# sonniki/image-captioning-with-external-knowledge

Hardware: AMD Instinct MI355X
Metric: decode_steps_per_sec (higher is better)
Workload: dtype f32 (3xbf16 split products, fp32 accumulate); 1 GPU; cfg2: geo variant, per-GPU batch 64 x 20 decode positions, 14x14x2048 features, K=20 knowledge rows, vocab 10000; global_batch=64, graph=True, collective_backend=none, split_allreduce=False, parallelism=dp1 (one flat-bucket all-reduce per step)

## Files before the change

image-captioning-with-external-knowledge_amd/csrc/backward.hip:

```cpp
#include "common.h"

namespace ick {
namespace {

template <int NJ>
__global__ __launch_bounds__(256) void layernorm_bwd_kernel(const float* __restrict__ dy, const float* __restrict__ x,
                                                            const float* __restrict__ res,
                                                            const float* __restrict__ gamma,
                                                            const float* __restrict__ mean,
                                                            const float* __restrict__ rstd, float* __restrict__ dz,
                                                            float* __restrict__ dgamma, float* __restrict__ dbeta,
                                                            int64_t rows, int d, int rows_per_block,
                                                            float* __restrict__ dx_drop, DropArg darg,
                                                            float* __restrict__ partials) {
    chain_priority();
    extern __shared__ float sm[];
    const Dropout drop = darg.get();
    const int lane = threadIdx.x & 63, wave = threadIdx.x >> 6;
    float ag[NJ], ab[NJ], gm[NJ];
#pragma unroll
    for (int j = 0; j < NJ; ++j) {
        const int c = lane + 64 * j;
        ag[j] = 0.f; ab[j] = 0.f;
        gm[j] = c < d ? gamma[c] : 0.f;
// ... 208 lines not shown
                const float gw = g * enc / 5.0f;
#pragma unroll
                for (int w = 0; w < 5; ++w)
                    if (name[w] % kDetParts == p) dword[(int64_t)name[w] * d + c] += gw;
            }
            g = enc_g;
        }
        if (c >= type_off && ty % kDetParts == p) dtype_emb[(int64_t)ty * (d - type_off) + (c - type_off)] += g;
    }
}

__global__ __launch_bounds__(256) void fact_encode_bwd_det_kernel(const float* __restrict__ dfe,
                                                                  const int64_t* __restrict__ facts, float* __restrict__ dee,
                                                                  float* __restrict__ dpred, int num_pred, int B, int K,
                                                                  int F, int d) {
    const int p = blockIdx.x, c = blockIdx.y * 256 + threadIdx.x;
    for (int row = 0; row < B * F; ++row) {
        const int b = row / F;
        int subj = (int)facts[(int64_t)row * 3 + 1];
        int pred = (int)facts[(int64_t)row * 3 + 2];
        subj = subj < 0 ? 0 : (subj >= K ? K - 1 : subj);
        pred = pred < 0 ? 0 : (pred >= num_pred ? num_pred - 1 : pred);
        const bool e_mine = (b * K + subj) % kDetParts == p, p_mine = pred % kDetParts == p;
        if ((!e_mine && !p_mine) || c >= d) continue;
        const float g = dfe[(int64_t)row * d + c];
        if (e_mine) dee[((int64_t)b * K + subj) * d + c] += g;
        if (p_mine) dpred[(int64_t)pred * d + c] += g;
    }
}

__global__ __launch_bounds__(256) void pointer_bwd_dh_kernel(const float* __restrict__ ds, int64_t ds_ld, int col0,
                                                             const float* __restrict__ ctx, const float* __restrict__ w,
                                                             const float* __restrict__ ind, float* __restrict__ dh,
                                                             int T, int Kc, int d) {
    chain_priority();
    const int b = blockIdx.y, t = blockIdx.x;
    const float* dsr = ds + ((int64_t)b * T + t) * ds_ld + col0;
    for (int c = threadIdx.x; c < d; c += 256) {
        float acc = 0.f;
        const float* cc = ctx + (int64_t)b * Kc * d + c;
        int k = 0;
        for (; k + 8 <= Kc; k += 8) {
            float v[8], g[8];
#pragma unroll
            for (int q = 0; q < 8; ++q) {
                v[q] = cc[(int64_t)(k + q) * d];
                g[q] = dsr[k + q];
                if (ind) g[q] *= ind[((int64_t)b * T + t) * Kc + k + q];
            }
#pragma unroll
            for (int q = 0; q < 8; ++q) acc = fmaf(g[q], v[q], acc);
        }
        for (; k < Kc; ++k) {
            float g = dsr[k];
            if (ind) g *= ind[((int64_t)b * T + t) * Kc + k];
            acc = fmaf(g, cc[(int64_t)k * d], acc);
        }
        dh[((int64_t)b * T + t) * d + c] += acc * w[c];
    }
}

template <bool SEQ>
__global__ __launch_bounds__(256) void pointer_bwd_dctx_kernel(const float* __restrict__ ds, int64_t ds_ld, int col0,
                                                               const float* __restrict__ h, const float* __restrict__ ctx,
                                                               const float* __restrict__ w, const float* __restrict__ ind,
                                                               float* __restrict__ dctx, float* __restrict__ dw,
                                                               float* __restrict__ dbias, int B, int T, int Kc, int d) {
    chain_priority();
    extern __shared__ float gs[];
    float* red = gs + T * Kc;
    float* dwp = red + 4;
    const int lane = threadIdx.x & 63, wave = threadIdx.x >> 6;
  for (int b = SEQ ? 0 : blockIdx.x; b < (SEQ ? B : (int)blockIdx.x + 1); ++b) {
    float bsum = 0.f;
    for (int idx = threadIdx.x; idx < T * Kc; idx += 256) {
        const int t = idx / Kc, k = idx - t * Kc;
        float g = ds[((int64_t)b * T + t) * ds_ld + col0 + k];
        bsum += g;
        if (ind) g *= ind[((int64_t)b * T + t) * Kc + k];
        gs[idx] = g;
    }
    bsum = block_sum<4>(bsum, red);
    if (threadIdx.x == 0 && blockIdx.y == 0) { if (SEQ) dbias[0] += bsum; else atomicAdd(dbias, bsum); }
    const int c = blockIdx.y * 64 + lane;
    const bool ok = c < d;
    const float* hb = h + (int64_t)b * T * d + (ok ? c : 0);
    const float wc = ok ? w[c] : 0.f;
    float dwl = 0.f;
    for (int k = wave; k < Kc; k += 4) {
        float acc = 0.f;
        for (int t = 0; t < T; ++t) acc = fmaf(gs[t * Kc + k], hb[(int64_t)t * d], acc);
        if (ok) {
            const int64_t o = ((int64_t)b * Kc + k) * d + c;
            dctx[o] += acc * wc;
            dwl = fmaf(acc, ctx[o], dwl);
        }
    }
    dwp[wave * 64 + lane] = dwl;
    __syncthreads();
    if (wave == 0 && ok) {
        const float t = (dwp[lane] + dwp[64 + lane]) + (dwp[128 + lane] + dwp[192 + lane]);
        if (SEQ) dw[c] += t; else atomicAdd(dw + c, t);
    }
    if (SEQ) __syncthreads();
  }
}

__global__ __launch_bounds__(256) void entity_encode_bwd_kernel(int variant, const float* __restrict__ dee,
                                                                const float* __restrict__ ent, int cols,
                                                                const float* __restrict__ ee,
// ... 226 lines not shown
    hipLaunchKernelGGL(relu_bwd_kernel, dim3((int)std::min<int64_t>(ceil_div(n, 256), 2048)), dim3(256), 0,
                       (hipStream_t)stream, dy, act, dx, n, scale);
    ICK_LAUNCH_RET();
}

extern "C" int ick_colsum(const float* a, int64_t M, int32_t N, int64_t ld, float* out, void* stream) {
    ICK_CHECK_ARG(a && out && M > 0 && N > 0 && ld >= N);
    const int rpb = deterministic() ? (int)std::min<int64_t>(M, 1 << 30) : 64;
    ICK_CHECK_ARG(ceil_div(M, rpb) <= 65535);
    hipLaunchKernelGGL(colsum_kernel, dim3(ceil_div(N, 64), ceil_div(M, rpb)), dim3(256), 0, (hipStream_t)stream, a, M,
                       N, ld, out, rpb);
    ICK_LAUNCH_RET();
}

extern "C" int ick_caption_embed_bwd(const float* dx, const int64_t* captions, const int64_t* masks, float* dword,
                                     float* dee, float* dfe, int32_t B, int32_t L, int32_t K, int32_t F, int32_t V,
                                     int32_t d, int32_t pad_token, float scale, float drop_p, uint32_t drop_seed,
                                     uint32_t drop_site, const uint32_t* drop_epoch, void* stream) {
    ICK_CHECK_ARG(dx && captions && masks && dee && B > 0 && L > 0 && K > 0 && d > 0);
    if (deterministic())
        hipLaunchKernelGGL(caption_embed_bwd_det_kernel, dim3(kDetParts, ceil_div(d, 256)), dim3(256), 0,
                           (hipStream_t)stream, dx, captions, masks, dword, dee, dfe, B, L, K, F, V, d, pad_token, scale,
                           DropArg{drop_p, drop_seed, drop_site, drop_epoch});
    else
        hipLaunchKernelGGL(caption_embed_bwd_kernel, dim3(ceil_div((int64_t)B * L, 4)), dim3(256), 0, (hipStream_t)stream,
                           dx, captions, masks, dword, dee, dfe, B, L, K, F, V, d, pad_token, scale,
                           DropArg{drop_p, drop_seed, drop_site, drop_epoch});
    ICK_LAUNCH_RET();
}

extern "C" int ick_pointer_scores_bwd(const float* ds, int64_t ds_ld, int32_t col0, const float* h, const float* ctx,
                                      const float* w, const float* ind, float* dh, float* dctx, float* dw,
                                      float* dbias, int32_t B, int32_t T, int32_t Kc, int32_t d, void* stream) {
    ICK_CHECK_ARG(ds && h && ctx && w && dh && dctx && dw && dbias && B > 0 && B <= 65535 && T > 0 && Kc > 0 && d > 0);
    hipStream_t s = (hipStream_t)stream;
    hipLaunchKernelGGL(pointer_bwd_dh_kernel, dim3(T, B), dim3(256), 0, s, ds, ds_ld, col0, ctx, w, ind, dh, T, Kc, d);
    const size_t smem = ((size_t)T * Kc + 4 + 256) * sizeof(float);
    ICK_CHECK_ARG(smem <= 64 * 1024);
    if (deterministic())
        hipLaunchKernelGGL(pointer_bwd_dctx_kernel<true>, dim3(1, ceil_div(d, 64)), dim3(256), smem, s, ds, ds_ld, col0, h,
                           ctx, w, ind, dctx, dw, dbias, B, T, Kc, d);
    else
        hipLaunchKernelGGL(pointer_bwd_dctx_kernel<false>, dim3(B, ceil_div(d, 64)), dim3(256), smem, s, ds, ds_ld, col0, h,
                           ctx, w, ind, dctx, dw, dbias, B, T, Kc, d);
    ICK_LAUNCH_RET();
}

extern "C" int ick_entity_encode_bwd(int32_t variant, const float* dee, const float* entities, int32_t ent_cols,
                                     const float* ee, const float* word_emb, int32_t vocab, float* dtype_emb,
                                     int32_t ntypes, float* dword, int32_t B, int32_t K, int32_t d, void* stream) {
    ICK_CHECK_ARG(dee && entities && dtype_emb && B > 0 && K > 0 && d > 6);
    if (variant == ICK_NEWS) ICK_CHECK_ARG(ee && word_emb && vocab > 0);
    if (deterministic())
        hipLaunchKernelGGL(entity_encode_bwd_det_kernel, dim3(kDetParts, ceil_div(d, 256)), dim3(256), 0,
                           (hipStream_t)stream, variant, dee, entities, ent_cols, ee, word_emb, vocab, dtype_emb, ntypes,
                           dword, B, K, d);
    else
        hipLaunchKernelGGL(entity_encode_bwd_kernel, dim3(ceil_div((int64_t)B * K, 4)), dim3(256), 0, (hipStream_t)stream,
                           variant, dee, entities, ent_cols, ee, word_emb, vocab, dtype_emb, ntypes, dword, B, K, d);
    ICK_LAUNCH_RET();
}

extern "C" int ick_fact_encode_bwd(const float* dfe, const int64_t* facts, float* dee, float* dpred, int32_t num_pred,
                                   int32_t B, int32_t K, int32_t F, int32_t d, void* stream) {
    ICK_CHECK_ARG(dfe && facts && dee && dpred && B > 0 && K > 0 && F > 0 && d > 0);
    if (deterministic())
        hipLaunchKernelGGL(fact_encode_bwd_det_kernel, dim3(kDetParts, ceil_div(d, 256)), dim3(256), 0, (hipStream_t)stream,
                           dfe, facts, dee, dpred, num_pred, B, K, F, d);
    else
        hipLaunchKernelGGL(fact_encode_bwd_kernel, dim3(ceil_div((int64_t)B * F, 4)), dim3(256), 0, (hipStream_t)stream,
                           dfe, facts, dee, dpred, num_pred, B, K, F, d);
    ICK_LAUNCH_RET();
}

extern "C" int ick_context_gate_bwd(const int64_t* captions, const int64_t* facts, const float* dgate, float* dw,
                                    float* dbias, int32_t B, int32_t L, int32_t T, int32_t K, int32_t F, int32_t V,
                                    int32_t num_pred, int32_t d, int32_t mode, void* stream) {
// ... 53 lines not shown
```

image-captioning-with-external-knowledge_amd/csrc/common.h:

```cpp
#pragma once
#include <hip/hip_runtime.h>
#include <stdint.h>
#include <stdlib.h>

#include "ick_amd.h"

namespace ick {

using f32x4 = __attribute__((ext_vector_type(4))) float;

constexpr int kWave = 64;

inline int ceil_div(int64_t a, int64_t b) { return (int)((a + b - 1) / b); }

extern int g_deterministic;
inline bool deterministic() {
    if (g_deterministic < 0) {
        const char* e = getenv("ICK_DETERMINISTIC");
        g_deterministic = (e && e[0] && e[0] != '0') ? 1 : 0;
    }
    return g_deterministic == 1;
}

#define ICK_CHECK_ARG(cond)          \
// ... 84 lines not shown
    for (int i = 1; i < NW; ++i) r = fmaxf(r, scratch[i]);
    return r;
}

__device__ __forceinline__ uint32_t drop_hash(uint32_t seed, uint32_t site, uint32_t idx) {
    uint32_t x = idx * 0x9E3779B1u ^ (seed + site * 0x85EBCA6Bu);
    x ^= x >> 16; x *= 0x85EBCA6Bu; x ^= x >> 13; x *= 0xC2B2AE35u; x ^= x >> 16;
    return x;
}
struct Dropout {
    uint32_t thr, seed, site;
    float scale;
    __device__ __forceinline__ bool on() const { return thr != 0u; }
    __device__ __forceinline__ float mask(uint32_t idx) const { return drop_hash(seed, site, idx) >= thr ? scale : 0.f; }
};
__host__ __device__ __forceinline__ Dropout make_dropout(float p, uint32_t seed, uint32_t site) {
    Dropout d{0u, seed, site, 1.f};
    if (p > 0.f) {
        d.thr = (uint32_t)fminf(p * 4294967296.f, 4294967040.f);
        d.scale = 1.f / (1.f - p);
    }
    return d;
}
__device__ __forceinline__ uint32_t epoch_seed(uint32_t seed, const uint32_t* epoch) {
    if (epoch == nullptr) return seed;
#if defined(__HIP_DEVICE_COMPILE__)
    uint32_t v;
    asm volatile("s_load_dword %0, %1, 0x0\n\ts_waitcnt lgkmcnt(0)" : "=s"(v) : "s"(epoch) : "memory");
    return seed + v;
#else
    return seed + *epoch;
#endif
}
constexpr int kRuleHistMax = 128;
__device__ __forceinline__ uint4 rule_words(const int32_t* words) {
    if (words == nullptr) return make_uint4(0u, 0u, 0u, 0u);
#if defined(__HIP_DEVICE_COMPILE__)
    uint64_t w01;
    uint32_t w2;
    asm volatile("s_load_dwordx2 %0, %2, 0x0\n\ts_load_dword %1, %2, 0x8\n\ts_waitcnt lgkmcnt(0)"
                 : "=&s"(w01), "=&s"(w2) : "s"(words) : "memory");
    return make_uint4((uint32_t)w01, (uint32_t)(w01 >> 32), w2, 0u);
#else
    return make_uint4((uint32_t)words[0], (uint32_t)words[1], (uint32_t)words[2], (uint32_t)words[3]);
#endif
}

template <typename Tok>
__device__ __forceinline__ void mark_bans(const Tok* hist, int t, int n, int m, int end_token, uint32_t* bits, int c0,
                                          int nwords, int* hs) {
    const int tid = threadIdx.x, nt = blockDim.x;
    for (int w = tid; w < nwords; w += nt) bits[w] = 0u;
    if (n > 0)
        for (int p = tid; p < t; p += nt) hs[p] = (int)hist[p];
    __syncthreads();
    if (n > 0) {
        for (int p = n - 1 + tid; p < t; p += nt) {
            bool match = true;
            for (int j = 1; j < n; ++j) match = match && hs[p - j] == hs[t - j];
            const int c = hs[p] - c0;
            if (match && c >= 0 && c < 32 * nwords) atomicOr(&bits[c >> 5], 1u << (c & 31));
        }
    }
    if (tid == 0 && t < m) {
        const int c = end_token - c0;
        if (c >= 0 && c < 32 * nwords) atomicOr(&bits[c >> 5], 1u << (c & 31));
// ... 13 lines not shown
```

image-captioning-with-external-knowledge_amd/csrc/gemm.hip:

```cpp
#include <algorithm>
#include <cmath>
#include <cstdlib>
#include <type_traits>

#include "common.h"
#include "gemm_common.h"

#ifdef ICK_GEMM_STAMPS
__device__ unsigned long long ick_gemm_stamps[16384][8];
#define ICK_GSTAMP(i)                                                                                          \
    do {                                                                                                       \
        if (threadIdx.x == 0 && stamp_id < 16384) ick_gemm_stamps[stamp_id][i] = __builtin_readcyclecounter(); \
    } while (0)
extern "C" int ick_debug_read_gemm_stamps(unsigned long long* out, int n) {
    return (int)hipMemcpyFromSymbol(out, HIP_SYMBOL(ick_gemm_stamps), sizeof(unsigned long long) * 8 * n);
}
#else
#define ICK_GSTAMP(i)
#endif

namespace ick {

int launch_gemm_ps(const ick_gemm_args& a, bool akm, int tile, int tiles_m, int tiles_n, int kchunk, int split, int a_nt,
                   hipStream_t s);
// ... 179 lines not shown
__device__ __forceinline__ void read_frag_spl(const float* lds, int row0, int i, int q, bf16x8_t (&f)[3]) {
    const char* base = reinterpret_cast<const char*>(lds);
    if constexpr (KM) {
        constexpr int KLINE = kmajor_kline(R), PLANE = 32 * KLINE;
        const char* at = base + (8 * q + (i >> 2)) * KLINE + ((row0 ^ ((kKmSwapOn * (q & 1)) << (kmajor_swap(R) + 2))) + 4 * (i & 3)) * 2;
#pragma unroll
        for (int p = 0; p < 3; ++p) {
            const s16x4_t lo4 = __builtin_amdgcn_ds_read_tr16_b64_v4i16((lds_s16x4_ptr)(at + p * PLANE));
            const s16x4_t hi4 = __builtin_amdgcn_ds_read_tr16_b64_v4i16((lds_s16x4_ptr)(at + p * PLANE + 4 * KLINE));
            f[p] = __builtin_bit_cast(bf16x8_t, __builtin_shufflevector(lo4, hi4, 0, 1, 2, 3, 4, 5, 6, 7));
        }
    } else {
        constexpr int PLANE = R * 64;
        const int row = row0 + i;
        const char* at = base + row * 64 + 16 * (q ^ kc_swz(row));
#pragma unroll
        for (int p = 0; p < 3; ++p)
            f[p] = __builtin_bit_cast(bf16x8_t, *reinterpret_cast<const u32x4_t*>(at + p * PLANE));
    }
}

__device__ __forceinline__ bool split_major(int& bid, int& zid, int nt, int nsplit) {
    if (nsplit < 8 || (nsplit & 7) != 0) return false;
    const int lin = bid + nt * zid;
    const int x = lin & 7, j = lin >> 3;
    const int r = j / nt;
    zid = x + 8 * r;
    bid = j - r * nt;
    return true;
}

template <int WM, int WN, int TM, int TN, bool AKM, bool BKM, bool VEC, int BKT, bool SPL = false, int LSTG = 2>
__device__ __forceinline__ void gemm_tile(const ick_gemm_args& p, int tiles_m, int tiles_n, int kchunk, int bid,
                                          int zid, float* smem, bool xcd_remap = true) {
    constexpr int BM = WM * TM * 16, BN = WN * TN * 16;
    constexpr int BK = BKT;
    using SA = Stager<BM, AKM, VEC, BKT, WM * WN * 64, SPL>;
    using SB = Stager<BN, BKM, VEC, BKT, WM * WN * 64, SPL>;
    constexpr int STAGE = SA::FLOATS + SB::FLOATS;
#ifdef ICK_GEMM_STAMPS
    const int stamp_id = bid + zid * tiles_m * tiles_n;
    if (threadIdx.x == 0 && stamp_id < 16384) {
        unsigned hw;
        asm volatile("s_getreg_b32 %0, hwreg(HW_REG_HW_ID)" : "=s"(hw));
        unsigned xcc;
        asm volatile("s_getreg_b32 %0, hwreg(HW_REG_XCC_ID)" : "=s"(xcc));
        ick_gemm_stamps[stamp_id][7] = ((unsigned long long)xcc << 32) | hw;
    }
#endif
    ICK_GSTAMP(0);

    const int nwg = tiles_m * tiles_n;
    if (xcd_remap) {
        const int xcd = bid & 7, qq = nwg >> 3, rr = nwg & 7;
        bid = (xcd < rr ? xcd * (qq + 1) : rr * (qq + 1) + (xcd - rr) * qq) + (bid >> 3);
    }
    int tm, tn;
    if (tiles_m <= tiles_n) { tm = bid % tiles_m; tn = bid / tiles_m; }
    else { tn = bid % tiles_n; tm = bid / tiles_n; }
    const int m0 = tm * BM, n0 = tn * BN;
    const int kbeg = zid * kchunk;
    const int kend = min(p.K, kbeg + kchunk);

    const RowMap amap{p.a_grp, p.a_gs, p.a_gmap, p.a_rs};
    const RowMap bmap{0, 0, nullptr, p.b_rs};
    SA sa; SB sb;
    sa.init(p.A, amap, p.a_ks, m0, p.M, p.a_extent);
    const bool only = (p.flags & ICK_GEMM_COLSUM_ONLY) != 0;
    sb.init(only ? p.A : p.B, bmap, p.b_ks, n0, p.N, p.b_extent);

    const int lane = threadIdx.x & 63, wave = threadIdx.x >> 6;
    const int wm = wave / WN, wn = wave % WN;
    const int fi = lane & 15, fq = lane >> 4;

    f32x4 acc[TM][TN];
#pragma unroll
    for (int a = 0; a < TM; ++a)
#pragma unroll
        for (int b = 0; b < TN; ++b) acc[a][b] = f32x4{0.f, 0.f, 0.f, 0.f};

    const int nk = (kend - kbeg + BK - 1) / BK;
    const bool colsum = AKM && p.colsum_a != nullptr && tn == 0;
    float csum = 0.f;
    if constexpr (SPL && AKM) sa.want_cs = colsum;
    if (nk > 0) {
        sa.template load<0>(kbeg, kend);
        if (!only) sb.template load<0>(kbeg, kend);
        if (nk > 1) { sa.template load<1>(kbeg + BK, kend); if (!only) sb.template load<1>(kbeg + BK, kend); }
        sa.template store<0>(smem, kbeg, kend);
        if (!only) sb.template store<0>(smem + SA::FLOATS, kbeg, kend);
    }
    __syncthreads();
    ICK_GSTAMP(1);
    auto phase = [&](int it, auto cur) {
        constexpr int CUR = decltype(cur)::value, NXT = 1 - CUR;
        const float* As = smem + (LSTG == 2 ? CUR * STAGE : 0);
        const float* Bs = As + SA::FLOATS;
        const int k0 = kbeg + it * BK;
        if (it + 2 < nk) { sa.template load<CUR>(k0 + 2 * BK, kend); if (!only) sb.template load<CUR>(k0 + 2 * BK, kend); }
        if constexpr (SPL) {
// ... 54 lines not shown
                    for (int b = 0; b < TN; ++b)
                        acc[a][b] = __builtin_amdgcn_mfma_f32_16x16x4f32(af[a][u], bf[b][u], acc[a][b], 0, 0, 0);
        }
        if constexpr (AKM && !SPL) {
            if (colsum && threadIdx.x < BM) {
#pragma unroll 8
                for (int k = 0; k < BK; ++k) csum += As[k * SA::LD + threadIdx.x];
            }
        }
        if constexpr (LSTG == 1) __syncthreads();
        if (it + 1 < nk) {
            float* An = smem + (LSTG == 2 ? NXT * STAGE : 0);
            sa.template store<NXT>(An, k0 + BK, kend);
            if (!only) sb.template store<NXT>(An + SA::FLOATS, k0 + BK, kend);
        }
        __syncthreads();
    };
    for (int it = 0; it < nk; it += 2) {
        phase(it, std::integral_constant<int, 0>{});
        if (it + 1 < nk) phase(it + 1, std::integral_constant<int, 1>{});
    }

    ICK_GSTAMP(2);
    if constexpr (SPL && AKM) {
        if (colsum) {
            *reinterpret_cast<float4*>(smem + sa.r0 * BM + 4 * sa.c) = sa.cs;
            __syncthreads();
            if (threadIdx.x < BM) {
#pragma unroll 4
                for (int r = 0; r < SA::KP; ++r) csum += smem[r * BM + threadIdx.x];
            }
        }
    }
    if (colsum && threadIdx.x < BM && m0 + (int)threadIdx.x < p.M) atomicAdd(p.colsum_a + m0 + threadIdx.x, csum);
    if (only) return;

    gemm_epilogue<TM, TN>(p, acc, m0, n0, wm, wn, fi, fq, zid);
    ICK_GSTAMP(3);
}

template <int WM, int WN, int TM, int TN, bool AKM, bool BKM, bool VEC, int BKT, bool SPL, int LSTG = 2>
__global__ __launch_bounds__(WM * WN * 64) void gemm_kernel(ick_gemm_args p, int tiles_m, int tiles_n, int kchunk) {
    extern __shared__ __attribute__((aligned(16))) float smem[];
    if constexpr (TM == 1) chain_priority();
    const int nt = tiles_m * tiles_n;
    int bid = blockIdx.x, zid = blockIdx.z;
    const bool by_split = split_major(bid, zid, nt, gridDim.z);
    gemm_tile<WM, WN, TM, TN, AKM, BKM, VEC, BKT, SPL, LSTG>(p, tiles_m, tiles_n, kchunk, bid, zid, smem, !by_split);
}

constexpr int kGroupMax = 8;
struct GroupArgs {
    int count;
    int wg_end[kGroupMax];
    int tiles_m[kGroupMax], tiles_n[kGroupMax], kchunk[kGroupMax], split[kGroupMax];
    ick_gemm_args g[kGroupMax];
};

template <int WM, int WN, int TM, int TN, bool AKM, bool BKM, bool VEC, int BKT, bool SPL>
__global__ __launch_bounds__(256) void gemm_group_kernel(GroupArgs ga) {
    extern __shared__ __attribute__((aligned(16))) float smem[];
    int gi = 0;
    while (gi + 1 < ga.count && (int)blockIdx.x >= ga.wg_end[gi]) ++gi;
    const int local = blockIdx.x - (gi > 0 ? ga.wg_end[gi - 1] : 0);
    const int nt = ga.tiles_m[gi] * ga.tiles_n[gi];
    if (local >= nt * ga.split[gi]) return;
    int zid = local / nt, bid = local - zid * nt;
    const bool by_split = split_major(bid, zid, nt, ga.split[gi]);
    gemm_tile<WM, WN, TM, TN, AKM, BKM, VEC, BKT, SPL>(ga.g[gi], ga.tiles_m[gi], ga.tiles_n[gi], ga.kchunk[gi], bid, zid,
                                                       smem, !by_split);
}

struct Plan {
    ick_gemm_args a;
    bool akm, bkm, vec;
    bool big;
    bool wide;
    bool spl;
    bool xl;
    bool ps;
    int ps_tile, ps_nt;
    int tiles_m, tiles_n, kchunk, split;
};

template <int WM, int WN, int TM, int TN, bool AKM, bool BKM, bool VEC, bool SPL, int LSTG = 2>
int launch_tile_s(const Plan& pl, hipStream_t s) {
    constexpr int BM = WM * TM * 16, BN = WN * TN * 16, NT = WM * WN * 64;
    constexpr int STAGE = Stager<BM, AKM, VEC, 32, NT, SPL>::FLOATS + Stager<BN, BKM, VEC, 32, NT, SPL>::FLOATS;
    constexpr size_t smem = LSTG * STAGE * sizeof(float);
    static_assert(smem <= 160 * 1024, "tile exceeds the LDS of a CU");
    const size_t lds = smem;
    if (lds > 64 * 1024) {
        static LdsAttrOnce attr;
        if (int e = attr.ensure(reinterpret_cast<const void*>(gemm_kernel<WM, WN, TM, TN, AKM, BKM, VEC, 32, SPL, LSTG>), 160 * 1024))
            return e;
    }
    const int gx = pl.tiles_m * pl.tiles_n;
    hipLaunchKernelGGL((gemm_kernel<WM, WN, TM, TN, AKM, BKM, VEC, 32, SPL, LSTG>), dim3(gx, 1, pl.split),
                       dim3(NT), lds, s, pl.a, pl.tiles_m, pl.tiles_n, pl.kchunk);
    ICK_LAUNCH_RET();
}
template <int WM, int WN, int TM, int TN, bool AKM, bool BKM, bool VEC>
int launch_tile(const Plan& pl, hipStream_t s) {
// ... 52 lines not shown
        g_gemm_split = e ? std::min(2, std::max(0, atoi(e))) : 1;
    }
    return g_gemm_split;
}

inline bool aligned16(const void* p) { return (reinterpret_cast<uintptr_t>(p) & 15) == 0; }

int make_plan(const ick_gemm_args* in, Plan& pl, int force_big = 0) {
    if (!in) return ICK_EINVAL;
    ick_gemm_args& a = pl.a;
    a = *in;
    if (a.flags & ICK_GEMM_COLSUM_ONLY) {
        ICK_CHECK_ARG(a.A && a.colsum_a && a.M > 0 && a.K > 0);
        a.B = a.A; a.C = a.colsum_a; a.bias = nullptr; a.gate = nullptr;
        a.N = 1; a.b_rs = 1; a.b_ks = a.a_ks; a.c_rs = 1; a.c_grp = 0; a.hs_dh = 0; a.b_extent = a.a_extent;
        a.drop_p = 0.f;
        a.flags = ICK_GEMM_COLSUM_ONLY | ICK_GEMM_ATOMIC;
    }
    ICK_CHECK_ARG(a.A && a.B && a.C);
    ICK_CHECK_ARG(a.M > 0 && a.N > 0 && a.K > 0);
    const bool akm = a.a_rs == 1 && a.a_ks != 1, bkm = a.b_rs == 1 && a.b_ks != 1;
    ICK_CHECK_ARG((a.a_rs == 1) || (a.a_ks == 1));
    ICK_CHECK_ARG((a.b_rs == 1) || (a.b_ks == 1));
    if (a.split_k > 1) ICK_CHECK_ARG(a.flags & ICK_GEMM_ATOMIC);
    if (a.colsum_a) ICK_CHECK_ARG(akm);
    if (a.gate) ICK_CHECK_ARG(a.hs_dh <= 0 && a.c_grp <= 0 && a.split_k <= 1 && !(a.flags & (ICK_GEMM_ATOMIC | ICK_GEMM_ACCUM)));
    if (a.hs_dh > 0) {
        ICK_CHECK_ARG(a.hs_dhp >= a.hs_dh && a.hs_H > 0 && a.hs_S > 0 && a.hs_s0 >= 0);
        ICK_CHECK_ARG(a.N % (a.hs_H * a.hs_dh) == 0);
        ICK_CHECK_ARG(a.hs_s0 + (a.c_grp > 0 ? a.c_grp : a.M) <= a.hs_S);
    } else {
        a.hs_dh = 0;
    }
    if (a.a_grp <= 0) { a.a_grp = 0; a.a_gmap = nullptr; }
    if (a.c_grp <= 0) { a.c_grp = 0; a.c_gmap = nullptr; }
    bool avec, bvec;
    if (akm) {
        avec = aligned16(a.A) && a.a_ks % 4 == 0 && a.M % 4 == 0 && (a.a_grp == 0 || (a.a_grp % 4 == 0 && a.a_gs % 4 == 0));
    } else {
        avec = aligned16(a.A) && a.a_rs % 4 == 0 && a.K % 4 == 0 && (a.a_grp == 0 || a.a_gs % 4 == 0);
    }
    if (a.flags & ICK_GEMM_COLSUM_ONLY) bvec = true;
    else if (bkm) bvec = aligned16(a.B) && a.b_ks % 4 == 0 && a.N % 4 == 0;
    else bvec = aligned16(a.B) && a.b_rs % 4 == 0 && a.K % 4 == 0;
    auto extent_of = [](int64_t rows, int64_t rs, int64_t K, int64_t ks, int grp, int64_t gs, bool has_map) -> int64_t {
        if (has_map) return 0;
        if (grp <= 0) return (rows - 1) * rs + (K - 1) * ks + 1;
        const int64_t ng = (rows + grp - 1) / grp;
        return (ng - 1) * gs + (std::min<int64_t>(grp, rows) - 1) * rs + (K - 1) * ks + 1;
    };
    if (a.a_extent <= 0) a.a_extent = extent_of(a.M, a.a_rs, a.K, a.a_ks, a.a_grp, a.a_gs, a.a_gmap != nullptr);
    if (a.b_extent <= 0) a.b_extent = extent_of(a.N, a.b_rs, a.K, a.b_ks, 0, 0, false);
    const int64_t kMaxExtent = ((int64_t)1 << 29) - 64;
    a.a_extent = std::min(a.a_extent & ~(int64_t)3, kMaxExtent - 4);
    a.b_extent = std::min(a.b_extent & ~(int64_t)3, kMaxExtent - 4);
    const int64_t a_need = extent_of(a.M, a.a_rs, a.K, a.a_ks, a.a_grp, a.a_gs, a.a_gmap != nullptr);
    const int64_t b_need = extent_of(a.N, a.b_rs, a.K, a.b_ks, 0, 0, false);
    pl.vec = avec && bvec && a.a_extent >= 4 && a.b_extent >= 4 && a_need <= a.a_extent + 3 && b_need <= a.b_extent + 3;
    pl.akm = akm; pl.bkm = bkm;
    a.flags &= 0xff;
    const int split_req = a.split_k > 1 ? a.split_k : 1;
    const int64_t wgs64 = (int64_t)ceil_div(a.M, 64) * ceil_div(a.N, 64) * split_req;
    pl.big = !pl.vec || wgs64 >= 512;
    if (force_big > 0) pl.big = true;
    pl.wide = pl.vec && pl.big && a.M >= 128 && akm && !bkm && a.N <= 320 && a.M >= 4096 && a.K >= 1024 && split_req == 1;
    pl.spl = pl.vec && pl.big && (gemm_split_mode() == 2 || (gemm_split_mode() == 1 && !bkm));
// ... 139 lines not shown
```

image-captioning-with-external-knowledge_amd/csrc/gemm_common.h:

```cpp
#pragma once
#include "common.h"

namespace ick {
namespace {

struct RowMap {
    int grp;
    int64_t gs;
    const int32_t* gmap;
    int64_t rs;
    __device__ __forceinline__ int64_t operator()(int r) const {
        if (grp <= 0) return (int64_t)r * rs;
        const int g = r / grp;
        const int i = r - g * grp;
        const int64_t gg = gmap ? (int64_t)gmap[g] : (int64_t)g;
        return gg * gs + (int64_t)i * rs;
    }
};

template <int N>
__device__ __forceinline__ void map_rows(const RowMap& m, const int (&rows)[N], int64_t (&off)[N]) {
    if (m.grp <= 0) {
#pragma unroll
        for (int i = 0; i < N; ++i) off[i] = (int64_t)rows[i] * m.rs;
// ... 13 lines not shown
    for (int i = 0; i < N; ++i) off[i] = (int64_t)g[i] * m.gs + (int64_t)in[i] * m.rs;
}

__device__ __forceinline__ int64_t col_offset(const ick_gemm_args& p, int col) {
    if (p.hs_dh <= 0) return col;
    const int hd = p.hs_H * p.hs_dh;
    const int seg = col / hd, r = col - seg * hd;
    const int h = r / p.hs_dh, j = r - h * p.hs_dh;
    return ((int64_t)seg * p.hs_H + h) * ((int64_t)p.hs_S * p.hs_dhp) + j;
}

typedef unsigned int u32x4_t __attribute__((ext_vector_type(4)));
constexpr uint32_t kOobOffset = 0x80000000u;

typedef __bf16 bf16x2_t __attribute__((ext_vector_type(2)));
typedef __bf16 bf16x8_t __attribute__((ext_vector_type(8)));
typedef float f32x2_t __attribute__((ext_vector_type(2)));
typedef short s16x4_t __attribute__((ext_vector_type(4)));
typedef __attribute__((address_space(3))) s16x4_t* lds_s16x4_ptr;

__device__ __forceinline__ uint32_t pack_bf16(float a, float b) {
    return __builtin_bit_cast(uint32_t, __builtin_convertvector(f32x2_t{a, b}, bf16x2_t));
}
__device__ __forceinline__ void split3(float a, float b, uint32_t& hi, uint32_t& mid, uint32_t& lo) {
    hi = pack_bf16(a, b);
    const float ra = a - __builtin_bit_cast(float, hi << 16), rb = b - __builtin_bit_cast(float, hi & 0xffff0000u);
    mid = pack_bf16(ra, rb);
    const float sa = ra - __builtin_bit_cast(float, mid << 16), sb = rb - __builtin_bit_cast(float, mid & 0xffff0000u);
    lo = pack_bf16(sa, sb);
}
__device__ __forceinline__ int kc_swz(int row) { return (-(row >> 2)) & 3; }

template <int TM, int TN>
__device__ __forceinline__ void gemm_epilogue(const ick_gemm_args& p, f32x4 (&acc)[TM][TN], int m0, int n0, int wm, int wn,
                                              int fi, int fq, int zid) {
    const bool hs = p.hs_dh > 0;
    const RowMap cmap{p.c_grp, p.c_gs, p.c_gmap, hs ? (int64_t)p.hs_dhp : p.c_rs};
    const int64_t row_bias = hs ? (int64_t)p.hs_s0 * p.hs_dhp : 0;
    const bool relu = p.flags & ICK_GEMM_RELU;
    const int mode = (p.flags & ICK_GEMM_ATOMIC) ? 2 : ((p.flags & ICK_GEMM_ACCUM) ? 1 : 0);
    float bv[TN];
    int cols[TN];
    int64_t co[TN];
#pragma unroll
    for (int b = 0; b < TN; ++b) {
        cols[b] = n0 + (wn * TN + b) * 16 + fi;
        co[b] = col_offset(p, cols[b]);
        bv[b] = (p.bias != nullptr && zid == 0 && cols[b] < p.N) ? p.bias[cols[b]] : 0.f;
    }
    const float alpha = p.alpha;
    int64_t coff[TM][4];
    int rowid[TM][4];
    const Dropout drop = make_dropout(p.drop_p, epoch_seed(p.drop_seed, p.drop_epoch), p.drop_site);
    {
        int rws[TM * 4];
        int64_t mo[TM * 4];
#pragma unroll
        for (int a = 0; a < TM; ++a)
#pragma unroll
            for (int r = 0; r < 4; ++r) {
                rowid[a][r] = m0 + (wm * TM + a) * 16 + fq * 4 + r;
                rws[a * 4 + r] = min(rowid[a][r], p.M - 1);
            }
        map_rows<TM * 4>(cmap, rws, mo);
#pragma unroll
        for (int a = 0; a < TM; ++a)
#pragma unroll
            for (int r = 0; r < 4; ++r) coff[a][r] = rowid[a][r] < p.M ? mo[a * 4 + r] + row_bias : -1;
    }
#pragma unroll
    for (int a = 0; a < TM; ++a)
#pragma unroll
        for (int r = 0; r < 4; ++r)
#pragma unroll
            for (int b = 0; b < TN; ++b) {
                float v = acc[a][b][r] * alpha + bv[b];
                if (relu) v = fmaxf(v, 0.f);
                if (drop.on()) v *= drop.mask((uint32_t)rowid[a][r] * (uint32_t)p.N + (uint32_t)cols[b]);
                acc[a][b][r] = v;
            }
    if (p.gate != nullptr) {
        float g[TM][4][TN];
#pragma unroll
        for (int a = 0; a < TM; ++a)
#pragma unroll
            for (int r = 0; r < 4; ++r)
#pragma unroll
                for (int b = 0; b < TN; ++b)
                    g[a][r][b] = p.gate[(coff[a][r] >= 0 && cols[b] < p.N) ? (int64_t)rowid[a][r] * p.gate_rs + cols[b] : 0];
#pragma unroll
        for (int a = 0; a < TM; ++a)
#pragma unroll
            for (int r = 0; r < 4; ++r)
#pragma unroll
                for (int b = 0; b < TN; ++b) acc[a][b][r] = g[a][r][b] > 0.f ? acc[a][b][r] * p.gate_scale : 0.f;
    }
    if (mode == 1) {
        float old[TM][4][TN];
#pragma unroll
        for (int a = 0; a < TM; ++a)
#pragma unroll
// ... 33 lines not shown
```

image-captioning-with-external-knowledge_amd/csrc/gemm_ps.hip:

```cpp
#include <algorithm>

#include "gemm_common.h"

#ifdef ICK_PS_STAMPS
__device__ unsigned long long ick_ps_stamps[10];
#define ICK_PSTAMP(var)                                   \
    do {                                                  \
        __builtin_amdgcn_sched_barrier(0);                \
        var = __builtin_amdgcn_s_memtime();               \
        __builtin_amdgcn_sched_barrier(0);                \
    } while (0)
extern "C" int ick_debug_read_ps_stamps(unsigned long long* out) {
    return (int)hipMemcpyFromSymbol(out, HIP_SYMBOL(ick_ps_stamps), sizeof(ick_ps_stamps));
}
#else
#define ICK_PSTAMP(var)
#endif

namespace ick {
namespace {

typedef __attribute__((address_space(3))) void* lds_void_ptr;

inline int64_t ps_rows(int N) { return (int64_t)ceil_div(N, 64) * 64; }
inline int64_t ps_bytes(int N, int K) { return (int64_t)ceil_div(K, 32) * 3 * ps_rows(N) * 64; }

constexpr int kPsMaxItems = 16;
struct PsBatch {
    int count;
    int first[kPsMaxItems + 1];
    ick_presplit_item it[kPsMaxItems];
};

__global__ __launch_bounds__(256) void presplit_kernel(PsBatch b) {
    __shared__ float tile[64][33];
    int gi = 0;
    while (gi + 1 < b.count && (int)blockIdx.x >= b.first[gi + 1]) ++gi;
    const ick_presplit_item it = b.it[gi];
    const int local = blockIdx.x - b.first[gi];
    const int blocks_n = (it.N + 63) / 64;
    const int nb = local % blocks_n, s = local / blocks_n;
    const int t = threadIdx.x;
    const float* src = it.src;
    const bool al16 = (reinterpret_cast<uintptr_t>(src) & 15) == 0;
    if (it.src_cs == 1) {
        const int r = t >> 2, kk = (t & 3) * 8;
        const int n = nb * 64 + r;
        const int k0 = 32 * s + kk;
        if (al16 && (it.src_rs & 3) == 0 && n < it.N && k0 + 7 < it.K) {
            const float4* q = reinterpret_cast<const float4*>(src + (int64_t)n * it.src_rs + k0);
            const float4 a = q[0], b = q[1];
            tile[r][kk + 0] = a.x; tile[r][kk + 1] = a.y; tile[r][kk + 2] = a.z; tile[r][kk + 3] = a.w;
            tile[r][kk + 4] = b.x; tile[r][kk + 5] = b.y; tile[r][kk + 6] = b.z; tile[r][kk + 7] = b.w;
        } else {
#pragma unroll
            for (int j = 0; j < 8; ++j) {
                const int k = k0 + j;
                tile[r][kk + j] = (n < it.N && k < it.K) ? src[(int64_t)n * it.src_rs + k] : 0.f;
            }
        }
    } else {
        const int kk = t >> 3, r0 = (t & 7) * 8;
        const int k = 32 * s + kk;
        const int n0 = nb * 64 + r0;
        if (al16 && it.src_rs == 1 && (it.src_cs & 3) == 0 && n0 + 7 < it.N && k < it.K) {
            const float4* q = reinterpret_cast<const float4*>(src + n0 + (int64_t)k * it.src_cs);
            const float4 a = q[0], b = q[1];
            tile[r0 + 0][kk] = a.x; tile[r0 + 1][kk] = a.y; tile[r0 + 2][kk] = a.z; tile[r0 + 3][kk] = a.w;
            tile[r0 + 4][kk] = b.x; tile[r0 + 5][kk] = b.y; tile[r0 + 6][kk] = b.z; tile[r0 + 7][kk] = b.w;
        } else {
#pragma unroll
            for (int j = 0; j < 8; ++j) {
                const int n = n0 + j;
                tile[n - nb * 64][kk] = (n < it.N && k < it.K) ? src[(int64_t)n * it.src_rs + (int64_t)k * it.src_cs] : 0.f;
            }
        }
    }
    __syncthreads();
    const int r = t >> 2, c = t & 3;
    uint32_t h[4], m[4], l[4];
#pragma unroll
    for (int j = 0; j < 4; ++j) split3(tile[r][8 * c + 2 * j], tile[r][8 * c + 2 * j + 1], h[j], m[j], l[j]);
    const int64_t np = (int64_t)blocks_n * 64;
    char* dst = reinterpret_cast<char*>(it.dst) + ((int64_t)s * 3 * np + nb * 64 + r) * 64 + c * 16;
    *reinterpret_cast<uint4*>(dst) = uint4{h[0], h[1], h[2], h[3]};
    *reinterpret_cast<uint4*>(dst + np * 64) = uint4{m[0], m[1], m[2], m[3]};
    *reinterpret_cast<uint4*>(dst + 2 * np * 64) = uint4{l[0], l[1], l[2], l[3]};
}

}

template <int WM_, int WN_, int TM_, int TN_, bool AKM_, int D_, int PF_>
struct PsCfg {
    static constexpr int WM = WM_, WN = WN_, TM = TM_, TN = TN_, D = D_;
    static constexpr int PF = PF_ < TN_ ? PF_ : TN_;
    static constexpr int ST = D + 1;
    static constexpr bool AKM = AKM_;
    static constexpr int BM = WM * TM * 16, BN = WN * TN * 16, NW = WM * WN, NT = NW * 64;
    static constexpr int A_STAGE = BM * 32 * 4;
    static constexpr int B_PLANE = BN * 64;
    static constexpr int B_STAGE = 3 * B_PLANE;
    static constexpr int NPA = BM / 8;
    static constexpr int NPB = 3 * BN / 16;
    static constexpr int PA_W = NPA / NW;
    static constexpr int PB_W = (NPB + NW - 1) / NW;
    static constexpr bool UNIFORM = D >= 2;
    static constexpr int SCRATCH = UNIFORM && (NPB % NW != 0) ? 1024 : 0;
// ... 74 lines not shown
#ifdef ICK_PS_STAMPS
    unsigned long long t_start = 0, t_loop = 0, t_end = 0;
    ICK_PSTAMP(t_start);
    const unsigned long long rt_start = __builtin_amdgcn_s_memrealtime();
#endif
    char* const As = smem_ps;
    char* const Bs = smem_ps + ST * C::A_STAGE;
    char* const scratch = Bs + ST * C::B_STAGE;
    const int lane = threadIdx.x & 63;
    const int wave = __builtin_amdgcn_readfirstlane((int)(threadIdx.x >> 6));
    constexpr int WN = C::WN;
    const int wm = wave / WN, wn = wave % WN;
    const int fi = lane & 15, fq = lane >> 4;

    int bid = blockIdx.x;
    int zid = blockIdx.z;
    {
        const int nwg = tiles_m * tiles_n;
        if (gridDim.z > 1) {
            const int total = nwg * (int)gridDim.z, lin = bid + nwg * zid;
            const int xcd = lin & 7, qq = total >> 3, rr = total & 7;
            const int v = xcd * qq + min(xcd, rr) + (lin >> 3);
            zid = v / nwg;
            bid = v - zid * nwg;
        } else {
            const int xcd = bid & 7, qq = nwg >> 3, rr = nwg & 7;
            bid = (xcd < rr ? xcd * (qq + 1) : rr * (qq + 1) + (xcd - rr) * qq) + (bid >> 3);
        }
    }
    int tm, tn;
    if (tiles_m <= tiles_n) { tm = bid % tiles_m; tn = bid / tiles_m; }
    else { tn = bid % tiles_n; tm = bid / tiles_n; }
    const int m0 = tm * BM, n0 = tn * BN;
    const int kbeg = zid * kchunk;
    const int kend = min(p.K, kbeg + kchunk);
    const int nk = (kend - kbeg + 31) >> 5;
    const int s0 = kbeg >> 5;

    const __amdgpu_buffer_rsrc_t rsrc_a =
        __builtin_amdgcn_make_buffer_rsrc(const_cast<float*>(p.A), (short)0, (int)(p.a_extent * 4), 0x00020000);
    const RowMap amap{p.a_grp, p.a_gs, p.a_gmap, p.a_rs};
    uint32_t avoff[C::PA_W];
    int akl[C::PA_W];
#pragma unroll
    for (int j = 0; j < C::PA_W; ++j) {
        const int g = wave + NW * j;
        int row, extra;
        if constexpr (AKM) {
            constexpr int LPK = BM / 4, KPP = 64 / LPK;
            const int kl = g * KPP + lane / LPK, cpos = lane % LPK;
            const int c = (cpos - 4 * ((kl >> 3) & 3)) & (LPK - 1);
            row = m0 + 4 * c;
            akl[j] = kl;
            extra = 0;
            const int one[1] = {min(row, p.M - 1)};
            int64_t mo[1];
            map_rows<1>(amap, one, mo);
            avoff[j] = row < p.M ? (uint32_t)(mo[0] * 4) + (uint32_t)((int64_t)kl * p.a_ks * 4) : kOobOffset;
        } else {
            const int rt = g * 8 + (lane >> 3), cpos = lane & 7;
            const int c = cpos ^ ((rt >> 1) & 7);
            row = m0 + rt;
            akl[j] = 4 * c;
            extra = 4 * c;
            const int one[1] = {min(row, p.M - 1)};
            int64_t mo[1];
            map_rows<1>(amap, one, mo);
            avoff[j] = row < p.M ? (uint32_t)((mo[0] + extra) * 4) : kOobOffset;
        }
    }
    const __amdgpu_buffer_rsrc_t rsrc_b =
        __builtin_amdgcn_make_buffer_rsrc(const_cast<void*>(p.b_ps), (short)0, (int)bps_bytes, 0x00020000);
    const uint32_t bvoff = (uint32_t)((n0 + (lane >> 2)) * 64 + (((lane & 3) ^ ((-(lane >> 4)) & 3)) * 16));

    auto dma_b = [&](int it, int buf) { ps_dma_b<C>(rsrc_b, Bs, scratch, buf, wave, bvoff, s0 + it, it < nk, n0, np_rows); };
    auto dma_a = [&](int it, int buf) {
        const int k0 = kbeg + 32 * it;
        const uint32_t soff = it < nk ? (uint32_t)(AKM ? (int64_t)k0 * p.a_ks * 4 : (int64_t)k0 * 4) : 0u;
        ps_dma_a<C>(rsrc_a, As, buf, wave, avoff, akl, k0, kend, soff, a_nt != 0);
    };

    f32x4 acc[TM][TN];
#pragma unroll
    for (int a = 0; a < TM; ++a)
#pragma unroll
        for (int b = 0; b < TN; ++b) acc[a][b] = f32x4{0.f, 0.f, 0.f, 0.f};

#pragma unroll
    for (int i = 0; i < D; ++i) { dma_b(i, i); dma_a(i, i); }
    ICK_WAIT_VMCNT(C::IN_FLIGHT);
    ICK_LDS_BARRIER();

#ifdef ICK_PS_STAMPS
    unsigned long long ph[6] = {0, 0, 0, 0, 0, 0}, ta = 0, tb = 0, tc = 0, td = 0, te = 0, tf = 0;
    ICK_PSTAMP(t_loop);
#endif
    int buf = 0;
    for (int it = 0; it < nk; ++it) {
        ICK_PSTAMP(ta);
        int nb = buf + D;
        if (nb >= ST) nb -= ST;
// ... 56 lines not shown
                for (int j = 0; j < GB; ++j)
#pragma unroll
                    for (int a = 0; a < TM; ++a) {
                        const int b = g * GB + j;
                        if (b < TN)
                            acc[a][b] = __builtin_amdgcn_mfma_f32_16x16x32_bf16(af[a][pa[q]], bf[g & 1][j][pb[q]], acc[a][b], 0, 0, 0);
                    }
                constexpr int NS = NG * 6, NP = C::PB_W + C::PA_W;
                constexpr int SPAN = D >= 2 ? NS : (NS + 1) / 2;
                constexpr int STRIDE = SPAN / NP > 0 ? SPAN / NP : 1;
                const int slot = g * 6 + q;
                if (slot % STRIDE == 0 && slot / STRIDE < NP) piece(slot / STRIDE);
                if (slot == NS - 1) {
#pragma unroll
                    for (int r = (NS - 1) / STRIDE + 1; r < NP; ++r) piece(r);
                }
            }
        }
        ICK_PSTAMP(td);
        ICK_WAIT_VMCNT(C::IN_FLIGHT);
        ICK_PSTAMP(te);
        ICK_LDS_BARRIER();
        ICK_PSTAMP(tf);
#ifdef ICK_PS_STAMPS
        ph[0] += tb - ta; ph[1] += tc - tb; ph[2] += td - tc; ph[3] += te - td; ph[4] += tf - te; ph[5] += 1;
#endif
        if (++buf == ST) buf = 0;
    }
#ifdef ICK_PS_STAMPS
    ICK_PSTAMP(t_end);
    const unsigned long long t_loop_end = t_end;
#endif
    ICK_WAIT_VMCNT(0);
    gemm_epilogue<TM, TN>(p, acc, m0, n0, wm, wn, fi, fq, zid);
#ifdef ICK_PS_STAMPS
    asm volatile("s_waitcnt vmcnt(0)" ::: "memory");
    ICK_PSTAMP(t_end);
    if (threadIdx.x == 0 && blockIdx.x == (gridDim.x >> 1) && blockIdx.z == 0) {
        for (int i = 0; i < 6; ++i) ick_ps_stamps[i] = ph[i];
        ick_ps_stamps[6] = t_loop - t_start;
        ick_ps_stamps[7] = t_end - t_loop_end;
        ick_ps_stamps[8] = t_end - t_start;
        ick_ps_stamps[9] = __builtin_amdgcn_s_memrealtime() - rt_start;
    }
#endif
}


namespace {

template <class C>
int launch_ps_cfg(const ick_gemm_args& a, int np_rows, int64_t bytes, int tiles_m, int tiles_n, int kchunk, int split,
                  int a_nt, hipStream_t s) {
    static LdsAttrOnce attr;
    if (int e = attr.ensure(reinterpret_cast<const void*>(gemm_ps_kernel<C::WM, C::WN, C::TM, C::TN, C::AKM, C::D, C::PF>), 160 * 1024))
        return e;
    hipLaunchKernelGGL((gemm_ps_kernel<C::WM, C::WN, C::TM, C::TN, C::AKM, C::D, C::PF>), dim3(tiles_m * tiles_n, 1, split),
                       dim3(C::NT), C::LDS, s, a, np_rows, bytes, tiles_m, tiles_n, kchunk, a_nt);
    ICK_LAUNCH_RET();
}

template <int WM, int WN, int TM, int TN, int D, int PF>
int launch_ps_tile(const ick_gemm_args& a, bool akm, int np, int64_t bytes, int tiles_m, int tiles_n, int kchunk, int split,
                   int a_nt, hipStream_t s) {
    if (akm) return launch_ps_cfg<PsCfg<WM, WN, TM, TN, true, D, PF>>(a, np, bytes, tiles_m, tiles_n, kchunk, split, a_nt, s);
    return launch_ps_cfg<PsCfg<WM, WN, TM, TN, false, D, PF>>(a, np, bytes, tiles_m, tiles_n, kchunk, split, a_nt, s);
}
// ... 18 lines not shown
        case 1: return launch_ps_tile<8, 1, 1, 8, 1, 2>(a, akm, np, bytes, tiles_m, tiles_n, kchunk, split, a_nt, s);
        case 2: return launch_ps_tile<8, 1, 1, 10, 2, 10>(a, akm, np, bytes, tiles_m, tiles_n, kchunk, split, a_nt, s);
        case 3: return launch_ps_tile<4, 2, 2, 10, 1, 3>(a, akm, np, bytes, tiles_m, tiles_n, kchunk, split, a_nt, s);
        case 4: return launch_ps_tile<8, 1, 1, 8, 2, 8>(a, akm, np, bytes, tiles_m, tiles_n, kchunk, split, a_nt, s);
        case 5: return launch_ps_tile<4, 2, 2, 4, 1, 2>(a, akm, np, bytes, tiles_m, tiles_n, kchunk, split, a_nt, s);
        case 6: return launch_ps_tile<4, 2, 2, 5, 2, 5>(a, akm, np, bytes, tiles_m, tiles_n, kchunk, split, a_nt, s);
        case 7: return launch_ps_tile<4, 1, 2, 8, 1, 2>(a, akm, np, bytes, tiles_m, tiles_n, kchunk, split, a_nt, s);
        case 8: return launch_ps_tile<2, 2, 2, 5, 1, 5>(a, akm, np, bytes, tiles_m, tiles_n, kchunk, split, a_nt, s);
        case 9: return launch_ps_tile<8, 1, 1, 5, 1, 2>(a, akm, np, bytes, tiles_m, tiles_n, kchunk, split, a_nt, s);
        case 10: return launch_ps_tile<8, 1, 1, 10, 1, 10>(a, akm, np, bytes, tiles_m, tiles_n, kchunk, split, a_nt, s);
    }
    return ICK_EINVAL;
}

}

extern "C" int ick_presplit_bytes(int32_t N, int32_t K, int64_t* bytes) {
    if (N <= 0 || K <= 0 || !bytes) return ICK_EINVAL;
    *bytes = ick::ps_bytes(N, K);
    return ICK_OK;
}

extern "C" int ick_presplit_weights(const ick_presplit_item* items, int32_t count, void* stream) {
    using namespace ick;
    if (!items || count <= 0) return ICK_EINVAL;
    for (int i0 = 0; i0 < count; i0 += kPsMaxItems) {
        PsBatch b;
        b.count = std::min(kPsMaxItems, count - i0);
        int total = 0;
        for (int i = 0; i < b.count; ++i) {
            const ick_presplit_item& it = items[i0 + i];
            ICK_CHECK_ARG(it.src && it.dst && it.N > 0 && it.K > 0);
            ICK_CHECK_ARG(it.src_cs == 1 || it.src_rs == 1);
            ICK_CHECK_ARG((reinterpret_cast<uintptr_t>(it.dst) & 15) == 0);
            b.it[i] = it;
            b.first[i] = total;
            total += ceil_div(it.N, 64) * ceil_div(it.K, 32);
        }
        b.first[b.count] = total;
        hipLaunchKernelGGL(presplit_kernel, dim3(total), dim3(256), 0, (hipStream_t)stream, b);
        hipError_t e = hipGetLastError();
        if (e != hipSuccess) return (int)e;
    }
    return ICK_OK;
}
```

image-captioning-with-external-knowledge_amd/csrc/score_head.hip:

```cpp
#include "common.h"

namespace ick {
namespace {

constexpr int kMaxPerLane = 16;

template <int NJ>
__global__ __launch_bounds__(256) void pointer_scores_kernel(const float* __restrict__ h, const float* __restrict__ ctx,
                                                             const float* __restrict__ w, const float* __restrict__ bias,
                                                             const float* __restrict__ ind, float* __restrict__ out,
                                                             int T, int Kc, int d, int64_t out_ld, int col0,
                                                             const int32_t* __restrict__ out_gmap) {
    chain_priority();
    constexpr int KB = 4;
    const int lane = threadIdx.x & 63, wave = threadIdx.x >> 6;
    const int b = blockIdx.y, t = blockIdx.x;
    const float* hr = h + ((int64_t)b * T + t) * d;
    float hv[NJ], wv[NJ];
#pragma unroll
    for (int j = 0; j < NJ; ++j) {
        const int c = lane + 64 * j;
        hv[j] = c < d ? hr[c] : 0.f;
        wv[j] = c < d ? w[c] : 0.f;
    }
    const int ob = out_gmap ? out_gmap[b] : b;
    float* orow = out + ((int64_t)ob * T + t) * out_ld + col0;
    const float bs = bias[0];
    for (int k0 = wave; k0 < Kc; k0 += 4 * KB) {
        float cv[KB][NJ];
#pragma unroll
        for (int q = 0; q < KB; ++q) {
            const int k = k0 + 4 * q;
            const float* cr = ctx + ((int64_t)b * Kc + (k < Kc ? k : 0)) * d;
#pragma unroll
            for (int j = 0; j < NJ; ++j) {
                const int c = lane + 64 * j;
                cv[q][j] = (k < Kc && c < d) ? cr[c] : 0.f;
            }
        }
#pragma unroll
        for (int q = 0; q < KB; ++q) {
            const int k = k0 + 4 * q;
            if (k >= Kc) break;
            float acc = 0.f;
#pragma unroll
            for (int j = 0; j < NJ; ++j) acc = fmaf(__fmul_rn(hv[j], cv[q][j]), wv[j], acc);
            acc = wave_sum(acc);
            if (lane == 0) {
                const float f = ind ? ind[((int64_t)b * T + t) * Kc + k] : 1.f;
                orow[k] = acc * f + bs;
            }
        }
    }
}

struct Top2 {
    float v1, v2;
    int i1, i2;
};
// ... 81 lines not shown
    }
    out = o[i];
    if (i < max_len - 1) {
        next_token[b] = out;
        next_mask[b] = (has_facts && out >= V + K) ? 2 : (out >= V ? 1 : 0);
    }
}

__global__ void greedy_update_kernel(const int32_t* __restrict__ best, const int32_t* __restrict__ second,
                                     int64_t* __restrict__ output, int32_t* __restrict__ hist,
                                     int32_t* __restrict__ finished, int64_t* __restrict__ next_token,
                                     int64_t* __restrict__ next_mask, int B, int step, int max_len, int V, int K,
                                     int has_facts, int end_token) {
    const int b = blockIdx.x * blockDim.x + threadIdx.x;
    if (b >= B) return;
    greedy_update_one(b, best[b], second[b], output, hist, finished, next_token, next_mask, step, max_len, V, K,
                      has_facts, end_token);
}

__global__ __launch_bounds__(256) void greedy_select_kernel(const float* __restrict__ scores, int64_t ld, int Vx,
                                                            int64_t* __restrict__ output, int32_t* __restrict__ hist,
                                                            int32_t* __restrict__ finished,
                                                            int64_t* __restrict__ next_token,
                                                            int64_t* __restrict__ next_mask, int step, int max_len,
                                                            int V, int K, int has_facts, int end_token) {
    __shared__ Top2 sh[256];
    const int b = blockIdx.x;
    const Top2 t = row_top2(scores + (int64_t)b * ld, Vx, sh);
    if (threadIdx.x == 0)
        greedy_update_one(b, t.i1, t.i2 == 0x7fffffff ? t.i1 : t.i2, output, hist, finished, next_token, next_mask, step,
                          max_len, V, K, has_facts, end_token);
}

template <bool kWeighted>
__global__ __launch_bounds__(256) void packed_ce_rows_kernel(const float* __restrict__ scores, int64_t ld,
                                                             const int64_t* __restrict__ caps,
                                                             const int32_t* __restrict__ dl, int L, int Vx, int pad,
                                                             float* __restrict__ row_loss, float* __restrict__ dscores,
                                                             const float* __restrict__ weight) {
    __shared__ float red[4];
    const int t = blockIdx.x, b = blockIdx.y, tid = threadIdx.x;
    const int64_t row = (int64_t)b * L + t;
    const float* r = scores + row * ld;
    float* dr = dscores ? dscores + row * ld : nullptr;
    int64_t target = -1;
    bool use = t < L - 1 && t < dl[b];
    if (use) {
        target = caps[(int64_t)b * L + t + 1];
        use = target != pad && target >= 0 && target < Vx;
    }
    if (!use) {
        if (tid == 0) row_loss[row] = -1.f;
        if (dr) {
            const int z4 = ((ld & 3) == 0 && (reinterpret_cast<uintptr_t>(dscores) & 15) == 0) ? (int)(Vx >> 2) : 0;
            float4* d4 = reinterpret_cast<float4*>(dr);
            for (int i = tid; i < z4; i += 256) d4[i] = make_float4(0.f, 0.f, 0.f, 0.f);
            for (int i = 4 * z4 + tid; i < Vx; i += 256) dr[i] = 0.f;
        }
        return;
    }
    constexpr int kCeVec = 10;
    const bool in_regs = (Vx & 3) == 0 && (ld & 3) == 0 && Vx <= 256 * 4 * kCeVec &&
                         (reinterpret_cast<uintptr_t>(scores) & 15) == 0 &&
                         (dr == nullptr || (reinterpret_cast<uintptr_t>(dscores) & 15) == 0);
    if (in_regs) {
        const float4* r4 = reinterpret_cast<const float4*>(r);
        const int n4 = Vx >> 2;
        float4 x[kCeVec];
        float m = -INFINITY;
#pragma unroll
        for (int j = 0; j < kCeVec; ++j) {
            const int i = tid + 256 * j;
            x[j] = i < n4 ? r4[i] : make_float4(-INFINITY, -INFINITY, -INFINITY, -INFINITY);
            m = fmaxf(m, fmaxf(fmaxf(x[j].x, x[j].y), fmaxf(x[j].z, x[j].w)));
        }
        m = block_max<4>(m, red);
        float s = 0.f;
#pragma unroll
        for (int j = 0; j < kCeVec; ++j) {
// ... 81 lines not shown
            }
#pragma unroll
            for (int j = 0; j < 4; ++j) {
                const int i = i0 + tid + 256 * j;
                if (i < n4) {
                    float4 gq = make_float4(__expf(x[j].x - m) * inv, __expf(x[j].y - m) * inv, __expf(x[j].z - m) * inv,
                                            __expf(x[j].w - m) * inv);
                    if (i == tq) {
                        if (tr == 0) gq.x -= wr; else if (tr == 1) gq.y -= wr; else if (tr == 2) gq.z -= wr; else gq.w -= wr;
                    }
                    d4[i] = gq;
                }
            }
        }
        for (int i0 = 4 * n4; i0 < Vx; i0 += 256 * 8) {
            float x[8];
#pragma unroll
            for (int j = 0; j < 8; ++j) {
                const int i = i0 + tid + 256 * j;
                x[j] = i < Vx ? r[i] : 0.f;
            }
#pragma unroll
            for (int j = 0; j < 8; ++j) {
                const int i = i0 + tid + 256 * j;
                if (i < Vx) dr[i] = __expf(x[j] - m) * inv - (i == target ? wr : 0.f);
            }
        }
    }
}

template <bool kWeighted>
__global__ __launch_bounds__(256) void packed_ce_reduce_kernel(const float* __restrict__ row_loss, int n, int L,
                                                               const float* __restrict__ weight,
                                                               float* __restrict__ loss_sum, float* __restrict__ count) {
    __shared__ float red[4];
    float s = 0.f, c = 0.f;
    for (int i = threadIdx.x; i < n; i += 256) {
        const float v = row_loss[i];
        if (v > -0.5f) { s += kWeighted ? weight[i / L] * v : v; c += 1.f; }
    }
    s = block_sum<4>(s, red);
    c = block_sum<4>(c, red);
    if (threadIdx.x == 0) { loss_sum[0] = s; count[0] = c; }
}

}
}

extern "C" int ick_pointer_scores(const float* h, const float* ctx, const float* w, const float* bias,
                                  const float* ind, float* out, int32_t B, int32_t T, int32_t Kc, int32_t d,
                                  int64_t out_ld, int32_t col0, const int32_t* out_gmap, void* stream) {
    using namespace ick;
    ICK_CHECK_ARG(h && ctx && w && bias && out && B > 0 && T > 0 && Kc > 0 && d > 0 && d <= 64 * kMaxPerLane);
    ICK_CHECK_ARG(B <= 65535 && col0 >= 0 && out_ld >= col0 + Kc);
    hipStream_t s = (hipStream_t)stream;
    if (d <= 320)
        hipLaunchKernelGGL(pointer_scores_kernel<5>, dim3(T, B), dim3(256), 0, s, h, ctx, w, bias, ind, out, T, Kc, d,
                           out_ld, col0, out_gmap);
    else if (d <= 512)
        hipLaunchKernelGGL(pointer_scores_kernel<8>, dim3(T, B), dim3(256), 0, s, h, ctx, w, bias, ind, out, T, Kc, d,
                           out_ld, col0, out_gmap);
    else
        hipLaunchKernelGGL(pointer_scores_kernel<kMaxPerLane>, dim3(T, B), dim3(256), 0, s, h, ctx, w, bias, ind, out, T,
                           Kc, d, out_ld, col0, out_gmap);
    ICK_LAUNCH_RET();
}

extern "C" int ick_top2(const float* scores, int64_t ld, int32_t B, int32_t Vx, int32_t* best, int32_t* second,
                        void* stream) {
    using namespace ick;
    ICK_CHECK_ARG(scores && best && second && B > 0 && Vx > 0 && ld >= Vx);
    hipLaunchKernelGGL(top2_kernel, dim3(B), dim3(256), 0, (hipStream_t)stream, scores, ld, Vx, best, second);
    ICK_LAUNCH_RET();
}

extern "C" int ick_greedy_update(const int32_t* best, const int32_t* second, int64_t* output, int32_t* top2_hist,
                                 int32_t* finished, int64_t* next_token, int64_t* next_mask, int32_t B, int32_t step,
                                 int32_t max_len, int32_t V, int32_t K, int32_t has_facts, int32_t end_token,
                                 void* stream) {
    using namespace ick;
    ICK_CHECK_ARG(best && second && output && top2_hist && finished && next_token && next_mask);
    ICK_CHECK_ARG(B > 0 && step >= 0 && step < max_len);
    hipLaunchKernelGGL(greedy_update_kernel, dim3(ceil_div(B, 64)), dim3(64), 0, (hipStream_t)stream, best, second,
                       output, top2_hist, finished, next_token, next_mask, B, step, max_len, V, K, has_facts,
                       end_token);
    ICK_LAUNCH_RET();
}

extern "C" int ick_greedy_select(const float* scores, int64_t ld, int32_t B, int32_t Vx, int64_t* output,
                                 int32_t* top2_hist, int32_t* finished, int64_t* next_token, int64_t* next_mask,
                                 int32_t step, int32_t max_len, int32_t V, int32_t K, int32_t has_facts,
                                 int32_t end_token, void* stream) {
    using namespace ick;
    ICK_CHECK_ARG(scores && output && top2_hist && finished && next_token && next_mask);
    ICK_CHECK_ARG(B > 0 && Vx > 0 && ld >= Vx && step >= 0 && step < max_len);
    hipLaunchKernelGGL(greedy_select_kernel, dim3(B), dim3(256), 0, (hipStream_t)stream, scores, ld, Vx, output,
                       top2_hist, finished, next_token, next_mask, step, max_len, V, K, has_facts, end_token);
    ICK_LAUNCH_RET();
}

extern "C" int ick_packed_ce(const float* scores, int64_t ld, const int64_t* captions_sorted,
                             const int32_t* decode_len, int32_t B, int32_t L, int32_t Vx, int32_t pad_token,
                             float* row_loss, float* loss_sum, float* count, float* dscores, void* stream) {
    using namespace ick;
    ICK_CHECK_ARG(scores && captions_sorted && decode_len && row_loss && loss_sum && count);
    ICK_CHECK_ARG(B > 0 && B <= 65535 && L > 0 && Vx > 0 && ld >= Vx);
    hipStream_t s = (hipStream_t)stream;
    hipLaunchKernelGGL(packed_ce_rows_kernel<false>, dim3(L, B), dim3(256), 0, s, scores, ld, captions_sorted, decode_len,
                       L, Vx, pad_token, row_loss, dscores, nullptr);
    hipLaunchKernelGGL(packed_ce_reduce_kernel<false>, dim3(1), dim3(256), 0, s, row_loss, B * L, L, nullptr, loss_sum,
                       count);
    ICK_LAUNCH_RET();
}

extern "C" int ick_packed_ce_weighted(const float* scores, int64_t ld, const int64_t* captions_sorted,
                                      const int32_t* decode_len, const float* weights, int32_t B, int32_t L, int32_t Vx,
                                      int32_t pad_token, float* row_loss, float* loss_sum, float* count, float* dscores,
                                      void* stream) {
    using namespace ick;
    ICK_CHECK_ARG(scores && captions_sorted && decode_len && weights && row_loss && loss_sum && count);
    ICK_CHECK_ARG(B > 0 && B <= 65535 && L > 0 && Vx > 0 && ld >= Vx && (int64_t)B * L <= INT32_MAX);
    hipStream_t s = (hipStream_t)stream;
    hipLaunchKernelGGL(packed_ce_rows_kernel<true>, dim3(L, B), dim3(256), 0, s, scores, ld, captions_sorted, decode_len,
                       L, Vx, pad_token, row_loss, dscores, weights);
    hipLaunchKernelGGL(packed_ce_reduce_kernel<true>, dim3(1), dim3(256), 0, s, row_loss, B * L, L, weights, loss_sum,
                       count);
    ICK_LAUNCH_RET();
}
```

image-captioning-with-external-knowledge_amd/decoder.py:

```python
import math
import os
import struct

import torch
from torch import nn

from . import ops
from .lib import IckError

VARIANT_TYPE_OFFSET = {"geo": 4, "knowledge": 6, "news": 5}
VARIANT_NUM_TYPES = {"geo": 1000, "knowledge": 1000, "news": 20}
VARIANT_NUM_PREDICATES = {"geo": 0, "knowledge": 3000, "news": 3500}


def _sinusoid_table(max_len, d):
    pos = torch.arange(max_len, dtype=torch.float32).unsqueeze(1)
    freq = torch.exp(torch.arange(0, d, 2, dtype=torch.float32) * (-math.log(10000.0) / d))
    table = torch.zeros(max_len, d)
    table[:, 0::2] = torch.sin(pos * freq)
    table[:, 1::2] = torch.cos(pos * freq)
    return table.unsqueeze(1)


class _GraphedCall:
# ... 689 lines not shown
        dh = d // H
        x = t["x"]
        B, T, _ = x.shape
        t["ca"] = torch.empty_like(x)
        t["lse_c"] = torch.empty(B * H * T, device=x.device, dtype=torch.float32) if save else None
        ops.attention_heads(t["qc"], kv, t["ca"], H, dh, T, S, 0, 2 * li, 2 * li + 1, lse=t["lse_c"], drop=t["d_ca"])
        if pk is None:
            t["o2"] = ops.linear(t["ca"], *_wb(layer.multihead_attn.out_proj))
            t["x2"], t["m2"], t["r2"] = _with_stats(ops.add_layernorm(
                t["o2"], t["x1"], *_ln(layer.norm2), save_stats=save, drop=t["d2"]), save)
            t["f"] = ops.linear(t["x2"], *_wb(layer.linear1), relu=True, drop=t["d_ff"])
            t["o3"] = ops.linear(t["f"], *_wb(layer.linear2))
            x3, t["m3"], t["r3"] = _with_stats(ops.add_layernorm(
                t["o3"], t["x2"], *_ln(layer.norm3), save_stats=save, drop=t["d3"]), save)
            return x3, None
        t["x2"] = torch.empty_like(x)
        t["o2"], t["o3"] = (torch.empty_like(x), torch.empty_like(x)) if save else (None, None)
        t["f"] = torch.empty(B, T, layer.linear1.out_features, device=x.device, dtype=torch.float32)
        t["m2"], t["r2"] = ops.rowchain_fwd(
            t["ca"], pk[("d", li, "co")], layer.multihead_attn.out_proj.bias.detach(), t["x1"], *_ln(layer.norm2),
            t["x2"], drop1=t["d2"], o_out=t["o2"], save_stats=save, w2p=pk[("d", li, "l1")],
            b2=layer.linear1.bias.detach(), y2=t["f"], relu=True, drop2=t["d_ff"])
        layers = self.transformer_decoder.layers
        nxt = layers[li + 1] if li + 1 < len(layers) else None
        x3 = torch.empty_like(x)
        qkv_n = None if nxt is None else torch.empty(B, 3, H, T, ops.DHP, device=x.device, dtype=torch.float32)
        t["m3"], t["r3"] = ops.rowchain_fwd(
            t["f"], pk[("d", li, "l2")], layer.linear2.bias.detach(), t["x2"], *_ln(layer.norm3), x3, drop1=t["d3"],
            o_out=t["o3"], save_stats=save, w2p=None if nxt is None else pk[("d", li + 1, "si")],
            b2=None if nxt is None else nxt.self_attn.in_proj_bias.detach(), y2=qkv_n,
            heads=None if nxt is None else (3, H, T, 0, T))
        return x3, qkv_n

    def _score_head(self, h, ee, fe, eib, hv, out, vocab_ps=None):
        B, T, d = h.shape
        V, K = self.vocab_size, ee.shape[1]
        ops.gemm_raw(h if hv is None else hv, self.fc_vocab.weight.detach(), out, B * T, V, d, d, 1, d, 1, out.stride(1),
                     bias=self.fc_vocab.bias.detach(), b_ps=vocab_ps)
        ops.pointer_scores(h, ee, *_wb(self.fc_entity), out, V)
        if self.has_facts:
            ops.pointer_scores(h, fe, *_wb(self.fc_fact), out, V + K, ind=eib)

    @torch.no_grad()
    def get_context_indicators(self, captions, facts, entity_context_size, out_length):
        if not self.has_facts:
            raise AttributeError("the geo variant has no get_context_indicators (geo-aware/models.py)")
        dev = self.fc_vocab.weight.device
        captions = captions.to(device=dev, dtype=torch.int64)
        facts = facts.to(device=dev, dtype=torch.int64).contiguous()
        B, Lc = captions.shape
        mode = 1 if out_length == 1 else 0
        if mode == 0 and out_length > Lc:
            captions = torch.cat([captions, captions.new_full((B, out_length - Lc), self.word_map["<pad>"])], dim=1)
        eib, pi = ops.context_indicators(captions.contiguous(), facts, entity_context_size, self.vocab_size, mode=mode,
                                         dense_pred=self.num_predicates)
        return eib[:, :out_length].unsqueeze(3), pi[:, :out_length].unsqueeze(3)

    @torch.no_grad()
    def get_scores(self, h, entities_encoded, facts_encoded=None, entity_idx_before=None, predicate_indicator=None):
        dev = self.fc_vocab.weight.device
        hb = h.detach().to(dev, torch.float32).permute(1, 0, 2).contiguous()
        ee = entities_encoded.detach().to(dev, torch.float32).contiguous()
        B, T, d = hb.shape
        fe = eib = hv = None
        if self.has_facts:
            if facts_encoded is None or entity_idx_before is None or predicate_indicator is None:
                raise IckError("%s variant: get_scores(h, entities_encoded, facts_encoded, entity_idx_before, "
                               "predicate_indicator)" % self.variant)
            fe = facts_encoded.detach().to(dev, torch.float32).contiguous()
            eib = entity_idx_before.detach().to(dev, torch.float32).reshape(B, T, fe.shape[1]).contiguous()
            pi = predicate_indicator.detach().to(dev, torch.float32).reshape(B * T, self.num_predicates).contiguous()
            gate = ops.linear(pi, self.fc_predicate.weight.detach(), self.fc_predicate.bias.detach()).view(B, T, d)
            hv = ops.mul(hb, gate)
        out = torch.empty(B, T, self.vocab_size + ee.shape[1] + (0 if fe is None else fe.shape[1]), device=dev,
# ... 603 lines not shown
```

image-captioning-with-external-knowledge_amd/lib.py:

```python
import ctypes as C
import os

_PKG = os.path.dirname(os.path.abspath(__file__))
LIB_PATH = os.path.join(_PKG, "libick_amd.so")
if os.environ.get("ICK_LIB_PATH"):
    LIB_PATH = os.environ["ICK_LIB_PATH"]

ICK_GEO, ICK_KNOWLEDGE, ICK_NEWS = 0, 1, 2
VARIANT_ID = {"geo": ICK_GEO, "knowledge": ICK_KNOWLEDGE, "news": ICK_NEWS}
GEMM_RELU, GEMM_ACCUM, GEMM_ATOMIC, GEMM_COLSUM_ONLY = 1, 2, 4, 16

vp = C.c_void_p
i32 = C.c_int32
i64 = C.c_int64
f32 = C.c_float
u32 = C.c_uint32


class GemmArgs(C.Structure):
    _fields_ = [
        ("A", vp), ("B", vp), ("C", vp), ("bias", vp),
        ("M", i32), ("N", i32), ("K", i32),
        ("a_rs", i64), ("a_ks", i64), ("a_grp", i32), ("a_gs", i64), ("a_gmap", vp),
        ("b_rs", i64), ("b_ks", i64),
        ("c_rs", i64), ("c_grp", i32), ("c_gs", i64), ("c_gmap", vp),
        ("flags", i32), ("split_k", i32), ("alpha", f32),
        ("hs_dh", i32), ("hs_dhp", i32), ("hs_H", i32), ("hs_S", i32), ("hs_s0", i32),
        ("drop_p", f32), ("drop_seed", u32), ("drop_site", u32), ("drop_epoch", vp),
        ("a_extent", i64), ("b_extent", i64), ("colsum_a", vp),
        ("gate", vp), ("gate_rs", i64), ("gate_scale", f32),
        ("b_ps", vp),
    ]


class RowChainArgs(C.Structure):
    _fields_ = [
        ("A", vp), ("a_rs", i64), ("a_grp", i32), ("a_gs", i64),
        ("M", i32), ("K1", i32), ("d", i32),
        ("w1p", vp), ("b1", vp), ("res", vp), ("res_rs", i64),
        ("gamma", vp), ("beta", vp), ("eps", f32),
        ("drop1_p", f32), ("drop_seed", u32), ("drop1_site", u32), ("drop_epoch", vp),
        ("o", vp), ("o_rs", i64),
        ("x", vp), ("x_rs", i64), ("x_grp", i32), ("x_gs", i64),
        ("mean", vp), ("rstd", vp),
        ("w2p", vp), ("b2", vp), ("N2", i32), ("flags", i32),
        ("drop2_p", f32), ("drop2_site", u32),
        ("y2", vp), ("y2_rs", i64), ("y2_grp", i32), ("y2_gs", i64),
        ("hs_dh", i32), ("hs_dhp", i32), ("hs_H", i32), ("hs_S", i32), ("hs_s0", i32),
    ]


class RowChainBwdArgs(C.Structure):
    _fields_ = [
        ("M", i32), ("d", i32), ("drop_seed", u32), ("drop_epoch", vp),
        ("g0", vp), ("g0_rs", i64), ("K0", i32), ("w0p", vp), ("g0_grp", i32), ("g0_gs", i64),
        ("dzin", vp), ("dzin_rs", i64),
        ("o1", vp), ("res1", vp), ("mean1", vp), ("rstd1", vp), ("gamma1", vp),
        ("drop1_p", f32), ("drop1_site", u32),
        ("do1", vp), ("part1", vp),
        ("w1p", vp), ("N1", i32), ("act", vp), ("gate_scale", f32), ("t_out", vp),
        ("w2p", vp),
        ("o2", vp), ("res2", vp), ("mean2", vp), ("rstd2", vp), ("gamma2", vp),
        ("drop2_p", f32), ("drop2_site", u32),
        ("do2", vp), ("part2", vp),
        ("w3p", vp), ("out3", vp), ("dz_out", vp), ("flags", i32),
    ]


class PackItem(C.Structure):
    _fields_ = [("src", vp), ("dst", vp), ("N", i32), ("K", i32), ("src_rs", i64), ("src_cs", i64), ("dst_rs", i64)]


class GemmPlanInfo(C.Structure):
    _fields_ = [(n, i32) for n in ("tile_m", "tile_n", "waves", "tiles_m", "tiles_n", "split_k", "a_kmajor", "b_kmajor",
                                   "vec", "split_bf16", "presplit")]


class PresplitItem(C.Structure):
    _fields_ = [("src", vp), ("dst", vp), ("N", i32), ("K", i32), ("src_rs", i64), ("src_cs", i64)]


class AdamItem(C.Structure):
    _fields_ = [("off", i64), ("rows", i32), ("K", i32), ("drow0", i32), ("Nd", i32), ("pack", vp), ("pack_t", vp),
                ("copy", vp), ("ps", vp), ("ps_t", vp), ("tr", vp), ("copy_ld", i64), ("tr_ld", i64)]


class AdamBlock(C.Structure):
    _fields_ = [("item", i32), ("tn", i32), ("tk", i32), ("cnt4", i32), ("off4", i64), ("copy", vp)]


class AttnArgs(C.Structure):
    _fields_ = [
        ("Q", vp), ("K", vp), ("V", vp), ("O", vp), ("lse", vp),
        ("B", i32), ("H", i32), ("T", i32), ("S", i32), ("dh", i32),
        ("q_bs", i64), ("q_hs", i64), ("q_ts", i64), ("k_bs", i64), ("k_hs", i64), ("k_ss", i64),
        ("v_bs", i64), ("v_hs", i64), ("v_ss", i64), ("o_bs", i64), ("o_ts", i64),
        ("scale", f32), ("causal", i32), ("q_pos0", i32), ("kv_len", vp),
        ("drop_p", f32), ("drop_seed", u32), ("drop_site", u32), ("drop_epoch", vp),
    ]


class AttnBwdArgs(C.Structure):
    _fields_ = [
        ("Q", vp), ("K", vp), ("V", vp), ("O", vp), ("dO", vp), ("lse", vp), ("dQ", vp), ("dK", vp), ("dV", vp),
        ("B", i32), ("H", i32), ("T", i32), ("S", i32), ("dh", i32),
        ("q_bs", i64), ("q_hs", i64), ("q_ts", i64), ("k_bs", i64), ("k_hs", i64), ("k_ss", i64),
        ("v_bs", i64), ("v_hs", i64), ("v_ss", i64), ("o_bs", i64), ("o_ts", i64),
        ("dq_bs", i64), ("dq_ts", i64), ("dk_bs", i64), ("dk_ss", i64), ("dv_bs", i64), ("dv_ss", i64),
        ("scale", f32), ("causal", i32), ("q_pos0", i32),
        ("drop_p", f32), ("drop_seed", u32), ("drop_site", u32), ("drop_epoch", vp),
    ]

# ... 80 lines not shown
    "ick_decode_layers_attn": [C.POINTER(DecodeCtx), vp, i32, i32, vp],
    "ick_decode_init": [C.POINTER(DecodeCtx), i32, i32, vp],
    "ick_decode_select_greedy": [C.POINTER(DecodeCtx), i32, vp],
    "ick_decode_select_beam": [C.POINTER(DecodeCtx), C.POINTER(BeamState), i32, vp],
    "ick_decode_beam_supported": [i32, i32],
    "ick_decode_select_sample": [C.POINTER(DecodeCtx), C.POINTER(SampleState), i32, vp],
    "ick_decode_sample_supported": [i32, i32],
    "ick_decode_select_beam_rules": [C.POINTER(DecodeCtx), C.POINTER(BeamState), C.POINTER(DecodeRules), i32, vp],
    "ick_decode_select_sample_rules": [C.POINTER(DecodeCtx), C.POINTER(SampleState), C.POINTER(DecodeRules), i32, vp],
    "ick_decode_select_beam_diverse": [C.POINTER(DecodeCtx), C.POINTER(BeamState), C.POINTER(DecodeRules),
                                       C.POINTER(DecodeDiversity), i32, vp],
    "ick_decode_select_beam_forced": [C.POINTER(DecodeCtx), C.POINTER(BeamState), C.POINTER(DecodeRules),
                                      C.POINTER(DecodeConstraints), i32, vp],
    "ick_attention_bwd": [C.POINTER(AttnBwdArgs), vp],
    "ick_layernorm_bwd": [vp, vp, vp, vp, vp, vp, vp, vp, vp, i64, i32, vp, f32, u32, u32, vp, vp, vp],
    "ick_layernorm_bwd_rows_per_block": [],
    "ick_gemm_grouped": [vp, i32, vp],
    "ick_attention_bwd_overwrites": [i32, i32, i32],
    "ick_attention_plan": [i32, i32, i32, i32, i32, C.POINTER(i32)],
    "ick_relu_bwd": [vp, vp, vp, i64, f32, vp],
    "ick_colsum": [vp, i64, i32, i64, vp, vp],
    "ick_caption_embed_bwd": [vp, vp, vp, vp, vp, vp, i32, i32, i32, i32, i32, i32, i32, f32, f32, u32, u32, vp, vp],
    "ick_pointer_scores_bwd": [vp, i64, i32, vp, vp, vp, vp, vp, vp, vp, vp, i32, i32, i32, i32, vp],
    "ick_entity_encode_bwd": [i32, vp, vp, i32, vp, vp, i32, vp, i32, vp, i32, i32, i32, vp],
    "ick_fact_encode_bwd": [vp, vp, vp, vp, i32, i32, i32, i32, i32, vp],
    "ick_context_gate_bwd": [vp, vp, vp, vp, vp, i32, i32, i32, i32, i32, i32, i32, i32, i32, vp],
    "ick_adam_clamp": [vp, vp, vp, vp, i64, f32, f32, f32, f32, f32, f32, i32, vp, vp, vp],
    "ick_adam_clamp_derive": [vp, vp, vp, vp, vp, vp, i32, f32, f32, f32, f32, f32, f32, i32, vp, vp, vp],
    "ick_counter_add": [vp, u32, vp],
    "ick_counter_add_if": [vp, u32, vp, vp],
    "ick_timestamp": [vp, vp],
    "ick_copy_batch": [vp, vp, vp, i32, vp],
    "ick_scale_by_ratio": [vp, i64, vp, vp, vp],
}

_lib = None
PROFILE = None
_proxy = None


class IckError(RuntimeError):
    pass


def load():
    return _proxy if _proxy is not None else load_raw()


def load_raw():
    global _lib
    if _lib is None:
        if not os.path.exists(LIB_PATH):
            raise IckError(
                "libick_amd.so is missing (%s): build it with `python -c 'import __graft_entry__ as g; g.build()'`"
                " -- there is no fallback path" % LIB_PATH)
        import torch
        lib = C.CDLL(LIB_PATH)
        for name, argtypes in SIGNATURES.items():
            fn = getattr(lib, name)
            fn.argtypes = argtypes
            fn.restype = C.c_int
        _lib = lib
    return _lib


_ERRS = {-1: "ICK_EINVAL (bad shape / null pointer / unsupported size)", -2: "ICK_EALIGN", -3: "ICK_EWORKSPACE"}
# ... 6 lines not shown
```

image-captioning-with-external-knowledge_amd/ops.py:

```python
import contextlib
import ctypes as C
import gc
import math
import os

import torch

from . import lib as L


def _p(t):
    return None if t is None else t.data_ptr()


def _stream():
    return torch.cuda.current_stream().cuda_stream


def _f32c(t, name):
    if t.dtype != torch.float32 or not t.is_cuda:
        raise L.IckError("%s must be a float32 device tensor (got %s on %s)" % (name, t.dtype, t.device))
    return t


TIMED = None


def _extent(t):
    return (t.untyped_storage().nbytes() - t.storage_offset() * t.element_size()) // 4


def _drop(a, drop):
    if drop is not None and drop[0] > 0.0:
        a.drop_p, a.drop_seed, a.drop_site = float(drop[0]), int(drop[1]) & 0xFFFFFFFF, int(drop[2]) & 0xFFFFFFFF
        a.drop_epoch = _p(drop[3]) if len(drop) > 3 else None


def _dargs(drop):
    if drop is not None and drop[0] > 0.0:
        return (float(drop[0]), int(drop[1]) & 0xFFFFFFFF, int(drop[2]) & 0xFFFFFFFF,
                _p(drop[3]) if len(drop) > 3 else None)
    return 0.0, 0, 0, None


def gemm_args(A, B, Cout, M, N, K, a_rs, a_ks, b_rs, b_ks, c_rs, bias=None, a_grp=0, a_gs=0, a_gmap=None,
              c_grp=0, c_gs=0, c_gmap=None, relu=False, accumulate=False, atomic=False, split_k=1, alpha=1.0,
              drop=None, colsum_a=None, gate=None, gate_scale=1.0, b_ps=None):
    for t in (A, B, Cout):
        if t.dtype != torch.float32:
            raise L.IckError("ick_gemm operands must be float32, got %s" % t.dtype)
    a = L.GemmArgs()
    a.A, a.B, a.C, a.bias = _p(A), _p(B), _p(Cout), _p(bias)
    a.M, a.N, a.K = M, N, K
    a.a_rs, a.a_ks, a.a_grp, a.a_gs, a.a_gmap = a_rs, a_ks, a_grp, a_gs, _p(a_gmap)
    a.b_rs, a.b_ks = b_rs, b_ks
    a.c_rs, a.c_grp, a.c_gs, a.c_gmap = c_rs, c_grp, c_gs, _p(c_gmap)
    a.flags = (L.GEMM_RELU if relu else 0) | (L.GEMM_ACCUM if accumulate else 0) | (L.GEMM_ATOMIC if atomic else 0)
    a.split_k = split_k
    a.alpha = alpha
    a.a_extent, a.b_extent = _extent(A), _extent(B)
    a.colsum_a = _p(colsum_a)
    if gate is not None:
        a.gate, a.gate_rs, a.gate_scale = _p(gate), gate.stride(0), gate_scale
    if b_ps is not None:
        assert b_ps.numel() * b_ps.element_size() == presplit_bytes(N, K), "b_ps is not the pre-split copy of an (N, K) matrix"
        a.b_ps = _p(b_ps)
    _drop(a, drop)
    return a


DEFAULT_GEMM_SPLIT = 1


def presplit_bytes(N, K):
    n = L.i64()
    L.check(L.load_raw().ick_presplit_bytes(int(N), int(K), C.byref(n)), "ick_presplit_bytes")
    return int(n.value)


def presplit_weights(pairs):
    items = (L.PresplitItem * len(pairs))()
    for it, (src, dst) in zip(items, pairs):
        assert src.dim() == 2 and src.dtype == torch.float32 and (src.stride(1) == 1 or src.stride(0) == 1)
        assert dst.numel() * dst.element_size() == presplit_bytes(src.shape[0], src.shape[1])
        it.src, it.dst, it.N, it.K = _p(src), _p(dst), src.shape[0], src.shape[1]
        it.src_rs, it.src_cs = src.stride(0), src.stride(1)
    L.check(L.load().ick_presplit_weights(items, len(pairs), _stream()), "ick_presplit_weights")


def presplit_buffer(N, K, device):
    return torch.empty(presplit_bytes(N, K), device=device, dtype=torch.uint8)


def presplit_cached(holder, name, w2d, key):
    if gemm_split_mode() == 0:
        return None
    cache = holder.__dict__.setdefault("_ps_cache", {})
    ent = cache.get(name)
    nbytes = presplit_bytes(w2d.shape[0], w2d.shape[1])
    if ent is None or ent[1].numel() != nbytes or ent[1].device != w2d.device:
        ent = cache[name] = [None, torch.empty(nbytes, device=w2d.device, dtype=torch.uint8)]
    if ent[0] != key:
        presplit_weights([(w2d, ent[1])])
        ent[0] = key
    return ent[1]


def colsum_problem(a2d, out, split_k=1):
    rows, cols = a2d.shape
    a = L.GemmArgs()
    a.A, a.colsum_a = _p(a2d), _p(out)
    a.M, a.N, a.K = cols, 1, rows
    a.a_rs, a.a_ks = 1, a2d.stride(0)
    a.flags, a.split_k, a.alpha = L.GEMM_COLSUM_ONLY | (L.GEMM_ATOMIC if split_k > 1 else 0), split_k, 1.0
    a.a_extent = _extent(a2d)
    return a


def set_deterministic(on=True):
    L.check(L.load().ick_set_deterministic(1 if on else 0), "ick_set_deterministic")


def set_gemm_split(mode):
    L.check(L.load().ick_set_gemm_split(int(mode)), "ick_set_gemm_split")


def gemm_split_mode():
    return int(L.load().ick_get_gemm_split())


def is_deterministic():
    return bool(L.load().ick_get_deterministic())


def wgrad_split(rows, n_out, k_in, grouped=False):
    if is_deterministic():
        return 1
    tiles = ((n_out + 63) // 64) * ((k_in + 63) // 64)
    cap = 2 if grouped else 16
    return max(1, min(cap, rows // 256, (1600 + tiles // 2) // tiles))


CONV1_TILE = (128, 64)


def conv1_tile():
    return (128, 80) if gemm_split_mode() >= 1 else CONV1_TILE

# ... 303 lines not shown
    B, Lc = captions.shape
    K, d = entities_encoded.shape[1], entities_encoded.shape[2]
    F = 0 if facts_encoded is None else facts_encoded.shape[1]
    out = torch.empty(B, Lc, d, device=captions.device, dtype=torch.float32)
    emb = torch.empty_like(out) if want_emb else None
    L.check(L.load().ick_caption_embed(_p(captions), _p(masks), _p(word_emb), _p(entities_encoded),
                                       _p(facts_encoded), _p(pe), _p(out), _p(emb), B, Lc, K, F, V, d, pad_token,
                                       scale, pos0, *_dargs(drop), _stream()), "ick_caption_embed")
    return (out, emb) if want_emb else out


def context_indicators(captions, facts, K, V, fc_pred_wt=None, fc_pred_b=None, mode=0, eib=None, gate=None,
                       dense_pred=0):
    B, Lc = captions.shape
    F = facts.shape[1]
    T = Lc if mode == 0 else 1
    if eib is None:
        eib = torch.empty(B, T, F, device=captions.device, dtype=torch.float32)
    num_pred = d = 0
    if fc_pred_wt is not None:
        num_pred, d = fc_pred_wt.shape
        if gate is None:
            gate = torch.empty(B, T, d, device=captions.device, dtype=torch.float32)
    elif dense_pred:
        num_pred = d = dense_pred
        if gate is None:
            gate = torch.empty(B, T, d, device=captions.device, dtype=torch.float32)
    L.check(L.load().ick_context_indicators(_p(captions), _p(facts), _p(fc_pred_wt), _p(fc_pred_b), _p(eib),
                                            _p(gate), B, Lc, T, K, F, V, num_pred, d, mode, _stream()),
            "ick_context_indicators")
    return eib, gate


def pointer_scores(h, ctx, w, bias, out, col0, ind=None, out_gmap=None):
    B, T, d = h.shape
    Kc = ctx.shape[1]
    L.check(L.load().ick_pointer_scores(_p(h), _p(ctx), _p(w), _p(bias), _p(ind), _p(out), B, T, Kc, d,
                                        out.stride(-2), col0, _p(out_gmap), _stream()), "ick_pointer_scores")
    return out


def mul(a, b, out=None):
    if out is None:
        out = torch.empty_like(a)
    L.check(L.load().ick_mul(_p(a), _p(b), _p(out), a.numel(), _stream()), "ick_mul")
    return out


def top2(scores):
    B, Vx = scores.shape
    best = torch.empty(B, device=scores.device, dtype=torch.int32)
    second = torch.empty_like(best)
    L.check(L.load().ick_top2(_p(scores), scores.stride(0), B, Vx, _p(best), _p(second), _stream()), "ick_top2")
    return best, second


def greedy_select(scores, output, hist, finished, next_token, next_mask, step, V, K, has_facts, end_token):
    B, Vx = scores.shape
    L.check(L.load().ick_greedy_select(_p(scores), scores.stride(0), B, Vx, _p(output), _p(hist), _p(finished),
                                       _p(next_token), _p(next_mask), step, output.shape[1], V, K, int(has_facts),
                                       end_token, _stream()), "ick_greedy_select")


def greedy_update(best, second, output, hist, finished, next_token, next_mask, step, V, K, has_facts, end_token):
    B, max_len = output.shape
    L.check(L.load().ick_greedy_update(_p(best), _p(second), _p(output), _p(hist), _p(finished), _p(next_token),
                                       _p(next_mask), B, step, max_len, V, K, int(has_facts), end_token, _stream()),
            "ick_greedy_update")

# ... 46 lines not shown
def decode_select_greedy(ctx, pos):
    L.check(L.load().ick_decode_select_greedy(C.byref(ctx), pos, _stream()), "ick_decode_select_greedy")


def decode_select_beam(ctx, beam_state, pos):
    L.check(L.load().ick_decode_select_beam(C.byref(ctx), C.byref(beam_state), pos, _stream()), "ick_decode_select_beam")


def decode_select_beam_rules(ctx, beam_state, rules, pos):
    L.check(L.load().ick_decode_select_beam_rules(C.byref(ctx), C.byref(beam_state), C.byref(rules), pos, _stream()),
            "ick_decode_select_beam_rules")


def decode_select_beam_diverse(ctx, beam_state, rules, diversity, pos):
    L.check(L.load().ick_decode_select_beam_diverse(C.byref(ctx), C.byref(beam_state),
                                                    None if rules is None else C.byref(rules), C.byref(diversity),
                                                    pos, _stream()), "ick_decode_select_beam_diverse")


def decode_select_beam_forced(ctx, beam_state, rules, constraints, pos):
    L.check(L.load().ick_decode_select_beam_forced(C.byref(ctx), C.byref(beam_state),
                                                   None if rules is None else C.byref(rules), C.byref(constraints),
                                                   pos, _stream()), "ick_decode_select_beam_forced")


def decode_select_sample_rules(ctx, sample_state, rules, pos):
    L.check(L.load().ick_decode_select_sample_rules(C.byref(ctx), C.byref(sample_state), C.byref(rules), pos,
                                                    _stream()), "ick_decode_select_sample_rules")


def decode_select_sample(ctx, sample_state, pos):
    L.check(L.load().ick_decode_select_sample(C.byref(ctx), C.byref(sample_state), pos, _stream()),
            "ick_decode_select_sample")


def packed_ce(scores, captions_sorted, decode_len, pad_token, want_grad=False, out_sum=None, out_count=None):
    B, Lc, Vx = scores.shape
    dev = scores.device
    row_loss = torch.empty(B * Lc, device=dev, dtype=torch.float32)
    loss_sum = out_sum if out_sum is not None else torch.empty(1, device=dev, dtype=torch.float32)
    count = out_count if out_count is not None else torch.empty(1, device=dev, dtype=torch.float32)
    dscores = None
    if want_grad:
        dscores = torch.empty(B, Lc, scores.stride(1), device=dev, dtype=torch.float32)[:, :, :Vx]
        assert scores.stride(0) == Lc * scores.stride(1) and scores.stride(2) == 1
    L.check(L.load().ick_packed_ce(_p(scores), scores.stride(1), _p(captions_sorted), _p(decode_len), B, Lc, Vx,
                                   pad_token, _p(row_loss), _p(loss_sum), _p(count), _p(dscores), _stream()),
            "ick_packed_ce")
    return loss_sum, count, dscores


def packed_ce_weighted(scores, captions_sorted, decode_len, weights, pad_token, want_grad=False, out_sum=None,
                       out_count=None):
    B, Lc, Vx = scores.shape
    dev = scores.device
    if weights.shape != (B,) or weights.dtype != torch.float32 or not weights.is_cuda or not weights.is_contiguous():
        raise L.IckError("packed_ce_weighted needs contiguous (B,) float32 weights on the device")
    row_loss = torch.empty(B * Lc, device=dev, dtype=torch.float32)
    loss_sum = out_sum if out_sum is not None else torch.empty(1, device=dev, dtype=torch.float32)
    count = out_count if out_count is not None else torch.empty(1, device=dev, dtype=torch.float32)
    dscores = None
    if want_grad:
        dscores = torch.empty(B, Lc, scores.stride(1), device=dev, dtype=torch.float32)[:, :, :Vx]
        assert scores.stride(0) == Lc * scores.stride(1) and scores.stride(2) == 1
    L.check(L.load().ick_packed_ce_weighted(_p(scores), scores.stride(1), _p(captions_sorted), _p(decode_len),
                                            _p(weights), B, Lc, Vx, pad_token, _p(row_loss), _p(loss_sum), _p(count),
# ... 247 lines not shown
        ev = self.signals.get(key)
        if ev is not None:
            torch.cuda.current_stream().wait_event(ev)

    def wait_or_join(self, key):
        self.flush_group()
        self.flush()
        if key in self.signals:
            self.wait(key)
        else:
            self.join()

    def submit(self, fn, *tensors):
        self.deferred.append((self.mark(), fn, tensors))

    def flush(self):
        work, self.deferred = self.deferred, []
        for ev, fn, tensors in work:
            with self.fork(*tensors, after=ev):
                fn()

    def join(self):
        self.flush_group()
        self.flush()
        if self.pending:
            torch.cuda.current_stream().wait_stream(self.stream)
            self.pending = False


SIDE = None


def linear_bwd(dy, x, w, dw, db, need_dx=True, dx=None, accumulate_dx=False, group_now=False, gate=None,
               gate_scale=1.0, wt_ps=None, xt_ps=None):
    M, N = dy.shape
    K = x.shape[1]

    wg = None
    extra = []
    if dw is not None and xt_ps is not None and gemm_split_mode() >= 1 and not is_deterministic():
        tiles = ((N + 127) // 128) * ((K + 127) // 128)
        split = max(1, min(8, 480 // tiles, M // 512))
        wg = gemm_args(dy, x, dw, N, K, M, 1, dy.stride(0), 1, x.stride(0), dw.stride(0), atomic=True,
                       split_k=split, b_ps=xt_ps)
        if db is not None:
            extra.append(colsum_problem(dy, db, split_k=max(1, min(16, M // 256))))
    elif dw is not None:
        wg = gemm_args(dy, x, dw, N, K, M, 1, dy.stride(0), 1, x.stride(0), dw.stride(0), atomic=True,
                       split_k=wgrad_split(M, N, K, grouped=SIDE is not None), colsum_a=db)

    def param_grads():
        if wg is not None and extra:
            gemm_grouped([wg] + extra)
        elif wg is not None:
            _log_plan(wg)
            L.check(L.load().ick_gemm(C.byref(wg), _stream()), "ick_gemm(wgrad)")
        elif db is not None:
            colsum(dy, db)

    overlap = SIDE is not None and (dw is not None or db is not None)
    if overlap:
        if wg is not None:
            SIDE.add_problem(wg, dy, x, xt_ps)
            for e in extra:
                SIDE.add_problem(e, dy)
            if group_now:
                SIDE.flush_group()
        else:
            SIDE.submit(param_grads, dy, x)
    if need_dx:
        split = max(1, min(16, N // 1024)) if (M * K) <= 1280 * 512 else 1
        if is_deterministic():
            split = 1
        elif accumulate_dx and split == 1 and N >= 512 and (M * K) <= 1280 * 512:
            split = max(1, min(8, (N + 150) // 300))
        if wt_ps is not None and split > 1 and gemm_split_mode() >= 1 and K <= 320:
            split = max(1, min(16, N // 512, 256 // ((M + 63) // 64)))
        if split > 1:
            if dx is None:
                dx = torch.zeros(M, K, device=dy.device, dtype=torch.float32)
            elif not accumulate_dx:
                dx.zero_()
            gemm_raw(dy, w, dx, M, K, N, dy.stride(0), 1, 1, w.stride(0), dx.stride(0), atomic=True, split_k=split,
                     b_ps=wt_ps)
        else:
            if dx is None:
                dx = torch.empty(M, K, device=dy.device, dtype=torch.float32)
            gemm_raw(dy, w, dx, M, K, N, dy.stride(0), 1, 1, w.stride(0), dx.stride(0), accumulate=accumulate_dx,
                     gate=gate, gate_scale=gate_scale)
            gate = None
    if not overlap:
        param_grads()
    if gate is not None:
        relu_bwd(dx, gate, out=dx, scale=gate_scale)
    return dx


def caption_embed_bwd(dx, captions, masks, dword, dee, dfe, V, pad_token, scale, drop=None):
    B, Lc = captions.shape
    K, d = dee.shape[1], dee.shape[2]
    F = 0 if dfe is None else dfe.shape[1]
    L.check(L.load().ick_caption_embed_bwd(_p(dx), _p(captions), _p(masks), _p(dword), _p(dee), _p(dfe), B, Lc, K, F,
                                           V, d, pad_token, scale, *_dargs(drop), _stream()), "ick_caption_embed_bwd")


def pointer_scores_bwd(dscores, col0, h, ctx, w, ind, dh, dctx, dw, dbias):
    B, T, d = h.shape
    Kc = ctx.shape[1]
    L.check(L.load().ick_pointer_scores_bwd(_p(dscores), dscores.stride(-2), col0, _p(h), _p(ctx), _p(w), _p(ind),
                                            _p(dh), _p(dctx), _p(dw), _p(dbias), B, T, Kc, d, _stream()),
            "ick_pointer_scores_bwd")


def entity_encode_bwd(variant, dee, entities, ee, dtype_emb, word_emb=None, dword=None):
    B, K, cols = entities.shape
    d = dee.shape[2]
    L.check(L.load().ick_entity_encode_bwd(L.VARIANT_ID[variant], _p(dee), _p(entities), cols, _p(ee), _p(word_emb),
                                           0 if word_emb is None else word_emb.shape[0], _p(dtype_emb),
                                           dtype_emb.shape[0], _p(dword), B, K, d, _stream()),
            "ick_entity_encode_bwd")


def fact_encode_bwd(dfe, facts, dee, dpred):
    B, F, d = dfe.shape
    K = dee.shape[1]
    L.check(L.load().ick_fact_encode_bwd(_p(dfe), _p(facts), _p(dee), _p(dpred), dpred.shape[0], B, K, F, d,
                                         _stream()), "ick_fact_encode_bwd")


def context_gate_bwd(captions, facts, dgate, dw, dbias, K, V, mode=0):
    B, Lc = captions.shape
    F = facts.shape[1]
    T, d = dgate.shape[1], dgate.shape[2]
    L.check(L.load().ick_context_gate_bwd(_p(captions), _p(facts), _p(dgate), _p(dw), _p(dbias), B, Lc, T, K, F, V,
                                          dw.shape[1], d, mode, _stream()), "ick_context_gate_bwd")


def adam_clamp(p, g, m, v, step, lr, clip=5.0, gscale=1.0, beta1=0.9, beta2=0.999, eps=1e-8, step_tensor=None,
               gscale_den=None):
    L.check(L.load().ick_adam_clamp(_p(p), _p(g), _p(m), _p(v), p.numel(), gscale, clip, lr, beta1, beta2, eps, step,
                                    _p(step_tensor), _p(gscale_den), _stream()), "ick_adam_clamp")
# ... 21 lines not shown
```

image-captioning-with-external-knowledge_amd/profiling.py:

```python
import ctypes as C

import torch

from . import lib as L

PEAK_FP32_MFMA_TFLOPS = 157.3
PEAK_HBM_GBS = 8000.0
PEAK_BF16_MFMA_TFLOPS = 2500.0
PEAK_SPLIT_FP32_EQ_TFLOPS = PEAK_BF16_MFMA_TFLOPS / 6.0
PER_CU_L2_STREAM_GBS = 134.0


def _struct(arg):
    return arg._obj if hasattr(arg, "_obj") else arg


def _gemm_label(a):
    lay = ("A k-major" if (a.a_rs == 1 and a.a_ks != 1) else "A row-major") + ", " + \
          ("B k-major" if (a.b_rs == 1 and a.b_ks != 1) else "B row-major")
    return "%dx%dx%d (%s%s)" % (a.M, a.N, a.K, lay, ", split-K %d" % a.split_k if a.split_k > 1 else "")


TRACE_KEYS = {}

# ... 38 lines not shown
        a = _struct(args[0])
        return "attention forward (T=%d)" % a.T if a.T > 1 else "attention decode step", 4.0 * a.B * a.H * a.T * a.S * a.dh, "flop"
    if name == "ick_attention_bwd":
        a = _struct(args[0])
        return "attention backward", 10.0 * a.B * a.H * a.T * a.S * a.dh, "flop"
    if name == "ick_rowchain_fwd":
        a = _struct(args[0])
        fl = 2.0 * a.M * (a.K1 * a.d + (a.d * a.N2 if a.w2p else 0))
        return ("row chain forward (out-projection + add & norm + next Linear)", fl, "flop", 0.0,
                4.0 * (a.K1 * a.d + (a.d * a.N2 if a.w2p else 0)))
    if name == "ick_rowchain_bwd":
        a = _struct(args[0])
        fl = 2.0 * a.M * ((a.K0 * a.d if a.g0 else 0) + (2 * a.d * a.N1 if a.w1p else 0) + a.d * a.d)
        return ("row chain backward (Linear' + norm' [+ FFN' + norm'] + out-projection')", fl, "flop", 0.0,
                4.0 * ((a.K0 * a.d if a.g0 else 0) + (2 * a.d * a.N1 if a.w1p else 0) + a.d * a.d))
    if name == "ick_pack_weights":
        arr, n = args[0], args[1]
        return "packed weight copies", 8.0 * sum(arr[i].N * arr[i].K for i in range(n)), "byte"
    if name == "ick_presplit_weights":
        arr, n = args[0], args[1]
        return "presplit weights", 10.0 * sum(arr[i].N * arr[i].K for i in range(n)), "byte"
    if name == "ick_add_layernorm":
        rows, d = args[5], args[6]
        return "residual + LayerNorm", 4.0 * rows * d * 3, "byte"
    if name == "ick_layernorm_bwd":
        rows, d = args[9], args[10]
        return "LayerNorm backward", 4.0 * rows * d * 5, "byte"
    if name == "ick_packed_ce":
        B, Lc, Vx = args[4], args[5], args[6]
        return "packed cross entropy (+ gradient)", 4.0 * B * Lc * Vx * (2 if args[11] else 1), "byte"
    if name == "ick_packed_ce_weighted":
        B, Lc, Vx = args[5], args[6], args[7]
        return "weighted packed cross entropy (+ gradient)", 4.0 * B * Lc * Vx * (2 if args[12] else 1), "byte"
    if name == "ick_adam_clamp":
        return "clamp + Adam", 4.0 * args[4] * 7, "byte"
    if name == "ick_adam_clamp_derive":
        return "clamp + Adam + re-laid-out weight copies", float(getattr(L, "ADAM_DERIVE_BYTES", 0)), "byte"
    if name == "ick_decode_layers":
        c = _struct(args[0])
        kv = 4.0 * c.R * c.layers * 2 * c.H * c.S * 32
        w = 4.0 * (c.layers * (4 * c.d * c.d + 2 * c.d * c.d + 2 * c.d * c.FF) + c.V * c.d)
        return "fused decode step (3 kernels / layer + head + vocabulary)", kv + w, "byte"
    if name == "ick_decode_layers_part":
        c = _struct(args[0])
        kv = 4.0 * c.R * c.layers * 2 * c.H * c.S * 32
        w = 4.0 * (c.layers * (4 * c.d * c.d + 2 * c.d * c.d + 2 * c.d * c.FF) + c.V * c.d)
        first = 4.0 * 4 * c.d * c.d
        return ("fused decode step (3 kernels / layer + head + vocabulary)", first if args[2] == 1 else kv + w - first, "byte")
    if name == "ick_decode_select_greedy":
        return "greedy selection + next-token embedding", None, None
    return name[4:].replace("_", " "), None, None


class _Profiled:
    def __init__(self, lib):
        self._lib = lib

    def __getattr__(self, name):
        fn = getattr(self._lib, name)
        argtypes = L.SIGNATURES.get(name)
        if L.PROFILE is None or not argtypes or argtypes[-1] is not L.vp:
            return fn

        def timed(*args):
            label, work, unit, *rest = classify(name, args)
            e0, e1 = torch.cuda.Event(enable_timing=True), torch.cuda.Event(enable_timing=True)
# ... 62 lines not shown
```

image-captioning-with-external-knowledge_amd/training.py:

```python
import functools
import math
import os
import weakref

import torch

from . import dp, ops
from .decoder import DropSites
from .lib import IckError
from .weights import DerivedWeights


class Tape:

    def __init__(self):
        self.enc_layers = {}
        self.dec_layers = []
        self.misc = {}


def _p(x):
    return x.detach()


def forward_with_tape(dec, captions, caption_masks, entities, facts, enc_tok, gmap, seed=0, epoch=None,
                      fresh_pack=False, overlap=False, feats=None, conv1=None, side_tail=None, derived=None, pre_side=None):
    tape = Tape()
    m = tape.misc
    ds = DropSites(seed, dec.training, epoch)
    d, V, H = dec.emb_dim, dec.vocab_size, dec.num_heads
    B, L = captions.shape
    P = feats.shape[2] * feats.shape[3] if feats is not None else enc_tok.shape[1]
    K = entities.shape[1]
    dev = captions.device
    Fn = facts.shape[1] if dec.has_facts else 0
    nseg = 2 * len(dec.transformer_decoder.layers)
    S = P + K + Fn
    mem = torch.empty(B, S, d, device=dev, dtype=torch.float32)
    kv = torch.empty(B, nseg, H, S, ops.DHP, device=dev, dtype=torch.float32)
    tape.enc_layers["entities"] = []
    if dec.has_facts:
        tape.enc_layers["facts"] = []
    side = ops.SideStream(priority=-1) if overlap else None
    if side is None and side_tail is not None:
        side_tail()

    chain = dec.chain_supported()
    staged = chain and fresh_pack and overlap and derived is None
    first = lambda k: k[0] != "d" or (k[1] == 0 and k[2] in ("so", "cq", "si"))
    split_on = ops.gemm_split_mode() >= 1 and not ops.is_deterministic()

    lazy = pre_side is not None and side is not None and feats is not None and derived is not None
    if pre_side is not None and not lazy:
        pre_side()
    ee, fe = (None, None) if lazy else dec._encode_entities(entities, facts)
    if derived is not None:
        wkv, bkv, pk = derived.wkv, derived.bkv, derived.pk
        m["pkb"] = derived.pkb
        if split_on:
# ... 91 lines not shown
    if staged:
        dec._chain_pack(fresh=True, subset=lambda k: not first(k))
    elif derived is None and pk is not None and dec.chain_bwd_supported():
        m["pkb"] = dec._chain_pack(fresh=fresh_pack, bwd=True, extra=[(("kv", "T"), wkv.t())])
    if dec.has_facts:
        fact_chain()
    ops.project_heads(img, wkv, bkv, nseg, H, S, out=kv, s0=0, grp=P, w_ps=m.get("wkv_ps"))
    ops.stamp("fwd: image K/V projection done")
    m["d_pos"] = ds.site(dec.pos_encoder.dropout.p)
    x = ops.caption_embed(captions, caption_masks, _p(dec.word_embedding.weight), ee, fe, pe, V,
                          dec.word_map["<pad>"], math.sqrt(d), drop=m["d_pos"])
    qkv = None
    for li, layer in enumerate(dec.transformer_decoder.layers):
        t = dec._decoder_self_block(li, layer, x, pk, qkv=qkv, ds=ds, save=True)
        ops.stamp("fwd: layer %d reaches cross-attention" % li)
        if side is not None and li == 0:
            side.wait_or_join("ctx")
        x, qkv = dec._decoder_cross_block(li, layer, t, kv, S, pk, save=True)
        tape.dec_layers.append(t)
    if side is not None:
        side.join()
    ops.stamp("fwd: decoder layers done")
    eib = gate = hv = None
    if dec.has_facts:
        if derived is not None:
            pred_wt = derived.pred_wt
        else:
            pred_wt = _p(dec.fc_predicate.weight).t().contiguous() if fresh_pack else dec._pred_wt()
        eib, gate = ops.context_indicators(captions, facts, K, V, pred_wt, _p(dec.fc_predicate.bias), mode=0)
        hv = ops.mul(x, gate)
    Vx = V + K + Fn
    ld = (Vx + 3) // 4 * 4
    scores = torch.empty(B, L, ld, device=x.device, dtype=torch.float32)[:, :, :Vx]
    dec._score_head(x, ee, fe, eib, hv, scores, m.get("vocab_ps"))
    m.update(ee=ee, fe=fe, mem=mem, kv=kv, h=x, hv=hv, eib=eib, gate=gate, captions=captions, masks=caption_masks,
             entities=entities, facts=facts, P=P, K=K, Fn=Fn, S=S, wkv=wkv)
    return scores, tape


def _keep_scale(drop):
    return 1.0 if drop is None else 1.0 / (1.0 - drop[0])


def _g(grads, param):
    return grads.get(id(param))


def _lin_bwd(grads, dy2, x2, lin_w, lin_b, w_rows=None, need_dx=True, dx=None, acc=False, group_now=False,
             gate=None, gate_scale=1.0, wt_ps=None, xt_ps=None):
    gw, gb = _g(grads, lin_w), _g(grads, lin_b)
    w = _p(lin_w)
    if w_rows is not None:
        w = w[w_rows]
        gw = gw[w_rows] if gw is not None else None
        gb = gb[w_rows] if gb is not None else None
    return ops.linear_bwd(dy2, x2, w, gw, gb, need_dx=need_dx, dx=dx, accumulate_dx=acc, group_now=group_now,
                          gate=gate, gate_scale=gate_scale, wt_ps=wt_ps, xt_ps=xt_ps)


def _prezeroed(dec, captions, entities, facts):
    B, L = captions.shape[0], captions.shape[1]
    d, dev = dec.emb_dim, captions.device
    pre = {"dhv": torch.zeros(B * L, d, device=dev, dtype=torch.float32),
           "dee": torch.zeros(B, entities.shape[1], d, device=dev, dtype=torch.float32)}
    if facts is not None:
        pre["dfe"] = torch.zeros(B, facts.shape[1], d, device=dev, dtype=torch.float32)
    return pre


def _norm_args(t, i, res, layer_norm, grads, M, d, dev):
    return dict(o=t["o%d" % i], res=res, mean=t["m%d" % i], rstd=t["r%d" % i], gamma=_p(layer_norm.weight),
                drop=t["d%d" % i], do=torch.empty(M, d, device=dev, dtype=torch.float32),
                part=ops.ln_partials(M, d, dev))


def _context_encoder_bwd(dec, stack, tapes, dx, grads, pkb=None, tag="e", g_first=None):
    H, d = dec.num_heads, dec.emb_dim
    layers = list(stack.layers)
    if pkb is not None:
        dev = tapes[0]["x"].device
        dz, g0, w0p = dx, None, None
        if g_first is not None:
            dz, (g0, w0p) = None, g_first
        for li in reversed(range(len(layers))):
            layer, t = layers[li], tapes[li]
            B, T, _ = t["x"].shape
            M = B * T
            n2 = _norm_args(t, 2, t["x1"], layer.norm2, grads, M, d, dev)
            n1 = _norm_args(t, 1, t["x"], layer.norm1, grads, M, d, dev)
            dpre = torch.empty(M, layer.linear1.out_features, device=dev, dtype=torch.float32)
# ... 160 lines not shown
                               b_ps=mem_t_ps)
            extra = [] if gb is None else [ops.colsum_problem(sl, gb[d:], split_k=max(1, min(16, rows // 512)))]
        else:
            wg = ops.gemm_args(sl, mem2, gw[d:], 2 * d, d, rows, 1, sl.stride(0), 1, d, d, atomic=True,
                               split_k=1 if ops.is_deterministic() else 16,
                               colsum_a=None if gb is None else gb[d:])
            extra = []
        if ops.SIDE is not None:
            ops.SIDE.add_problem(wg, dkv_rows, mem2, mem_t_ps)
            for e in extra:
                ops.SIDE.add_problem(e, dkv_rows)
        else:
            ops.gemm_grouped([wg] + extra)
    elif gb is not None:
        ops.colsum(sl, gb[d:])


def _memory_t_presplit(m, B, S, d):
    if ops.gemm_split_mode() < 1 or ops.is_deterministic() or B * S < 2048:
        return None
    mem2 = m["mem"].view(B * S, d)
    buf = ops.presplit_buffer(d, B * S, mem2.device)

    def make():
        ops.presplit_weights([(mem2.t(), buf)])

    if ops.SIDE is not None:
        ops.SIDE.submit(make, mem2, buf)
    else:
        make()
    return buf


def _rows_t_presplit(x2):
    rows, d = x2.shape
    if ops.gemm_split_mode() < 1 or ops.is_deterministic() or rows < 1024:
        return None
    buf = ops.presplit_buffer(d, rows, x2.device)

    def make():
        ops.presplit_weights([(x2.t(), buf)])

    if ops.SIDE is not None:
        ops.SIDE.submit(make, x2, buf)
    else:
        make()
    return buf


def backward_from_tape(dec, tape, dscores, grads, overlap=True, want_image_grad=False):
    bp = BackwardPass(dec, tape, dscores, grads, overlap, want_image_grad)
    bp.early(join=False)
    bp.late()
    return tape.misc.get("d_img")


def early_parameters(dec):
    mods = [dec.fc_vocab, dec.fc_entity, dec.transformer_decoder]
    for name in ("fc_fact", "fc_predicate"):
        if getattr(dec, name, None) is not None:
            mods.append(getattr(dec, name))
    seen, out = set(), []
    for mod in mods:
        for prm in mod.parameters():
            if id(prm) not in seen:
                seen.add(id(prm))
                out.append(prm)
    return out


class BackwardPass:

    def __init__(self, dec, tape, dscores, grads, overlap=True, want_image_grad=False):
        self.side = ops.SideStream() if overlap else None
# ... 13 lines not shown
        self.joined = join

    def late(self):
        if self.side is not None and getattr(self, "joined", False):
            self.retired = self.side
            self.side = ops.SideStream()
        self._run(True)


def _backward_phases(dec, tape, dscores, grads, want_image_grad=False):
    m = tape.misc
    d, V, H = dec.emb_dim, dec.vocab_size, dec.num_heads
    h, ee, fe = m["h"], m["ee"], m["fe"]
    grads = dict(grads)
    for prm in unique_parameters(dec):
        if id(prm) not in grads and prm is not dec.word_embedding.weight:
            grads[id(prm)] = torch.zeros_like(prm)
    B, L, _ = h.shape
    P, K, Fn, S = m["P"], m["K"], m["Fn"], m["S"]
    M = B * L
    Vx = dscores.shape[2]
    dsc2 = dscores.view(M, Vx)
    dev = h.device
    pre = m.get("prezero") or {}

    def zeroed(name, like):
        t = pre.get(name)
        return t if t is not None and t.shape == like.shape else torch.zeros_like(like)

    dee = zeroed("dee", ee)
    dfe = zeroed("dfe", fe) if fe is not None else None
    hv = m["hv"] if dec.has_facts else h
    dhv0 = pre.get("dhv")
    hv_t_ps = _rows_t_presplit(hv.view(M, d)) if _g(grads, dec.fc_vocab.weight) is not None else None
    if dhv0 is not None and dhv0.shape == (M, d) and not ops.is_deterministic():
        dhv = _lin_bwd(grads, dsc2[:, :V], hv.view(M, d), dec.fc_vocab.weight, dec.fc_vocab.bias, dx=dhv0, acc=True,
                       group_now=True, wt_ps=m.get("vocab_t_ps"), xt_ps=hv_t_ps).view(B, L, d)
    else:
        dhv = _lin_bwd(grads, dsc2[:, :V], hv.view(M, d), dec.fc_vocab.weight, dec.fc_vocab.bias,
                       group_now=True, wt_ps=m.get("vocab_t_ps"), xt_ps=hv_t_ps).view(B, L, d)
    if dec.has_facts:
        dh = ops.mul(dhv, m["gate"])
        dgate = ops.mul(dhv, h)
        gw, gb = _g(grads, dec.fc_predicate.weight), _g(grads, dec.fc_predicate.bias)
        if gw is not None:
            ops.context_gate_bwd(m["captions"], m["facts"], dgate, gw, gb, K, V, mode=0)
    else:
        dh = dhv

    def gbuf(param):
        return _g(grads, param)

    ops.pointer_scores_bwd(dscores, V, h, ee, _p(dec.fc_entity.weight), None, dh, dee, gbuf(dec.fc_entity.weight),
                           gbuf(dec.fc_entity.bias))
    if dec.has_facts:
        ops.pointer_scores_bwd(dscores, V + K, h, fe, _p(dec.fc_fact.weight), m["eib"], dh, dfe,
                               gbuf(dec.fc_fact.weight), gbuf(dec.fc_fact.bias))
    layers = list(dec.transformer_decoder.layers)
    nseg = 2 * len(layers)
    dkv_rows = ops.attention_bwd_buffer((B, S, nseg * d), L, S, d // H, dev)
    dx = dh
    ops.stamp("bwd: head done")
    pkb = m.get("pkb")
    mem_t_ps = _memory_t_presplit(m, B, S, d)
    if pkb is not None:
        state = (dh.view(M, d), None, None)
        for li in reversed(range(len(layers))):
            state = _decoder_layer_bwd_chain(dec, li, layers[li], tape.dec_layers[li], state, dkv_rows, m["kv"], S,
                                             grads, pkb, mem2=m["mem"].view(B * S, d), mem_t_ps=mem_t_ps)
            ops.stamp("bwd: decoder layer %d done" % li)
        dx = state[0]
    else:
        for li in reversed(range(len(layers))):
            dx = _decoder_layer_bwd(dec, li, layers[li], tape.dec_layers[li], dx, dkv_rows, m["kv"], S, grads,
                                    mem2=m["mem"].view(B * S, d), mem_t_ps=mem_t_ps)
            ops.stamp("bwd: decoder layer %d done" % li)
    yield
    nctx = K + Fn
    dkv_ctx = dkv_rows[:, P:]
    fuse_ctx = pkb is not None and ops.rowchain_bwd_supported(nseg * d, d, 0)
    dctx = None
    if not fuse_ctx:
        ksplit = max(1, min(8, (nseg * d) // 450)) if B * nctx * d <= 1280 * 512 else 1
        if ops.is_deterministic():
            ksplit = 1
        dctx = (torch.zeros if ksplit > 1 else torch.empty)(B, nctx, d, device=dev, dtype=torch.float32)
        ops.gemm_raw(dkv_ctx, m["wkv"], dctx, B * nctx, d, nseg * d, nseg * d, 1, 1, d, d, a_grp=nctx,
                     a_gs=S * nseg * d, atomic=ksplit > 1, split_k=ksplit)
    if want_image_grad:
        d_img = torch.empty(B, P, d, device=dev, dtype=torch.float32)
# ... 29 lines not shown
        ctx.dec, ctx.tape, ctx.params, ctx.gmap = dec, tape, params, gmap
        ctx.enc_shape = enc_tok.shape
        return scores

    @staticmethod
    def backward(ctx, dscores):
        dec, params = ctx.dec, ctx.params
        grads = {id(p): torch.zeros_like(p) for p in params if p.requires_grad}
        want_img = ctx.needs_input_grad[5]
        d_img = backward_from_tape(dec, ctx.tape, dscores.contiguous(), grads, overlap=not ops.is_deterministic(),
                                   want_image_grad=want_img)
        d_enc = None
        if want_img:
            d_enc = torch.empty(ctx.enc_shape, device=d_img.device, dtype=torch.float32)
            d_enc.index_copy_(0, ctx.gmap.long(), d_img) if ctx.gmap is not None else d_enc.copy_(d_img)
        return (None,) * 5 + (d_enc, None) + tuple(grads.get(id(p)) for p in params)


def unique_parameters(dec):
    seen, out = set(), []
    for p in dec.parameters():
        if id(p) not in seen:
            seen.add(id(p))
            out.append(p)
    return out


class TrainStep:

    def __init__(self, decoder, lr=4e-4, grad_clip=5.0, betas=(0.9, 0.999), eps=1e-8, process_group=None, seed=0,
                 use_graph=True, encoder=None, deterministic=None, lazy_update=False):
        self.dec = decoder
        self.lazy = bool(lazy_update)
        self._pending = False
        self._gb = None
        if deterministic is None:
            deterministic = ops.is_deterministic()
        else:
            ops.set_deterministic(bool(deterministic))
        self.deterministic = bool(deterministic)
        self.enc = encoder
        self.seed = seed
        self.lr, self.clip, self.betas, self.eps = lr, grad_clip, betas, eps
        self.pg = process_group
        self.use_graph = use_graph
        self.step_count = 0
        params = [p for p in unique_parameters(decoder) if p.requires_grad]
        early_ids = {id(p) for p in early_parameters(decoder)}
        params = [p for p in params if id(p) in early_ids] + [p for p in params if id(p) not in early_ids]
        dev = params[0].device
        pad = lambda k: (k + 63) // 64 * 64
        n = sum(pad(p.numel()) for p in params)
        self.n = n
        self.n_early = sum(pad(p.numel()) for p in params if id(p) in early_ids)
        self.flat_p = torch.zeros(n, device=dev, dtype=torch.float32)
        self.flat_g = torch.zeros(n + 2, device=dev, dtype=torch.float32)
        self.flat_m = torch.zeros(n, device=dev, dtype=torch.float32)
        self.flat_v = torch.zeros(n, device=dev, dtype=torch.float32)
        self.counter = torch.zeros(1, device=dev, dtype=torch.int32)
        self.one = torch.ones(1, device=dev, dtype=torch.float32)
        self.grads = {}
        off = 0
        with torch.no_grad():
            for p in params:
                k = p.numel()
                self.flat_p[off:off + k].copy_(p.reshape(-1))
                p.data = self.flat_p[off:off + k].view(p.shape)
                self.grads[id(p)] = self.flat_g[off:off + k].view(p.shape)
                off += pad(k)
        self.params = params
        self._graphs = {}
        self.derived = None
        self._derived_tried = False
        dp.broadcast_bucket(self.flat_p, self.pg)
        env = os.environ.get("ICK_SPLIT_ALLREDUCE", "0")
        self.allreduce_probe_ms = None
        if dp.world_size(self.pg) > 1 and (env == "auto" or os.environ.get("ICK_ALLREDUCE_PROBE") == "1"):
            self.allreduce_probe_ms = dp.time_all_reduce(self.flat_g, self.pg)
        if env == "auto":
            self.split = self.allreduce_probe_ms is not None and self.allreduce_probe_ms > 0.26
        else:
            self.split = env not in ("", "0")

    def _overlap(self, off_switch):
        if self.deterministic:
            return False
        return bool((self.use_graph or os.environ.get("ICK_GROUP_SAME_STREAM")) and not os.environ.get(off_switch))

    def _enc_kwargs(self, enc_in):
        if enc_in.dim() == 4:
            c1 = self.enc.conv1
            return dict(enc_tok=None, feats=enc_in, conv1=(c1.weight.detach(), c1.bias.detach(), self.enc.conv1_presplit()))
        return dict(enc_tok=enc_in)

    def _loss(self, scores, captions, decode_len, weights):
        tail = dict(want_grad=True, out_sum=self.flat_g[self.n:self.n + 1], out_count=self.flat_g[self.n + 1:])
        pad = self.dec.word_map["<pad>"]
        if weights is None:
            return ops.packed_ce(scores, captions, decode_len, pad, **tail)
        return ops.packed_ce_weighted(scores, captions, decode_len, weights, pad, **tail)

    def _part_a(self, captions, caption_masks, entities, facts, enc_in, gmap, lengths, weights=None):
        dec = self.dec
        ops.stamp("A: start")
        box = {}

        def tail():
            self.flat_g.zero_()
            box["decode_len"] = (lengths.reshape(-1) - 1).to(torch.int32)
            box["prezero"] = _prezeroed(dec, captions, entities, facts)

        scores, tape = forward_with_tape(dec, captions, caption_masks, entities, facts, gmap=gmap,
                                         seed=self.seed * 2654435761 & 0xFFFFFFFF, epoch=self.counter, fresh_pack=True,
                                         overlap=self._overlap("ICK_NO_FWD_OVERLAP"),
                                         side_tail=tail, derived=self.derived,
                                         pre_side=self._deferred_update if self._lazy_active(enc_in) else None,
                                         **self._enc_kwargs(enc_in))
        decode_len = box["decode_len"]
        tape.misc["prezero"] = box.get("prezero")
        ops.stamp("fwd: scores done")
        _, _, dscores = self._loss(scores, captions, decode_len, weights)
        ops.stamp("CE done")
        backward_from_tape(dec, tape, dscores, self.grads, overlap=self._overlap("ICK_NO_BWD_OVERLAP"))
        ops.stamp("A: end (after join)")
        return self.flat_g

    def _lazy_active(self, enc_in):
        return bool(self.lazy and self.use_graph and self.derived is not None and not self.split and not self.deterministic
                    and enc_in is not None and enc_in.dim() == 4 and self._overlap("ICK_NO_FWD_OVERLAP"))

    def _deferred_update(self):
        self._adam()
        ops.counter_add_if(self.counter, 1, self.flat_g[self.n + 1:])

    def flush(self):
        if not self._pending:
            return
        if self._gb is not None:
            self._gb.replay()
        else:
            self._part_b()
        self.flat_g[self.n + 1:].zero_()
        self._pending = False
        self.dec.invalidate_caches()
        if self.derived is not None:
            self.derived.mark_current()

    def _adam(self):
        hyper = (1, self.lr, self.clip, 1.0, self.betas[0], self.betas[1], self.eps)
        if self.derived is not None:
            ops.adam_clamp_derive(self.flat_p, self.flat_g, self.flat_m, self.flat_v, self.derived.items_dev,
                                  self.derived.blocks_dev, self.derived.n_blocks, *hyper, step_tensor=self.counter,
                                  gscale_den=self.flat_g[self.n + 1:], nbytes=self.derived.nbytes)
        else:
            ops.adam_clamp(self.flat_p[:self.n], self.flat_g[:self.n], self.flat_m, self.flat_v, *hyper,
                           step_tensor=self.counter, gscale_den=self.flat_g[self.n + 1:])

    def _part_a1(self, captions, caption_masks, entities, facts, enc_in, gmap, lengths, weights=None):
        dec = self.dec
        box = {}

        def tail():
            self.flat_g.zero_()
            box["decode_len"] = (lengths.reshape(-1) - 1).to(torch.int32)
            box["prezero"] = _prezeroed(dec, captions, entities, facts)

        scores, tape = forward_with_tape(dec, captions, caption_masks, entities, facts, gmap=gmap,
                                         seed=self.seed * 2654435761 & 0xFFFFFFFF, epoch=self.counter, fresh_pack=True,
                                         overlap=self._overlap("ICK_NO_FWD_OVERLAP"),
                                         side_tail=tail, derived=self.derived, **self._enc_kwargs(enc_in))
        decode_len = box["decode_len"]
        tape.misc["prezero"] = box.get("prezero")
        self._ce = self._loss(scores, captions, decode_len, weights)
        self._bp = BackwardPass(dec, tape, self._ce[2], self.grads,
                                overlap=self._overlap("ICK_NO_BWD_OVERLAP"))
        self._bp.early(join=True)
        return self.flat_g

    def _part_a2(self):
        self._bp.late()
        return self.flat_g

    def _part_b(self):
        ops.stamp("B: start")
        self._adam()
        ops.counter_add(self.counter, 1)
        ops.stamp("B: end")
        return self.flat_g

    def _capture(self, fn, inputs):
        static = [None if t is None else t.contiguous().clone() for t in inputs]
        side = torch.cuda.Stream()
        side.wait_stream(torch.cuda.current_stream())
        with torch.cuda.stream(side):
            fn(*static)
        torch.cuda.current_stream().wait_stream(side)
        g = torch.cuda.CUDAGraph()
        with ops.capture(g):
            fn(*static)
        return g, static

    def _capture_split(self, inputs):
        static = [None if t is None else t.contiguous().clone() for t in inputs]
        side = torch.cuda.Stream()
        side.wait_stream(torch.cuda.current_stream())
        with torch.cuda.stream(side):
# ... 214 lines not shown
```

include/ick_amd.h:

```cpp
#ifndef ICK_AMD_H
#define ICK_AMD_H

#include <stdint.h>

#ifdef __cplusplus
extern "C" {
#endif

#define ICK_OK 0
#define ICK_EINVAL (-1)
#define ICK_EALIGN (-2)
#define ICK_EWORKSPACE (-3)

#define ICK_MAX_LAYERS 8

int ick_version(void);
int ick_set_deterministic(int on);
int ick_get_deterministic(void);
int ick_device_info(int* num_cu, int* wave_size, char* arch_name, int arch_name_len);

typedef struct {
    const float* A; const float* B; float* C; const float* bias;
    int32_t M, N, K;
    int64_t a_rs, a_ks; int32_t a_grp; int64_t a_gs; const int32_t* a_gmap;
    int64_t b_rs, b_ks;
    int64_t c_rs; int32_t c_grp; int64_t c_gs; const int32_t* c_gmap;
    int32_t flags;
    int32_t split_k;
    float   alpha;
    int32_t hs_dh, hs_dhp, hs_H, hs_S, hs_s0;
    float drop_p; uint32_t drop_seed, drop_site;
    const uint32_t* drop_epoch;
    int64_t a_extent, b_extent;
    float* colsum_a;
    const float* gate;
    int64_t gate_rs; float gate_scale;
    const void* b_ps;
} ick_gemm_args;

#define ICK_GEMM_RELU 1
#define ICK_GEMM_ACCUM 2
#define ICK_GEMM_ATOMIC 4
#define ICK_GEMM_COLSUM_ONLY 16

int ick_gemm(const ick_gemm_args* args, void* stream);
typedef struct {
    int32_t tile_m, tile_n, waves, tiles_m, tiles_n, split_k, a_kmajor, b_kmajor, vec;
    int32_t split_bf16;
    int32_t presplit;
} ick_gemm_plan_info;
int ick_gemm_plan(const ick_gemm_args* args, ick_gemm_plan_info* out);
int ick_set_gemm_split(int mode);
int ick_get_gemm_split(void);
typedef struct {
    const float* src; void* dst;
    int32_t N, K;
    int64_t src_rs, src_cs;
} ick_presplit_item;
int ick_presplit_bytes(int32_t N, int32_t K, int64_t* bytes);
int ick_presplit_weights(const ick_presplit_item* items, int32_t count, void* stream);
int ick_gemm_grouped(const ick_gemm_args* problems, int32_t count, void* stream);

int ick_add_layernorm(const float* x, const float* res, const float* gamma, const float* beta,
                      float* y, int64_t rows, int32_t d, float eps,
                      int64_t x_ld, int64_t res_ld, int64_t y_ld,
                      float* save_mean, float* save_rstd,
                      float drop_p, uint32_t drop_seed, uint32_t drop_site,
                      const uint32_t* drop_epoch, void* stream);

typedef struct {
    const float* A; int64_t a_rs; int32_t a_grp; int64_t a_gs;
    int32_t M, K1, d;
    const float* w1p; const float* b1;
    const float* res; int64_t res_rs;
    const float* gamma; const float* beta; float eps;
    float drop1_p; uint32_t drop_seed, drop1_site; const uint32_t* drop_epoch;
    float* o; int64_t o_rs;
    float* x; int64_t x_rs; int32_t x_grp; int64_t x_gs;
    float* mean; float* rstd;
    const float* w2p; const float* b2; int32_t N2; int32_t flags;
    float drop2_p; uint32_t drop2_site;
    float* y2; int64_t y2_rs; int32_t y2_grp; int64_t y2_gs;
    int32_t hs_dh, hs_dhp, hs_H, hs_S, hs_s0;
} ick_rowchain_args;
#define ICK_CHAIN_SLIM 256
#define ICK_CHAIN_PROJ 512
int ick_rowchain_supported(int32_t K1, int32_t d, int32_t N2);
int ick_rowchain_fwd(const ick_rowchain_args* args, void* stream);

typedef struct {
// ... 218 lines not shown
                        int32_t B, int32_t K, int32_t F, int32_t d, void* stream);
int ick_context_gate_bwd(const int64_t* captions, const int64_t* facts, const float* dgate, float* dw,
                         float* dbias, int32_t B, int32_t L, int32_t T, int32_t K, int32_t F, int32_t V,
                         int32_t num_pred, int32_t d, int32_t mode, void* stream);
int ick_adam_clamp(float* p, float* g, float* m, float* v, int64_t n, float gscale, float clip, float lr,
                   float beta1, float beta2, float eps, int32_t step, const uint32_t* step_ptr,
                   const float* gscale_den, void* stream);
typedef struct ick_adam_item {
    int64_t off;
    int32_t rows, K, drow0, Nd;
    float* pack;
    float* pack_t;
    float* copy;
    void* ps;
    void* ps_t;
    float* tr;
    int64_t copy_ld, tr_ld;
} ick_adam_item;
typedef struct ick_adam_block {
    int32_t item, tn, tk, cnt4;
    int64_t off4;
    float* copy;
} ick_adam_block;
int ick_adam_clamp_derive(float* p, float* g, float* m, float* v, const ick_adam_item* items,
                          const ick_adam_block* blocks, int32_t n_blocks, float gscale, float clip, float lr,
                          float beta1, float beta2, float eps, int32_t step, const uint32_t* step_ptr,
                          const float* gscale_den, void* stream);
int ick_counter_add(uint32_t* counter, uint32_t inc, void* stream);
int ick_counter_add_if(uint32_t* counter, uint32_t inc, const float* flag, void* stream);
int ick_copy_batch(const void* const* src, void* const* dst, const long long* bytes, int n, void* stream);
int ick_timestamp(unsigned long long* out, void* stream);
int ick_scale_by_ratio(float* x, int64_t n, const float* num, const float* den, void* stream);

#ifdef __cplusplus
}
#endif
#endif
```

Measured before the change: 734,500 decode-steps/s.

## Pack valid caption rows in the output head to skip padded positions

Adds a device-computed row map that compacts only the valid (non-padded) decode positions, so the vocab GEMM, pointer scores, cross-entropy and their backward passes run over packed rows. Because the graph is captured, the kernels read the row count from device memory through device_bound and exit early for tiles beyond it, while the launch grids stay fixed. This is meant to remove wasted FLOPs and memory traffic on padded rows in the largest GEMMs (vocab 10000). It adds a row-map kernel, gather steps and extra bound checks, and its benefit depends on how much padding the caption lengths leave.

```diff
diff --git a/image-captioning-with-external-knowledge_amd/csrc/backward.hip b/image-captioning-with-external-knowledge_amd/csrc/backward.hip
--- a/image-captioning-with-external-knowledge_amd/csrc/backward.hip
+++ b/image-captioning-with-external-knowledge_amd/csrc/backward.hip
@@ -264,10 +264,18 @@
 __global__ __launch_bounds__(256) void pointer_bwd_dh_kernel(const float* __restrict__ ds, int64_t ds_ld, int col0,
                                                              const float* __restrict__ ctx, const float* __restrict__ w,
                                                              const float* __restrict__ ind, float* __restrict__ dh,
-                                                             int T, int Kc, int d) {
+                                                             int T, int Kc, int d, const int32_t* __restrict__ rowmap,
+                                                             const int32_t* __restrict__ count) {
     chain_priority();
-    const int b = blockIdx.y, t = blockIdx.x;
-    const float* dsr = ds + ((int64_t)b * T + t) * ds_ld + col0;
+    int b = blockIdx.y, t = blockIdx.x;
+    int64_t dsrow = (int64_t)b * T + t;
+    if (rowmap != nullptr) {
+        if (dsrow >= device_bound((int)gridDim.y * T, count)) return;
+        const int lr = rowmap[dsrow];
+        b = lr / T;
+        t = lr - b * T;
+    }
+    const float* dsr = ds + dsrow * ds_ld + col0;
     for (int c = threadIdx.x; c < d; c += 256) {
         float acc = 0.f;
         const float* cc = ctx + (int64_t)b * Kc * d + c;
@@ -297,7 +305,8 @@
                                                                const float* __restrict__ h, const float* __restrict__ ctx,
                                                                const float* __restrict__ w, const float* __restrict__ ind,
                                                                float* __restrict__ dctx, float* __restrict__ dw,
-                                                               float* __restrict__ dbias, int B, int T, int Kc, int d) {
+                                                               float* __restrict__ dbias, int B, int T, int Kc, int d,
+                                                               const int32_t* __restrict__ rowstart) {
     chain_priority();
     extern __shared__ float gs[];
     float* red = gs + T * Kc;
@@ -305,9 +314,11 @@
     const int lane = threadIdx.x & 63, wave = threadIdx.x >> 6;
   for (int b = SEQ ? 0 : blockIdx.x; b < (SEQ ? B : (int)blockIdx.x + 1); ++b) {
     float bsum = 0.f;
+    const int64_t row0 = rowstart ? rowstart[b] : (int64_t)b * T;
+    const int nrow = rowstart ? min(T, rowstart[b + 1] - rowstart[b]) : T;
     for (int idx = threadIdx.x; idx < T * Kc; idx += 256) {
         const int t = idx / Kc, k = idx - t * Kc;
-        float g = ds[((int64_t)b * T + t) * ds_ld + col0 + k];
+        float g = t < nrow ? ds[(row0 + t) * ds_ld + col0 + k] : 0.f;
         bsum += g;
         if (ind) g *= ind[((int64_t)b * T + t) * Kc + k];
         gs[idx] = g;
@@ -600,17 +611,27 @@
 extern "C" int ick_pointer_scores_bwd(const float* ds, int64_t ds_ld, int32_t col0, const float* h, const float* ctx,
                                       const float* w, const float* ind, float* dh, float* dctx, float* dw,
                                       float* dbias, int32_t B, int32_t T, int32_t Kc, int32_t d, void* stream) {
+    return ick_pointer_scores_bwd_packed(ds, ds_ld, col0, h, ctx, w, ind, dh, dctx, dw, dbias, B, T, Kc, d, nullptr, nullptr,
+                                         stream);
+}
+
+extern "C" int ick_pointer_scores_bwd_packed(const float* ds, int64_t ds_ld, int32_t col0, const float* h, const float* ctx,
+                                             const float* w, const float* ind, float* dh, float* dctx, float* dw,
+                                             float* dbias, int32_t B, int32_t T, int32_t Kc, int32_t d,
+                                             const int32_t* rowmap, const int32_t* rowstart, void* stream) {
     ICK_CHECK_ARG(ds && h && ctx && w && dh && dctx && dw && dbias && B > 0 && B <= 65535 && T > 0 && Kc > 0 && d > 0);
+    ICK_CHECK_ARG((rowmap == nullptr) == (rowstart == nullptr) && (int64_t)B * T <= INT32_MAX);
     hipStream_t s = (hipStream_t)stream;
-    hipLaunchKernelGGL(pointer_bwd_dh_kernel, dim3(T, B), dim3(256), 0, s, ds, ds_ld, col0, ctx, w, ind, dh, T, Kc, d);
+    hipLaunchKernelGGL(pointer_bwd_dh_kernel, dim3(T, B), dim3(256), 0, s, ds, ds_ld, col0, ctx, w, ind, dh, T, Kc, d, rowmap,
+                       rowstart ? rowstart + B : nullptr);
     const size_t smem = ((size_t)T * Kc + 4 + 256) * sizeof(float);
     ICK_CHECK_ARG(smem <= 64 * 1024);
     if (deterministic())
         hipLaunchKernelGGL(pointer_bwd_dctx_kernel<true>, dim3(1, ceil_div(d, 64)), dim3(256), smem, s, ds, ds_ld, col0, h,
-                           ctx, w, ind, dctx, dw, dbias, B, T, Kc, d);
+                           ctx, w, ind, dctx, dw, dbias, B, T, Kc, d, rowstart);
     else
         hipLaunchKernelGGL(pointer_bwd_dctx_kernel<false>, dim3(B, ceil_div(d, 64)), dim3(256), smem, s, ds, ds_ld, col0, h,
-                           ctx, w, ind, dctx, dw, dbias, B, T, Kc, d);
+                           ctx, w, ind, dctx, dw, dbias, B, T, Kc, d, rowstart);
     ICK_LAUNCH_RET();
 }
 
diff --git a/image-captioning-with-external-knowledge_amd/csrc/common.h b/image-captioning-with-external-knowledge_amd/csrc/common.h
--- a/image-captioning-with-external-knowledge_amd/csrc/common.h
+++ b/image-captioning-with-external-knowledge_amd/csrc/common.h
@@ -140,6 +140,16 @@
     return seed + *epoch;
 #endif
 }
+__device__ __forceinline__ int device_bound(int host, const int32_t* dev) {
+    if (dev == nullptr) return host;
+#if defined(__HIP_DEVICE_COMPILE__)
+    int v;
+    asm volatile("s_load_dword %0, %1, 0x0\n\ts_waitcnt lgkmcnt(0)" : "=s"(v) : "s"(dev) : "memory");
+    return min(host, max(v, 0));
+#else
+    return host;
+#endif
+}
 constexpr int kRuleHistMax = 128;
 __device__ __forceinline__ uint4 rule_words(const int32_t* words) {
     if (words == nullptr) return make_uint4(0u, 0u, 0u, 0u);
diff --git a/image-captioning-with-external-knowledge_amd/csrc/gemm.hip b/image-captioning-with-external-knowledge_amd/csrc/gemm.hip
--- a/image-captioning-with-external-knowledge_amd/csrc/gemm.hip
+++ b/image-captioning-with-external-knowledge_amd/csrc/gemm.hip
@@ -235,7 +235,7 @@
 
 template <int WM, int WN, int TM, int TN, bool AKM, bool BKM, bool VEC, int BKT, bool SPL = false, int LSTG = 2>
 __device__ __forceinline__ void gemm_tile(const ick_gemm_args& p, int tiles_m, int tiles_n, int kchunk, int bid,
-                                          int zid, float* smem, bool xcd_remap = true) {
+                                          int zid, int nsplit, float* smem, bool xcd_remap = true) {
     constexpr int BM = WM * TM * 16, BN = WN * TN * 16;
     constexpr int BK = BKT;
     using SA = Stager<BM, AKM, VEC, BKT, WM * WN * 64, SPL>;
@@ -262,13 +262,16 @@
     if (tiles_m <= tiles_n) { tm = bid % tiles_m; tn = bid / tiles_m; }
     else { tn = bid % tiles_n; tm = bid / tiles_n; }
     const int m0 = tm * BM, n0 = tn * BN;
+    const int Mr = device_bound(p.M, p.m_bound), Kr = device_bound(p.K, p.k_bound);
+    if (p.k_bound != nullptr) kchunk = ((Kr + nsplit - 1) / nsplit + 31) / 32 * 32;
     const int kbeg = zid * kchunk;
-    const int kend = min(p.K, kbeg + kchunk);
+    if (m0 >= Mr || kbeg >= Kr) return;
+    const int kend = min(Kr, kbeg + kchunk);
 
     const RowMap amap{p.a_grp, p.a_gs, p.a_gmap, p.a_rs};
     const RowMap bmap{0, 0, nullptr, p.b_rs};
     SA sa; SB sb;
-    sa.init(p.A, amap, p.a_ks, m0, p.M, p.a_extent);
+    sa.init(p.A, amap, p.a_ks, m0, Mr, p.a_extent);
     const bool only = (p.flags & ICK_GEMM_COLSUM_ONLY) != 0;
     sb.init(only ? p.A : p.B, bmap, p.b_ks, n0, p.N, p.b_extent);
 
@@ -389,10 +392,10 @@
             }
         }
     }
-    if (colsum && threadIdx.x < BM && m0 + (int)threadIdx.x < p.M) atomicAdd(p.colsum_a + m0 + threadIdx.x, csum);
+    if (colsum && threadIdx.x < BM && m0 + (int)threadIdx.x < Mr) atomicAdd(p.colsum_a + m0 + threadIdx.x, csum);
     if (only) return;
 
-    gemm_epilogue<TM, TN>(p, acc, m0, n0, wm, wn, fi, fq, zid);
+    gemm_epilogue<TM, TN>(p, Mr, acc, m0, n0, wm, wn, fi, fq, zid);
     ICK_GSTAMP(3);
 }
 
@@ -403,7 +406,8 @@
     const int nt = tiles_m * tiles_n;
     int bid = blockIdx.x, zid = blockIdx.z;
     const bool by_split = split_major(bid, zid, nt, gridDim.z);
-    gemm_tile<WM, WN, TM, TN, AKM, BKM, VEC, BKT, SPL, LSTG>(p, tiles_m, tiles_n, kchunk, bid, zid, smem, !by_split);
+    gemm_tile<WM, WN, TM, TN, AKM, BKM, VEC, BKT, SPL, LSTG>(p, tiles_m, tiles_n, kchunk, bid, zid, (int)gridDim.z, smem,
+                                                             !by_split);
 }
 
 constexpr int kGroupMax = 8;
@@ -425,7 +429,7 @@
     int zid = local / nt, bid = local - zid * nt;
     const bool by_split = split_major(bid, zid, nt, ga.split[gi]);
     gemm_tile<WM, WN, TM, TN, AKM, BKM, VEC, BKT, SPL>(ga.g[gi], ga.tiles_m[gi], ga.tiles_n[gi], ga.kchunk[gi], bid, zid,
-                                                       smem, !by_split);
+                                                       ga.split[gi], smem, !by_split);
 }
 
 struct Plan {
@@ -544,6 +548,7 @@
     } else {
         a.hs_dh = 0;
     }
+    if (a.m_bound) ICK_CHECK_ARG(!(a.drop_p > 0.f) && a.gate == nullptr && a.colsum_a == nullptr);
     if (a.a_grp <= 0) { a.a_grp = 0; a.a_gmap = nullptr; }
     if (a.c_grp <= 0) { a.c_grp = 0; a.c_gmap = nullptr; }
     bool avec, bvec;
diff --git a/image-captioning-with-external-knowledge_amd/csrc/gemm_common.h b/image-captioning-with-external-knowledge_amd/csrc/gemm_common.h
--- a/image-captioning-with-external-knowledge_amd/csrc/gemm_common.h
+++ b/image-captioning-with-external-knowledge_amd/csrc/gemm_common.h
@@ -69,8 +69,8 @@
 __device__ __forceinline__ int kc_swz(int row) { return (-(row >> 2)) & 3; }
 
 template <int TM, int TN>
-__device__ __forceinline__ void gemm_epilogue(const ick_gemm_args& p, f32x4 (&acc)[TM][TN], int m0, int n0, int wm, int wn,
-                                              int fi, int fq, int zid) {
+__device__ __forceinline__ void gemm_epilogue(const ick_gemm_args& p, int M, f32x4 (&acc)[TM][TN], int m0, int n0, int wm,
+                                              int wn, int fi, int fq, int zid) {
     const bool hs = p.hs_dh > 0;
     const RowMap cmap{p.c_grp, p.c_gs, p.c_gmap, hs ? (int64_t)p.hs_dhp : p.c_rs};
     const int64_t row_bias = hs ? (int64_t)p.hs_s0 * p.hs_dhp : 0;
@@ -97,13 +97,13 @@
 #pragma unroll
             for (int r = 0; r < 4; ++r) {
                 rowid[a][r] = m0 + (wm * TM + a) * 16 + fq * 4 + r;
-                rws[a * 4 + r] = min(rowid[a][r], p.M - 1);
+                rws[a * 4 + r] = min(rowid[a][r], M - 1);
             }
         map_rows<TM * 4>(cmap, rws, mo);
 #pragma unroll
         for (int a = 0; a < TM; ++a)
 #pragma unroll
-            for (int r = 0; r < 4; ++r) coff[a][r] = rowid[a][r] < p.M ? mo[a * 4 + r] + row_bias : -1;
+            for (int r = 0; r < 4; ++r) coff[a][r] = rowid[a][r] < M ? mo[a * 4 + r] + row_bias : -1;
     }
 #pragma unroll
     for (int a = 0; a < TM; ++a)
diff --git a/image-captioning-with-external-knowledge_amd/csrc/gemm_ps.hip b/image-captioning-with-external-knowledge_amd/csrc/gemm_ps.hip
--- a/image-captioning-with-external-knowledge_amd/csrc/gemm_ps.hip
+++ b/image-captioning-with-external-knowledge_amd/csrc/gemm_ps.hip
@@ -42,12 +42,14 @@
     const int nb = local % blocks_n, s = local / blocks_n;
     const int t = threadIdx.x;
     const float* src = it.src;
+    const int Kr = device_bound(it.K, it.k_bound);
+    if (32 * s >= Kr) return;
     const bool al16 = (reinterpret_cast<uintptr_t>(src) & 15) == 0;
     if (it.src_cs == 1) {
         const int r = t >> 2, kk = (t & 3) * 8;
         const int n = nb * 64 + r;
         const int k0 = 32 * s + kk;
-        if (al16 && (it.src_rs & 3) == 0 && n < it.N && k0 + 7 < it.K) {
+        if (al16 && (it.src_rs & 3) == 0 && n < it.N && k0 + 7 < Kr) {
             const float4* q = reinterpret_cast<const float4*>(src + (int64_t)n * it.src_rs + k0);
             const float4 a = q[0], b = q[1];
             tile[r][kk + 0] = a.x; tile[r][kk + 1] = a.y; tile[r][kk + 2] = a.z; tile[r][kk + 3] = a.w;
@@ -56,15 +58,16 @@
 #pragma unroll
             for (int j = 0; j < 8; ++j) {
                 const int k = k0 + j;
-                tile[r][kk + j] = (n < it.N && k < it.K) ? src[(int64_t)n * it.src_rs + k] : 0.f;
+                tile[r][kk + j] = (n < it.N && k < Kr) ? src[(int64_t)n * it.src_rs + k] : 0.f;
             }
         }
     } else {
         const int kk = t >> 3, r0 = (t & 7) * 8;
         const int k = 32 * s + kk;
         const int n0 = nb * 64 + r0;
-        if (al16 && it.src_rs == 1 && (it.src_cs & 3) == 0 && n0 + 7 < it.N && k < it.K) {
-            const float4* q = reinterpret_cast<const float4*>(src + n0 + (int64_t)k * it.src_cs);
+        const int ks = (it.k_map != nullptr && k < Kr) ? it.k_map[k] : k;
+        if (al16 && it.src_rs == 1 && (it.src_cs & 3) == 0 && n0 + 7 < it.N && k < Kr) {
+            const float4* q = reinterpret_cast<const float4*>(src + n0 + (int64_t)ks * it.src_cs);
             const float4 a = q[0], b = q[1];
             tile[r0 + 0][kk] = a.x; tile[r0 + 1][kk] = a.y; tile[r0 + 2][kk] = a.z; tile[r0 + 3][kk] = a.w;
             tile[r0 + 4][kk] = b.x; tile[r0 + 5][kk] = b.y; tile[r0 + 6][kk] = b.z; tile[r0 + 7][kk] = b.w;
@@ -72,7 +75,7 @@
 #pragma unroll
             for (int j = 0; j < 8; ++j) {
                 const int n = n0 + j;
-                tile[n - nb * 64][kk] = (n < it.N && k < it.K) ? src[(int64_t)n * it.src_rs + (int64_t)k * it.src_cs] : 0.f;
+                tile[n - nb * 64][kk] = (n < it.N && k < Kr) ? src[(int64_t)n * it.src_rs + (int64_t)ks * it.src_cs] : 0.f;
             }
         }
     }
@@ -213,8 +216,11 @@
     if (tiles_m <= tiles_n) { tm = bid % tiles_m; tn = bid / tiles_m; }
     else { tn = bid % tiles_n; tm = bid / tiles_n; }
     const int m0 = tm * BM, n0 = tn * BN;
+    const int Mr = device_bound(p.M, p.m_bound), Kr = device_bound(p.K, p.k_bound);
+    if (p.k_bound != nullptr) kchunk = ((Kr + (int)gridDim.z - 1) / (int)gridDim.z + 31) / 32 * 32;
     const int kbeg = zid * kchunk;
-    const int kend = min(p.K, kbeg + kchunk);
+    if (m0 >= Mr || kbeg >= Kr) return;
+    const int kend = min(Kr, kbeg + kchunk);
     const int nk = (kend - kbeg + 31) >> 5;
     const int s0 = kbeg >> 5;
 
@@ -234,20 +240,20 @@
             row = m0 + 4 * c;
             akl[j] = kl;
             extra = 0;
-            const int one[1] = {min(row, p.M - 1)};
+            const int one[1] = {min(row, Mr - 1)};
             int64_t mo[1];
             map_rows<1>(amap, one, mo);
-            avoff[j] = row < p.M ? (uint32_t)(mo[0] * 4) + (uint32_t)((int64_t)kl * p.a_ks * 4) : kOobOffset;
+            avoff[j] = row < Mr ? (uint32_t)(mo[0] * 4) + (uint32_t)((int64_t)kl * p.a_ks * 4) : kOobOffset;
         } else {
             const int rt = g * 8 + (lane >> 3), cpos = lane & 7;
             const int c = cpos ^ ((rt >> 1) & 7);
             row = m0 + rt;
             akl[j] = 4 * c;
             extra = 4 * c;
-            const int one[1] = {min(row, p.M - 1)};
+            const int one[1] = {min(row, Mr - 1)};
             int64_t mo[1];
             map_rows<1>(amap, one, mo);
-            avoff[j] = row < p.M ? (uint32_t)((mo[0] + extra) * 4) : kOobOffset;
+            avoff[j] = row < Mr ? (uint32_t)((mo[0] + extra) * 4) : kOobOffset;
         }
     }
     const __amdgpu_buffer_rsrc_t rsrc_b =
@@ -370,7 +376,7 @@
     const unsigned long long t_loop_end = t_end;
 #endif
     ICK_WAIT_VMCNT(0);
-    gemm_epilogue<TM, TN>(p, acc, m0, n0, wm, wn, fi, fq, zid);
+    gemm_epilogue<TM, TN>(p, Mr, acc, m0, n0, wm, wn, fi, fq, zid);
 #ifdef ICK_PS_STAMPS
     asm volatile("s_waitcnt vmcnt(0)" ::: "memory");
     ICK_PSTAMP(t_end);
@@ -455,6 +461,7 @@
             const ick_presplit_item& it = items[i0 + i];
             ICK_CHECK_ARG(it.src && it.dst && it.N > 0 && it.K > 0);
             ICK_CHECK_ARG(it.src_cs == 1 || it.src_rs == 1);
+            ICK_CHECK_ARG(it.k_map == nullptr || (it.src_rs == 1 && it.src_cs != 1));
             ICK_CHECK_ARG((reinterpret_cast<uintptr_t>(it.dst) & 15) == 0);
             b.it[i] = it;
             b.first[i] = total;
diff --git a/image-captioning-with-external-knowledge_amd/csrc/score_head.hip b/image-captioning-with-external-knowledge_amd/csrc/score_head.hip
--- a/image-captioning-with-external-knowledge_amd/csrc/score_head.hip
+++ b/image-captioning-with-external-knowledge_amd/csrc/score_head.hip
@@ -10,11 +10,22 @@
                                                              const float* __restrict__ w, const float* __restrict__ bias,
                                                              const float* __restrict__ ind, float* __restrict__ out,
                                                              int T, int Kc, int d, int64_t out_ld, int col0,
-                                                             const int32_t* __restrict__ out_gmap) {
+                                                             const int32_t* __restrict__ out_gmap,
+                                                             const int32_t* __restrict__ rowmap,
+                                                             const int32_t* __restrict__ count) {
     chain_priority();
     constexpr int KB = 4;
     const int lane = threadIdx.x & 63, wave = threadIdx.x >> 6;
-    const int b = blockIdx.y, t = blockIdx.x;
+    int b = blockIdx.y, t = blockIdx.x;
+    int64_t orow_id = -1;
+    if (rowmap != nullptr) {
+        const int m = b * T + t;
+        if (m >= device_bound((int)gridDim.y * T, count)) return;
+        const int lr = rowmap[m];
+        b = lr / T;
+        t = lr - b * T;
+        orow_id = m;
+    }
     const float* hr = h + ((int64_t)b * T + t) * d;
     float hv[NJ], wv[NJ];
 #pragma unroll
@@ -23,8 +34,8 @@
         hv[j] = c < d ? hr[c] : 0.f;
         wv[j] = c < d ? w[c] : 0.f;
     }
-    const int ob = out_gmap ? out_gmap[b] : b;
-    float* orow = out + ((int64_t)ob * T + t) * out_ld + col0;
+    if (orow_id < 0) orow_id = (int64_t)(out_gmap ? out_gmap[b] : b) * T + t;
+    float* orow = out + orow_id * out_ld + col0;
     const float bs = bias[0];
     for (int k0 = wave; k0 < Kc; k0 += 4 * KB) {
         float cv[KB][NJ];
@@ -172,19 +183,27 @@
                           max_len, V, K, has_facts, end_token);
 }
 
-template <bool kWeighted>
+template <bool kWeighted, bool kPacked = false>
 __global__ __launch_bounds__(256) void packed_ce_rows_kernel(const float* __restrict__ scores, int64_t ld,
                                                              const int64_t* __restrict__ caps,
                                                              const int32_t* __restrict__ dl, int L, int Vx, int pad,
                                                              float* __restrict__ row_loss, float* __restrict__ dscores,
-                                                             const float* __restrict__ weight) {
+                                                             const float* __restrict__ weight,
+                                                             const int32_t* __restrict__ rowmap) {
     __shared__ float red[4];
-    const int t = blockIdx.x, b = blockIdx.y, tid = threadIdx.x;
+    int t = blockIdx.x, b = blockIdx.y;
+    const int tid = threadIdx.x;
     const int64_t row = (int64_t)b * L + t;
+    if constexpr (kPacked) {
+        if (row >= device_bound((int)gridDim.y * L, dl)) return;
+        const int lr = rowmap[row];
+        b = lr / L;
+        t = lr - b * L;
+    }
     const float* r = scores + row * ld;
     float* dr = dscores ? dscores + row * ld : nullptr;
     int64_t target = -1;
-    bool use = t < L - 1 && t < dl[b];
+    bool use = t < L - 1 && (kPacked || t < dl[b]);
     if (use) {
         target = caps[(int64_t)b * L + t + 1];
         use = target != pad && target >= 0 && target < Vx;
@@ -332,18 +351,85 @@
 template <bool kWeighted>
 __global__ __launch_bounds__(256) void packed_ce_reduce_kernel(const float* __restrict__ row_loss, int n, int L,
                                                                const float* __restrict__ weight,
-                                                               float* __restrict__ loss_sum, float* __restrict__ count) {
+                                                               float* __restrict__ loss_sum, float* __restrict__ count,
+                                                               const int32_t* __restrict__ rowmap,
+                                                               const int32_t* __restrict__ nrows) {
     __shared__ float red[4];
     float s = 0.f, c = 0.f;
+    n = device_bound(n, nrows);
     for (int i = threadIdx.x; i < n; i += 256) {
         const float v = row_loss[i];
-        if (v > -0.5f) { s += kWeighted ? weight[i / L] * v : v; c += 1.f; }
+        if (v > -0.5f) { s += kWeighted ? weight[(rowmap ? rowmap[i] : i) / L] * v : v; c += 1.f; }
     }
     s = block_sum<4>(s, red);
     c = block_sum<4>(c, red);
     if (threadIdx.x == 0) { loss_sum[0] = s; count[0] = c; }
 }
 
+__global__ __launch_bounds__(256) void head_rowmap_kernel(const int64_t* __restrict__ lengths, int B, int L,
+                                                          int32_t* __restrict__ decode_len, int32_t* __restrict__ rowstart,
+                                                          int32_t* __restrict__ rowmap) {
+    __shared__ int part[256];
+    __shared__ int total;
+    const int tid = threadIdx.x;
+    const int per = (B + 255) / 256;
+    const int b0 = min(B, tid * per), b1 = min(B, b0 + per);
+    auto valid = [&](int64_t len) { return (int)min((int64_t)(L - 1), max((int64_t)0, len - 1)); };
+    int sum = 0;
+    for (int b = b0; b < b1; ++b) {
+        const int64_t len = lengths[b];
+        decode_len[b] = (int32_t)(len - 1);
+        sum += valid(len);
+    }
+    part[tid] = sum;
+    __syncthreads();
+    if (tid == 0) {
+        int run = 0;
+        for (int i = 0; i < 256; ++i) { const int v = part[i]; part[i] = run; run += v; }
+        total = run;
+        rowstart[B] = run;
+    }
+    __syncthreads();
+    int run = part[tid];
+    for (int b = b0; b < b1; ++b) {
+        const int n = valid(lengths[b]);
+        rowstart[b] = run;
+        for (int t = 0; t < n; ++t) rowmap[run + t] = b * L + t;
+        run += n;
+    }
+    for (int m = total + tid; m < B * L; m += 256) rowmap[m] = 0;
+}
+
+__global__ __launch_bounds__(256) void gather_rows_kernel(const float* __restrict__ src, int64_t src_rs,
+                                                          const int32_t* __restrict__ rowmap,
+                                                          const int32_t* __restrict__ count, float* __restrict__ dst,
+                                                          int64_t dst_rs, int max_rows, int d) {
+    const int m = blockIdx.x * 4 + (threadIdx.x >> 6), lane = threadIdx.x & 63;
+    if (m >= device_bound(max_rows, count)) return;
+    const float* s = src + (int64_t)rowmap[m] * src_rs;
+    float* o = dst + (int64_t)m * dst_rs;
+    for (int c = lane; c < d; c += 64) o[c] = s[c];
+}
+
+}
+}
+
+namespace ick {
+namespace {
+int launch_pointer_scores(const float* h, const float* ctx, const float* w, const float* bias, const float* ind, float* out,
+                          int B, int T, int Kc, int d, int64_t out_ld, int col0, const int32_t* out_gmap,
+                          const int32_t* rowmap, const int32_t* count, hipStream_t s) {
+    if (d <= 320)
+        hipLaunchKernelGGL(pointer_scores_kernel<5>, dim3(T, B), dim3(256), 0, s, h, ctx, w, bias, ind, out, T, Kc, d,
+                           out_ld, col0, out_gmap, rowmap, count);
+    else if (d <= 512)
+        hipLaunchKernelGGL(pointer_scores_kernel<8>, dim3(T, B), dim3(256), 0, s, h, ctx, w, bias, ind, out, T, Kc, d,
+                           out_ld, col0, out_gmap, rowmap, count);
+    else
+        hipLaunchKernelGGL(pointer_scores_kernel<kMaxPerLane>, dim3(T, B), dim3(256), 0, s, h, ctx, w, bias, ind, out, T,
+                           Kc, d, out_ld, col0, out_gmap, rowmap, count);
+    ICK_LAUNCH_RET();
+}
 }
 }
 
@@ -353,16 +439,36 @@
     using namespace ick;
     ICK_CHECK_ARG(h && ctx && w && bias && out && B > 0 && T > 0 && Kc > 0 && d > 0 && d <= 64 * kMaxPerLane);
     ICK_CHECK_ARG(B <= 65535 && col0 >= 0 && out_ld >= col0 + Kc);
-    hipStream_t s = (hipStream_t)stream;
-    if (d <= 320)
-        hipLaunchKernelGGL(pointer_scores_kernel<5>, dim3(T, B), dim3(256), 0, s, h, ctx, w, bias, ind, out, T, Kc, d,
-                           out_ld, col0, out_gmap);
-    else if (d <= 512)
-        hipLaunchKernelGGL(pointer_scores_kernel<8>, dim3(T, B), dim3(256), 0, s, h, ctx, w, bias, ind, out, T, Kc, d,
-                           out_ld, col0, out_gmap);
-    else
-        hipLaunchKernelGGL(pointer_scores_kernel<kMaxPerLane>, dim3(T, B), dim3(256), 0, s, h, ctx, w, bias, ind, out, T,
-                           Kc, d, out_ld, col0, out_gmap);
+    return ick::launch_pointer_scores(h, ctx, w, bias, ind, out, B, T, Kc, d, out_ld, col0, out_gmap, nullptr, nullptr,
+                                      (hipStream_t)stream);
+}
+
+extern "C" int ick_pointer_scores_packed(const float* h, const float* ctx, const float* w, const float* bias,
+                                         const float* ind, float* out, int32_t B, int32_t T, int32_t Kc, int32_t d,
+                                         int64_t out_ld, int32_t col0, const int32_t* rowmap, const int32_t* count,
+                                         void* stream) {
+    using namespace ick;
+    ICK_CHECK_ARG(h && ctx && w && bias && out && B > 0 && T > 0 && Kc > 0 && d > 0 && d <= 64 * kMaxPerLane);
+    ICK_CHECK_ARG(B <= 65535 && col0 >= 0 && out_ld >= col0 + Kc && rowmap && count && (int64_t)B * T <= INT32_MAX);
+    return launch_pointer_scores(h, ctx, w, bias, ind, out, B, T, Kc, d, out_ld, col0, nullptr, rowmap, count,
+                                 (hipStream_t)stream);
+}
+
+extern "C" int ick_head_rowmap(const int64_t* lengths, int32_t B, int32_t L, int32_t* decode_len, int32_t* rowstart,
+                               int32_t* rowmap, void* stream) {
+    using namespace ick;
+    ICK_CHECK_ARG(lengths && decode_len && rowstart && rowmap && B > 0 && L > 0 && (int64_t)B * L <= INT32_MAX);
+    hipLaunchKernelGGL(head_rowmap_kernel, dim3(1), dim3(256), 0, (hipStream_t)stream, lengths, B, L, decode_len, rowstart,
+                       rowmap);
+    ICK_LAUNCH_RET();
+}
+
+extern "C" int ick_gather_rows(const float* src, int64_t src_rs, const int32_t* rowmap, const int32_t* count, float* dst,
+                               int64_t dst_rs, int32_t max_rows, int32_t d, void* stream) {
+    using namespace ick;
+    ICK_CHECK_ARG(src && rowmap && count && dst && max_rows > 0 && d > 0 && src_rs >= d && dst_rs >= d);
+    hipLaunchKernelGGL(gather_rows_kernel, dim3(ceil_div(max_rows, 4)), dim3(256), 0, (hipStream_t)stream, src, src_rs,
+                       rowmap, count, dst, dst_rs, max_rows, d);
     ICK_LAUNCH_RET();
 }
 
@@ -407,9 +513,31 @@
     ICK_CHECK_ARG(B > 0 && B <= 65535 && L > 0 && Vx > 0 && ld >= Vx);
     hipStream_t s = (hipStream_t)stream;
     hipLaunchKernelGGL(packed_ce_rows_kernel<false>, dim3(L, B), dim3(256), 0, s, scores, ld, captions_sorted, decode_len,
-                       L, Vx, pad_token, row_loss, dscores, nullptr);
+                       L, Vx, pad_token, row_loss, dscores, nullptr, nullptr);
     hipLaunchKernelGGL(packed_ce_reduce_kernel<false>, dim3(1), dim3(256), 0, s, row_loss, B * L, L, nullptr, loss_sum,
-                       count);
+                       count, nullptr, nullptr);
+    ICK_LAUNCH_RET();
+}
+
+extern "C" int ick_packed_ce_packed(const float* scores, int64_t ld, const int64_t* captions, const int32_t* rowmap,
+                                    const int32_t* count, const float* weights, int32_t B, int32_t L, int32_t Vx,
+                                    int32_t pad_token, float* row_loss, float* loss_sum, float* count_out, float* dscores,
+                                    void* stream) {
+    using namespace ick;
+    ICK_CHECK_ARG(scores && captions && rowmap && count && row_loss && loss_sum && count_out);
+    ICK_CHECK_ARG(B > 0 && B <= 65535 && L > 0 && Vx > 0 && ld >= Vx && (int64_t)B * L <= INT32_MAX);
+    hipStream_t s = (hipStream_t)stream;
+    if (weights != nullptr) {
+        hipLaunchKernelGGL((packed_ce_rows_kernel<true, true>), dim3(L, B), dim3(256), 0, s, scores, ld, captions, count, L,
+                           Vx, pad_token, row_loss, dscores, weights, rowmap);
+        hipLaunchKernelGGL(packed_ce_reduce_kernel<true>, dim3(1), dim3(256), 0, s, row_loss, B * L, L, weights, loss_sum,
+                           count_out, rowmap, count);
+    } else {
+        hipLaunchKernelGGL((packed_ce_rows_kernel<false, true>), dim3(L, B), dim3(256), 0, s, scores, ld, captions, count, L,
+                           Vx, pad_token, row_loss, dscores, nullptr, rowmap);
+        hipLaunchKernelGGL(packed_ce_reduce_kernel<false>, dim3(1), dim3(256), 0, s, row_loss, B * L, L, nullptr, loss_sum,
+                           count_out, rowmap, count);
+    }
     ICK_LAUNCH_RET();
 }
 
@@ -422,8 +550,8 @@
     ICK_CHECK_ARG(B > 0 && B <= 65535 && L > 0 && Vx > 0 && ld >= Vx && (int64_t)B * L <= INT32_MAX);
     hipStream_t s = (hipStream_t)stream;
     hipLaunchKernelGGL(packed_ce_rows_kernel<true>, dim3(L, B), dim3(256), 0, s, scores, ld, captions_sorted, decode_len,
-                       L, Vx, pad_token, row_loss, dscores, weights);
+                       L, Vx, pad_token, row_loss, dscores, weights, nullptr);
     hipLaunchKernelGGL(packed_ce_reduce_kernel<true>, dim3(1), dim3(256), 0, s, row_loss, B * L, L, weights, loss_sum,
-                       count);
-    ICK_LAUNCH_RET();
-}
+                       count, nullptr, nullptr);
+    ICK_LAUNCH_RET();
+}
diff --git a/image-captioning-with-external-knowledge_amd/decoder.py b/image-captioning-with-external-knowledge_amd/decoder.py
--- a/image-captioning-with-external-knowledge_amd/decoder.py
+++ b/image-captioning-with-external-knowledge_amd/decoder.py
@@ -745,14 +745,15 @@
             heads=None if nxt is None else (3, H, T, 0, T))
         return x3, qkv_n
 
-    def _score_head(self, h, ee, fe, eib, hv, out, vocab_ps=None):
+    def _score_head(self, h, ee, fe, eib, hv, out, vocab_ps=None, pack=None):
         B, T, d = h.shape
         V, K = self.vocab_size, ee.shape[1]
+        gather = {} if pack is None else dict(a_grp=1, a_gs=d, a_gmap=pack.rowmap, m_bound=pack.count)
         ops.gemm_raw(h if hv is None else hv, self.fc_vocab.weight.detach(), out, B * T, V, d, d, 1, d, 1, out.stride(1),
-                     bias=self.fc_vocab.bias.detach(), b_ps=vocab_ps)
-        ops.pointer_scores(h, ee, *_wb(self.fc_entity), out, V)
+                     bias=self.fc_vocab.bias.detach(), b_ps=vocab_ps, **gather)
+        ops.pointer_scores(h, ee, *_wb(self.fc_entity), out, V, pack=pack)
         if self.has_facts:
-            ops.pointer_scores(h, fe, *_wb(self.fc_fact), out, V + K, ind=eib)
+            ops.pointer_scores(h, fe, *_wb(self.fc_fact), out, V + K, ind=eib, pack=pack)
 
     @torch.no_grad()
     def get_context_indicators(self, captions, facts, entity_context_size, out_length):
diff --git a/image-captioning-with-external-knowledge_amd/lib.py b/image-captioning-with-external-knowledge_amd/lib.py
--- a/image-captioning-with-external-knowledge_amd/lib.py
+++ b/image-captioning-with-external-knowledge_amd/lib.py
@@ -30,6 +30,7 @@
         ("a_extent", i64), ("b_extent", i64), ("colsum_a", vp),
         ("gate", vp), ("gate_rs", i64), ("gate_scale", f32),
         ("b_ps", vp),
+        ("m_bound", vp), ("k_bound", vp),
     ]
 
 
@@ -77,7 +78,8 @@
 
 
 class PresplitItem(C.Structure):
-    _fields_ = [("src", vp), ("dst", vp), ("N", i32), ("K", i32), ("src_rs", i64), ("src_cs", i64)]
+    _fields_ = [("src", vp), ("dst", vp), ("N", i32), ("K", i32), ("src_rs", i64), ("src_cs", i64),
+                ("k_map", vp), ("k_bound", vp)]
 
 
 class AdamItem(C.Structure):
@@ -224,6 +226,11 @@
     "ick_timestamp": [vp, vp],
     "ick_copy_batch": [vp, vp, vp, i32, vp],
     "ick_scale_by_ratio": [vp, i64, vp, vp, vp],
+    "ick_head_rowmap": [vp, i32, i32, vp, vp, vp, vp],
+    "ick_pointer_scores_packed": [vp, vp, vp, vp, vp, vp, i32, i32, i32, i32, i64, i32, vp, vp, vp],
+    "ick_packed_ce_packed": [vp, i64, vp, vp, vp, vp, i32, i32, i32, i32, vp, vp, vp, vp, vp],
+    "ick_pointer_scores_bwd_packed": [vp, i64, i32, vp, vp, vp, vp, vp, vp, vp, vp, i32, i32, i32, i32, vp, vp, vp],
+    "ick_gather_rows": [vp, i64, vp, vp, vp, i64, i32, i32, vp],
 }
 
 _lib = None
diff --git a/image-captioning-with-external-knowledge_amd/ops.py b/image-captioning-with-external-knowledge_amd/ops.py
--- a/image-captioning-with-external-knowledge_amd/ops.py
+++ b/image-captioning-with-external-knowledge_amd/ops.py
@@ -45,7 +45,7 @@
 
 def gemm_args(A, B, Cout, M, N, K, a_rs, a_ks, b_rs, b_ks, c_rs, bias=None, a_grp=0, a_gs=0, a_gmap=None,
               c_grp=0, c_gs=0, c_gmap=None, relu=False, accumulate=False, atomic=False, split_k=1, alpha=1.0,
-              drop=None, colsum_a=None, gate=None, gate_scale=1.0, b_ps=None):
+              drop=None, colsum_a=None, gate=None, gate_scale=1.0, b_ps=None, m_bound=None, k_bound=None):
     for t in (A, B, Cout):
         if t.dtype != torch.float32:
             raise L.IckError("ick_gemm operands must be float32, got %s" % t.dtype)
@@ -65,6 +65,10 @@
     if b_ps is not None:
         assert b_ps.numel() * b_ps.element_size() == presplit_bytes(N, K), "b_ps is not the pre-split copy of an (N, K) matrix"
         a.b_ps = _p(b_ps)
+    for name, t in (("m_bound", m_bound), ("k_bound", k_bound)):
+        if t is not None:
+            assert t.dtype == torch.int32 and t.numel() == 1 and t.is_cuda, "%s is a one-element int32 device tensor" % name
+            setattr(a, name, _p(t))
     _drop(a, drop)
     return a
 
@@ -78,13 +82,16 @@
     return int(n.value)
 
 
-def presplit_weights(pairs):
+def presplit_weights(pairs, k_map=None, k_bound=None):
     items = (L.PresplitItem * len(pairs))()
     for it, (src, dst) in zip(items, pairs):
         assert src.dim() == 2 and src.dtype == torch.float32 and (src.stride(1) == 1 or src.stride(0) == 1)
         assert dst.numel() * dst.element_size() == presplit_bytes(src.shape[0], src.shape[1])
         it.src, it.dst, it.N, it.K = _p(src), _p(dst), src.shape[0], src.shape[1]
         it.src_rs, it.src_cs = src.stride(0), src.stride(1)
+        if k_map is not None:
+            assert k_map.dtype == torch.int32 and k_map.numel() >= src.shape[1] and src.stride(0) == 1
+        it.k_map, it.k_bound = _p(k_map), _p(k_bound)
     L.check(L.load().ick_presplit_weights(items, len(pairs), _stream()), "ick_presplit_weights")
 
 
@@ -106,7 +113,7 @@
     return ent[1]
 
 
-def colsum_problem(a2d, out, split_k=1):
+def colsum_problem(a2d, out, split_k=1, k_bound=None):
     rows, cols = a2d.shape
     a = L.GemmArgs()
     a.A, a.colsum_a = _p(a2d), _p(out)
@@ -114,6 +121,7 @@
     a.a_rs, a.a_ks = 1, a2d.stride(0)
     a.flags, a.split_k, a.alpha = L.GEMM_COLSUM_ONLY | (L.GEMM_ATOMIC if split_k > 1 else 0), split_k, 1.0
     a.a_extent = _extent(a2d)
+    a.k_bound = _p(k_bound)
     return a
 
 
@@ -483,9 +491,15 @@
     return eib, gate
 
 
-def pointer_scores(h, ctx, w, bias, out, col0, ind=None, out_gmap=None):
+def pointer_scores(h, ctx, w, bias, out, col0, ind=None, out_gmap=None, pack=None):
     B, T, d = h.shape
     Kc = ctx.shape[1]
+    if pack is not None:
+        assert out_gmap is None
+        L.check(L.load().ick_pointer_scores_packed(_p(h), _p(ctx), _p(w), _p(bias), _p(ind), _p(out), B, T, Kc, d,
+                                                   out.stride(-2), col0, _p(pack.rowmap), _p(pack.count), _stream()),
+                "ick_pointer_scores_packed")
+        return out
     L.check(L.load().ick_pointer_scores(_p(h), _p(ctx), _p(w), _p(bias), _p(ind), _p(out), B, T, Kc, d,
                                         out.stride(-2), col0, _p(out_gmap), _stream()), "ick_pointer_scores")
     return out
@@ -598,6 +612,51 @@
 def decode_select_sample(ctx, sample_state, pos):
     L.check(L.load().ick_decode_select_sample(C.byref(ctx), C.byref(sample_state), pos, _stream()),
             "ick_decode_select_sample")
+
+
+class HeadRows:
+
+    def __init__(self, lengths, B, Lc):
+        dev = lengths.device
+        lengths = lengths.reshape(-1)
+        if lengths.dtype != torch.int64 or not lengths.is_contiguous():
+            lengths = lengths.to(torch.int64).contiguous()
+        assert lengths.numel() == B
+        self.B, self.L = B, Lc
+        self.decode_len = torch.empty(B, device=dev, dtype=torch.int32)
+        self.rowstart = torch.empty(B + 1, device=dev, dtype=torch.int32)
+        self.rowmap = torch.empty(B * Lc, device=dev, dtype=torch.int32)
+        self.count = self.rowstart[B:]
+        L.check(L.load().ick_head_rowmap(_p(lengths), B, Lc, _p(self.decode_len), _p(self.rowstart), _p(self.rowmap),
+                                         _stream()), "ick_head_rowmap")
+
+
+def gather_rows(x2, pack):
+    rows, d = x2.shape
+    assert x2.stride(1) == 1 and rows == pack.rowmap.numel()
+    out = torch.empty(rows, d, device=x2.device, dtype=torch.float32)
+    L.check(L.load().ick_gather_rows(_p(x2), x2.stride(0), _p(pack.rowmap), _p(pack.count), _p(out), d, rows, d,
+                                     _stream()), "ick_gather_rows")
+    return out
+
+
+def packed_ce_rows(scores, captions, pack, pad_token, weights=None, want_grad=False, out_sum=None, out_count=None):
+    B, Lc, Vx = scores.shape
+    dev = scores.device
+    if weights is not None and (weights.shape != (B,) or weights.dtype != torch.float32 or not weights.is_cuda or
+                                not weights.is_contiguous()):
+        raise L.IckError("packed_ce_rows needs contiguous (B,) float32 weights on the device")
+    row_loss = torch.empty(B * Lc, device=dev, dtype=torch.float32)
+    loss_sum = out_sum if out_sum is not None else torch.empty(1, device=dev, dtype=torch.float32)
+    count = out_count if out_count is not None else torch.empty(1, device=dev, dtype=torch.float32)
+    dscores = None
+    assert scores.stride(0) == Lc * scores.stride(1) and scores.stride(2) == 1
+    if want_grad:
+        dscores = torch.empty(B, Lc, scores.stride(1), device=dev, dtype=torch.float32)[:, :, :Vx]
+    L.check(L.load().ick_packed_ce_packed(_p(scores), scores.stride(1), _p(captions), _p(pack.rowmap), _p(pack.count),
+                                          _p(weights), B, Lc, Vx, pad_token, _p(row_loss), _p(loss_sum), _p(count),
+                                          _p(dscores), _stream()), "ick_packed_ce_packed")
+    return loss_sum, count, dscores
 
 
 def packed_ce(scores, captions_sorted, decode_len, pad_token, want_grad=False, out_sum=None, out_count=None):
@@ -911,9 +970,12 @@
 
 
 def linear_bwd(dy, x, w, dw, db, need_dx=True, dx=None, accumulate_dx=False, group_now=False, gate=None,
-               gate_scale=1.0, wt_ps=None, xt_ps=None):
+               gate_scale=1.0, wt_ps=None, xt_ps=None, pack=None):
     M, N = dy.shape
     K = x.shape[1]
+    kb = pack.count if pack is not None else None
+    xk = x
+    assert pack is None or (need_dx and dx is not None and accumulate_dx and gate is None)
 
     wg = None
     extra = []
@@ -921,12 +983,13 @@
         tiles = ((N + 127) // 128) * ((K + 127) // 128)
         split = max(1, min(8, 480 // tiles, M // 512))
         wg = gemm_args(dy, x, dw, N, K, M, 1, dy.stride(0), 1, x.stride(0), dw.stride(0), atomic=True,
-                       split_k=split, b_ps=xt_ps)
+                       split_k=split, b_ps=xt_ps, k_bound=kb)
         if db is not None:
-            extra.append(colsum_problem(dy, db, split_k=max(1, min(16, M // 256))))
+            extra.append(colsum_problem(dy, db, split_k=max(1, min(16, M // 256)), k_bound=kb))
     elif dw is not None:
-        wg = gemm_args(dy, x, dw, N, K, M, 1, dy.stride(0), 1, x.stride(0), dw.stride(0), atomic=True,
-                       split_k=wgrad_split(M, N, K, grouped=SIDE is not None), colsum_a=db)
+        xk = gather_rows(x, pack) if pack is not None else x
+        wg = gemm_args(dy, xk, dw, N, K, M, 1, dy.stride(0), 1, xk.stride(0), dw.stride(0), atomic=True,
+                       split_k=wgrad_split(M, N, K, grouped=SIDE is not None), colsum_a=db, k_bound=kb)
 
     def param_grads():
         if wg is not None and extra:
@@ -935,12 +998,15 @@
             _log_plan(wg)
             L.check(L.load().ick_gemm(C.byref(wg), _stream()), "ick_gemm(wgrad)")
         elif db is not None:
-            colsum(dy, db)
+            if pack is not None:
+                gemm_grouped([colsum_problem(dy, db, k_bound=kb)])
+            else:
+                colsum(dy, db)
 
     overlap = SIDE is not None and (dw is not None or db is not None)
     if overlap:
         if wg is not None:
-            SIDE.add_problem(wg, dy, x, xt_ps)
+            SIDE.add_problem(wg, dy, x, xk, xt_ps)
             for e in extra:
                 SIDE.add_problem(e, dy)
             if group_now:
@@ -948,6 +1014,7 @@
         else:
             SIDE.submit(param_grads, dy, x)
     if need_dx:
+        scatter = {} if pack is None else dict(m_bound=kb, c_grp=1, c_gs=dx.stride(0), c_gmap=pack.rowmap)
         split = max(1, min(16, N // 1024)) if (M * K) <= 1280 * 512 else 1
         if is_deterministic():
             split = 1
@@ -961,12 +1028,12 @@
             elif not accumulate_dx:
                 dx.zero_()
             gemm_raw(dy, w, dx, M, K, N, dy.stride(0), 1, 1, w.stride(0), dx.stride(0), atomic=True, split_k=split,
-                     b_ps=wt_ps)
+                     b_ps=wt_ps, **scatter)
         else:
             if dx is None:
                 dx = torch.empty(M, K, device=dy.device, dtype=torch.float32)
             gemm_raw(dy, w, dx, M, K, N, dy.stride(0), 1, 1, w.stride(0), dx.stride(0), accumulate=accumulate_dx,
-                     gate=gate, gate_scale=gate_scale)
+                     gate=gate, gate_scale=gate_scale, **scatter)
             gate = None
     if not overlap:
         param_grads()
@@ -983,9 +1050,14 @@
                                            V, d, pad_token, scale, *_dargs(drop), _stream()), "ick_caption_embed_bwd")
 
 
-def pointer_scores_bwd(dscores, col0, h, ctx, w, ind, dh, dctx, dw, dbias):
+def pointer_scores_bwd(dscores, col0, h, ctx, w, ind, dh, dctx, dw, dbias, pack=None):
     B, T, d = h.shape
     Kc = ctx.shape[1]
+    if pack is not None:
+        L.check(L.load().ick_pointer_scores_bwd_packed(_p(dscores), dscores.stride(-2), col0, _p(h), _p(ctx), _p(w), _p(ind),
+                                                       _p(dh), _p(dctx), _p(dw), _p(dbias), B, T, Kc, d, _p(pack.rowmap),
+                                                       _p(pack.rowstart), _stream()), "ick_pointer_scores_bwd_packed")
+        return
     L.check(L.load().ick_pointer_scores_bwd(_p(dscores), dscores.stride(-2), col0, _p(h), _p(ctx), _p(w), _p(ind),
                                             _p(dh), _p(dctx), _p(dw), _p(dbias), B, T, Kc, d, _stream()),
             "ick_pointer_scores_bwd")
diff --git a/image-captioning-with-external-knowledge_amd/profiling.py b/image-captioning-with-external-knowledge_amd/profiling.py
--- a/image-captioning-with-external-knowledge_amd/profiling.py
+++ b/image-captioning-with-external-knowledge_amd/profiling.py
@@ -94,6 +94,10 @@
     if name == "ick_packed_ce_weighted":
         B, Lc, Vx = args[5], args[6], args[7]
         return "weighted packed cross entropy (+ gradient)", 4.0 * B * Lc * Vx * (2 if args[12] else 1), "byte"
+    if name == "ick_packed_ce_packed":
+        B, Lc, Vx = args[6], args[7], args[8]
+        return (("weighted " if args[5] else "") + "packed cross entropy (+ gradient)",
+                4.0 * B * Lc * Vx * (2 if args[13] else 1), "byte")
     if name == "ick_adam_clamp":
         return "clamp + Adam", 4.0 * args[4] * 7, "byte"
     if name == "ick_adam_clamp_derive":
diff --git a/image-captioning-with-external-knowledge_amd/training.py b/image-captioning-with-external-knowledge_amd/training.py
--- a/image-captioning-with-external-knowledge_amd/training.py
+++ b/image-captioning-with-external-knowledge_amd/training.py
@@ -24,7 +24,8 @@
 
 
 def forward_with_tape(dec, captions, caption_masks, entities, facts, enc_tok, gmap, seed=0, epoch=None,
-                      fresh_pack=False, overlap=False, feats=None, conv1=None, side_tail=None, derived=None, pre_side=None):
+                      fresh_pack=False, overlap=False, feats=None, conv1=None, side_tail=None, derived=None, pre_side=None,
+                      head_rows=None):
     tape = Tape()
     m = tape.misc
     ds = DropSites(seed, dec.training, epoch)
@@ -182,7 +183,8 @@
     Vx = V + K + Fn
     ld = (Vx + 3) // 4 * 4
     scores = torch.empty(B, L, ld, device=x.device, dtype=torch.float32)[:, :, :Vx]
-    dec._score_head(x, ee, fe, eib, hv, scores, m.get("vocab_ps"))
+    m["pack"] = head_rows() if head_rows is not None else None
+    dec._score_head(x, ee, fe, eib, hv, scores, m.get("vocab_ps"), pack=m["pack"])
     m.update(ee=ee, fe=fe, mem=mem, kv=kv, h=x, hv=hv, eib=eib, gate=gate, captions=captions, masks=caption_masks,
              entities=entities, facts=facts, P=P, K=K, Fn=Fn, S=S, wkv=wkv)
     return scores, tape
@@ -197,7 +199,7 @@
 
 
 def _lin_bwd(grads, dy2, x2, lin_w, lin_b, w_rows=None, need_dx=True, dx=None, acc=False, group_now=False,
-             gate=None, gate_scale=1.0, wt_ps=None, xt_ps=None):
+             gate=None, gate_scale=1.0, wt_ps=None, xt_ps=None, pack=None):
     gw, gb = _g(grads, lin_w), _g(grads, lin_b)
     w = _p(lin_w)
     if w_rows is not None:
@@ -205,7 +207,7 @@
         gw = gw[w_rows] if gw is not None else None
         gb = gb[w_rows] if gb is not None else None
     return ops.linear_bwd(dy2, x2, w, gw, gb, need_dx=need_dx, dx=dx, accumulate_dx=acc, group_now=group_now,
-                          gate=gate, gate_scale=gate_scale, wt_ps=wt_ps, xt_ps=xt_ps)
+                          gate=gate, gate_scale=gate_scale, wt_ps=wt_ps, xt_ps=xt_ps, pack=pack)
 
 
 def _prezeroed(dec, captions, entities, facts):
@@ -432,14 +434,17 @@
     return buf
 
 
-def _rows_t_presplit(x2):
+def _rows_t_presplit(x2, pack=None):
     rows, d = x2.shape
     if ops.gemm_split_mode() < 1 or ops.is_deterministic() or rows < 1024:
         return None
     buf = ops.presplit_buffer(d, rows, x2.device)
 
     def make():
-        ops.presplit_weights([(x2.t(), buf)])
+        if pack is None:
+            ops.presplit_weights([(x2.t(), buf)])
+        else:
+            ops.presplit_weights([(x2.t(), buf)], k_map=pack.rowmap, k_bound=pack.count)
 
     if ops.SIDE is not None:
         ops.SIDE.submit(make, x2, buf)
@@ -519,8 +524,14 @@
     dfe = zeroed("dfe", fe) if fe is not None else None
     hv = m["hv"] if dec.has_facts else h
     dhv0 = pre.get("dhv")
-    hv_t_ps = _rows_t_presplit(hv.view(M, d)) if _g(grads, dec.fc_vocab.weight) is not None else None
-    if dhv0 is not None and dhv0.shape == (M, d) and not ops.is_deterministic():
+    pack = m.get("pack")
+    hv_t_ps = _rows_t_presplit(hv.view(M, d), pack) if _g(grads, dec.fc_vocab.weight) is not None else None
+    if pack is not None:
+        if dhv0 is None or dhv0.shape != (M, d):
+            dhv0 = torch.zeros(M, d, device=dev, dtype=torch.float32)
+        dhv = _lin_bwd(grads, dsc2[:, :V], hv.view(M, d), dec.fc_vocab.weight, dec.fc_vocab.bias, dx=dhv0, acc=True,
+                       group_now=True, wt_ps=m.get("vocab_t_ps"), xt_ps=hv_t_ps, pack=pack).view(B, L, d)
+    elif dhv0 is not None and dhv0.shape == (M, d) and not ops.is_deterministic():
         dhv = _lin_bwd(grads, dsc2[:, :V], hv.view(M, d), dec.fc_vocab.weight, dec.fc_vocab.bias, dx=dhv0, acc=True,
                        group_now=True, wt_ps=m.get("vocab_t_ps"), xt_ps=hv_t_ps).view(B, L, d)
     else:
@@ -539,10 +550,10 @@
         return _g(grads, param)
 
     ops.pointer_scores_bwd(dscores, V, h, ee, _p(dec.fc_entity.weight), None, dh, dee, gbuf(dec.fc_entity.weight),
-                           gbuf(dec.fc_entity.bias))
+                           gbuf(dec.fc_entity.bias), pack=pack)
     if dec.has_facts:
         ops.pointer_scores_bwd(dscores, V + K, h, fe, _p(dec.fc_fact.weight), m["eib"], dh, dfe,
-                               gbuf(dec.fc_fact.weight), gbuf(dec.fc_fact.bias))
+                               gbuf(dec.fc_fact.weight), gbuf(dec.fc_fact.bias), pack=pack)
     layers = list(dec.transformer_decoder.layers)
     nseg = 2 * len(layers)
     dkv_rows = ops.attention_bwd_buffer((B, S, nseg * d), L, S, d // H, dev)
@@ -638,6 +649,7 @@
                  use_graph=True, encoder=None, deterministic=None, lazy_update=False):
         self.dec = decoder
         self.lazy = bool(lazy_update)
+        self.packed_head = os.environ.get("ICK_NO_PACKED_HEAD", "0") in ("", "0")
         self._pending = False
         self._gb = None
         if deterministic is None:
@@ -699,33 +711,43 @@
             return dict(enc_tok=None, feats=enc_in, conv1=(c1.weight.detach(), c1.bias.detach(), self.enc.conv1_presplit()))
         return dict(enc_tok=enc_in)
 
-    def _loss(self, scores, captions, decode_len, weights):
+    def _loss(self, scores, captions, decode_len, weights, pack=None):
         tail = dict(want_grad=True, out_sum=self.flat_g[self.n:self.n + 1], out_count=self.flat_g[self.n + 1:])
         pad = self.dec.word_map["<pad>"]
+        if pack is not None:
+            return ops.packed_ce_rows(scores, captions, pack, pad, weights=weights, **tail)
         if weights is None:
             return ops.packed_ce(scores, captions, decode_len, pad, **tail)
         return ops.packed_ce_weighted(scores, captions, decode_len, weights, pad, **tail)
+
+    def _side_tail(self, box, captions, entities, facts, lengths):
+        def tail():
+            self.flat_g.zero_()
+            if self.packed_head:
+                box["pack"] = ops.HeadRows(lengths, captions.shape[0], captions.shape[1])
+                box["decode_len"] = box["pack"].decode_len
+            else:
+                box["decode_len"] = (lengths.reshape(-1) - 1).to(torch.int32)
+            box["prezero"] = _prezeroed(self.dec, captions, entities, facts)
+
+        return tail
 
     def _part_a(self, captions, caption_masks, entities, facts, enc_in, gmap, lengths, weights=None):
         dec = self.dec
         ops.stamp("A: start")
         box = {}
-
-        def tail():
-            self.flat_g.zero_()
-            box["decode_len"] = (lengths.reshape(-1) - 1).to(torch.int32)
-            box["prezero"] = _prezeroed(dec, captions, entities, facts)
+        tail = self._side_tail(box, captions, entities, facts, lengths)
 
         scores, tape = forward_with_tape(dec, captions, caption_masks, entities, facts, gmap=gmap,
                                          seed=self.seed * 2654435761 & 0xFFFFFFFF, epoch=self.counter, fresh_pack=True,
                                          overlap=self._overlap("ICK_NO_FWD_OVERLAP"),
                                          side_tail=tail, derived=self.derived,
                                          pre_side=self._deferred_update if self._lazy_active(enc_in) else None,
-                                         **self._enc_kwargs(enc_in))
+                                         head_rows=lambda: box.get("pack"), **self._enc_kwargs(enc_in))
         decode_len = box["decode_len"]
         tape.misc["prezero"] = box.get("prezero")
         ops.stamp("fwd: scores done")
-        _, _, dscores = self._loss(scores, captions, decode_len, weights)
+        _, _, dscores = self._loss(scores, captions, decode_len, weights, box.get("pack"))
         ops.stamp("CE done")
         backward_from_tape(dec, tape, dscores, self.grads, overlap=self._overlap("ICK_NO_BWD_OVERLAP"))
         ops.stamp("A: end (after join)")
@@ -765,19 +787,16 @@
     def _part_a1(self, captions, caption_masks, entities, facts, enc_in, gmap, lengths, weights=None):
         dec = self.dec
         box = {}
-
-        def tail():
-            self.flat_g.zero_()
-            box["decode_len"] = (lengths.reshape(-1) - 1).to(torch.int32)
-            box["prezero"] = _prezeroed(dec, captions, entities, facts)
+        tail = self._side_tail(box, captions, entities, facts, lengths)
 
         scores, tape = forward_with_tape(dec, captions, caption_masks, entities, facts, gmap=gmap,
                                          seed=self.seed * 2654435761 & 0xFFFFFFFF, epoch=self.counter, fresh_pack=True,
                                          overlap=self._overlap("ICK_NO_FWD_OVERLAP"),
-                                         side_tail=tail, derived=self.derived, **self._enc_kwargs(enc_in))
+                                         side_tail=tail, derived=self.derived, head_rows=lambda: box.get("pack"),
+                                         **self._enc_kwargs(enc_in))
         decode_len = box["decode_len"]
         tape.misc["prezero"] = box.get("prezero")
-        self._ce = self._loss(scores, captions, decode_len, weights)
+        self._ce = self._loss(scores, captions, decode_len, weights, box.get("pack"))
         self._bp = BackwardPass(dec, tape, self._ce[2], self.grads,
                                 overlap=self._overlap("ICK_NO_BWD_OVERLAP"))
         self._bp.early(join=True)
diff --git a/include/ick_amd.h b/include/ick_amd.h
--- a/include/ick_amd.h
+++ b/include/ick_amd.h
@@ -36,6 +36,8 @@
     const float* gate;
     int64_t gate_rs; float gate_scale;
     const void* b_ps;
+    const int32_t* m_bound;
+    const int32_t* k_bound;
 } ick_gemm_args;
 
 #define ICK_GEMM_RELU 1
@@ -56,6 +58,8 @@
     const float* src; void* dst;
     int32_t N, K;
     int64_t src_rs, src_cs;
+    const int32_t* k_map;
+    const int32_t* k_bound;
 } ick_presplit_item;
 int ick_presplit_bytes(int32_t N, int32_t K, int64_t* bytes);
 int ick_presplit_weights(const ick_presplit_item* items, int32_t count, void* stream);
@@ -340,6 +344,21 @@
 int ick_timestamp(unsigned long long* out, void* stream);
 int ick_scale_by_ratio(float* x, int64_t n, const float* num, const float* den, void* stream);
 
+int ick_head_rowmap(const int64_t* lengths, int32_t B, int32_t L, int32_t* decode_len, int32_t* rowstart,
+                    int32_t* rowmap, void* stream);
+int ick_pointer_scores_packed(const float* h, const float* ctx, const float* w, const float* bias, const float* ind,
+                              float* out, int32_t B, int32_t T, int32_t Kc, int32_t d, int64_t out_ld, int32_t col0,
+                              const int32_t* rowmap, const int32_t* count, void* stream);
+int ick_packed_ce_packed(const float* scores, int64_t ld, const int64_t* captions, const int32_t* rowmap,
+                         const int32_t* count, const float* weights, int32_t B, int32_t L, int32_t Vx, int32_t pad_token,
+                         float* row_loss, float* loss_sum, float* count_out, float* dscores, void* stream);
+int ick_pointer_scores_bwd_packed(const float* ds, int64_t ds_ld, int32_t col0, const float* h, const float* ctx,
+                                  const float* w, const float* ind, float* dh, float* dctx, float* dw, float* dbias,
+                                  int32_t B, int32_t T, int32_t Kc, int32_t d, const int32_t* rowmap,
+                                  const int32_t* rowstart, void* stream);
+int ick_gather_rows(const float* src, int64_t src_rs, const int32_t* rowmap, const int32_t* count, float* dst,
+                    int64_t dst_rs, int32_t max_rows, int32_t d, void* stream);
+
 #ifdef __cplusplus
 }
 #endif
```

After: 758,500 decode-steps/s, median of 6. 1.03x the previous value.
